# mlcolab/Pathfinder.jl

Hardware: AMD Instinct MI355X
Metric: ELBO draws/sec (multipathfinder hot path: fit + ELBO + pool + PSIS + resample) (higher is better)
Workload: dtype f64

## Files before the change

### pathfinder.jl_amd/csrc/api_ctx.hip

```cpp
#include "api_internal.h"

#include <map>
#include <mutex>
#include <string>
#include <stdarg.h>
#include <stdio.h>

static thread_local char g_err[1024] = "";

void pf_set_error(const char *fmt, ...) {
    va_list ap;
    va_start(ap, fmt);
    vsnprintf(g_err, sizeof(g_err), fmt, ap);
    va_end(ap);
}

static hipEvent_t pf_kev_get(pfmi_ctx *c) {
    if (!c->kev_pool.empty()) { hipEvent_t e = c->kev_pool.back(); c->kev_pool.pop_back(); return e; }
    hipEvent_t e = nullptr;
    (void)hipEventCreate(&e);
    return e;
}
static void pf_kernel_resolve(pfmi_ctx *c, bool keep) {
    for (auto &p : c->kpending) {
// ... 5 lines not shown
        }
        if (p.e0) c->kev_pool.push_back(p.e0);
        if (p.e1) c->kev_pool.push_back(p.e1);
    }
    c->kpending.clear();
}
void pf_kernel_begin(pfmi_ctx *c) {
    if (c->profile == 1) (void)hipEventRecord(c->kev0, c->stream);
    else if (c->profile == 2) {
        if (c->kpending.size() >= 4096) pf_kernel_resolve(c, true);
        if (c->kcur) c->kev_pool.push_back(c->kcur);
        c->kcur = pf_kev_get(c);
        if (c->kcur) (void)hipEventRecord(c->kcur, c->stream);
    }
}
void pf_kernel_end(pfmi_ctx *c, const char *name) {
    if (c->profile == 2) {
        hipEvent_t e1 = pf_kev_get(c);
        if (e1) (void)hipEventRecord(e1, c->stream);
        c->kpending.push_back({name, c->kcur, e1});
        c->kcur = nullptr;
        return;
    }
    if (c->profile != 1) return;
    (void)hipEventRecord(c->kev1, c->stream);
    (void)hipEventSynchronize(c->kev1);
    float ms = 0.f;
    (void)hipEventElapsedTime(&ms, c->kev0, c->kev1);
    KernelStat &s = c->kstats[name];
    s.ms += ms;
    s.launches += 1;
}

#define PF_ARENA_BYTES (16u << 20)
#define PF_ARENA_MAX (4u << 20)
void pf_arena_reset(pfmi_ctx *c) { c->arena.off = 0; }
int32_t pf_upload(pfmi_ctx *c, void *dst, const void *src, size_t bytes) {
    if (bytes == 0) return PFMI_OK;
    if (bytes > PF_ARENA_MAX) {
        PF_HIP(hipMemcpyAsync(dst, src, bytes, hipMemcpyHostToDevice, c->stream));
        PF_HIP(hipStreamSynchronize(c->stream));
        pf_arena_reset(c);
        return PFMI_OK;
    }
    PinArena &a = c->arena;
    if (!a.base) {
        void *pp = nullptr;
        PF_HIP(hipHostMalloc(&pp, PF_ARENA_BYTES, hipHostMallocDefault));
        a.base = reinterpret_cast<char *>(pp); a.cap = PF_ARENA_BYTES; a.off = 0;
    }
    if (a.off + bytes > a.cap) {
        PF_HIP(hipStreamSynchronize(c->stream));
        a.off = 0;
    }
    memcpy(a.base + a.off, src, bytes);
    PF_HIP(hipMemcpyAsync(dst, a.base + a.off, bytes, hipMemcpyHostToDevice, c->stream));
    a.off += (bytes + 255) & ~(size_t)255;
    return PFMI_OK;
}
#define PF_DL_BYTES (4u << 20)
#define PF_DL_MAX (1u << 20)
int32_t pf_download(pfmi_ctx *c, void *dst, const void *src, size_t bytes) {
    if (bytes == 0) return PFMI_OK;
    PinArena &a = c->dl;
    if (bytes <= PF_DL_MAX) {
        if (!a.base) {
            void *pp = nullptr;
            PF_HIP(hipHostMalloc(&pp, PF_DL_BYTES, hipHostMallocMapped));
            a.base = reinterpret_cast<char *>(pp); a.cap = PF_DL_BYTES; a.off = 0;
        }
        if (a.off + bytes <= a.cap) {
            static const bool immediate = [] { const char *e = getenv("PFMI_DL_IMMEDIATE"); return e && e[0] == '1'; }();
            if (immediate) PF_HIP(hipMemcpyAsync(a.base + a.off, src, bytes, hipMemcpyDeviceToHost, c->stream));
            c->dl_pending.push_back(DlPending{dst, a.base + a.off, bytes, c->defer, immediate ? nullptr : static_cast<const char *>(src), immediate});
            a.off += (bytes + 255) & ~(size_t)255;
            return PFMI_OK;
        }
    }
    PF_TRY(pf_dl_flush(c));
    PF_HIP(hipMemcpyAsync(dst, src, bytes, hipMemcpyDeviceToHost, c->stream));
    return PFMI_OK;
}
static void pf_deferred_drop(pfmi_ctx *c) { c->dl_pending.clear(); c->post_sync.clear(); c->dl.off = 0; }
#define PF_DL_NSEG 24
struct DlSegs { const char *src[PF_DL_NSEG]; char *dst[PF_DL_NSEG]; uint32_t bytes[PF_DL_NSEG]; };
__global__ __launch_bounds__(256) void pf_dl_gather_kernel(DlSegs S) {
    const int y = blockIdx.y;
    const char *src = S.src[y];
    char *dst = S.dst[y];
    const uint32_t n = S.bytes[y];
    if (((reinterpret_cast<uintptr_t>(src) | reinterpret_cast<uintptr_t>(dst) | n) & 7u) == 0) {
        const uint32_t n8 = n >> 3;
        for (uint32_t i = blockIdx.x * 256 + threadIdx.x; i < n8; i += gridDim.x * 256)
            reinterpret_cast<uint64_t *>(dst)[i] = reinterpret_cast<const uint64_t *>(src)[i];
    } else {
        for (uint32_t i = blockIdx.x * 256 + threadIdx.x; i < n; i += gridDim.x * 256) dst[i] = src[i];
    }
}
int32_t pf_dl_flush(pfmi_ctx *c) {
    DlSegs S;
    int n = 0;
    uint32_t big = 0;
    auto launch = [&]() -> int32_t {
        if (n == 0) return PFMI_OK;
        const unsigned gx = big > (64u << 10) ? 32 : big > (4u << 10) ? 4 : 1;
        hipLaunchKernelGGL(pf_dl_gather_kernel, dim3(gx, (unsigned)n), dim3(256), 0, c->stream, S);
        PF_HIP(hipGetLastError());
        n = 0; big = 0;
        return PFMI_OK;
    };
    for (DlPending &q : c->dl_pending) {
        if (q.issued || q.src == nullptr) continue;
        S.src[n] = q.src; S.dst[n] = const_cast<char *>(q.slot); S.bytes[n] = (uint32_t)q.bytes;
        if ((uint32_t)q.bytes > big) big = (uint32_t)q.bytes;
        q.issued = true;
        if (++n == PF_DL_NSEG) PF_TRY(launch());
    }
    return launch();
}
int32_t pf_stream_sync(pfmi_ctx *c) {
    {
        const int32_t rf = pf_dl_flush(c);
        if (rf != PFMI_OK) { pf_deferred_drop(c); return rf; }
    }
    const hipError_t e = hipStreamSynchronize(c->stream);
    if (e != hipSuccess) { pf_deferred_drop(c); PF_HIP(e); }
    for (const DlPending &q : c->dl_pending) memcpy(q.dst, q.slot, q.bytes);
    c->dl_pending.clear();
    c->dl.off = 0;
    pf_arena_reset(c);
    int32_t rc = PFMI_OK;
    std::vector<std::function<int32_t()>> hooks;
    hooks.swap(c->post_sync);
    for (auto &h : hooks) { const int32_t r = h(); if (rc == PFMI_OK) rc = r; }
    return rc;
}
void pf_download_forget(pfmi_ctx *c) {
    size_t w = 0;
    for (size_t i = 0; i < c->dl_pending.size(); ++i) if (c->dl_pending[i].keep) c->dl_pending[w++] = c->dl_pending[i];
    c->dl_pending.resize(w);
    if (w == 0) c->dl.off = 0;
}
int32_t ensure_pinned(pfmi_ctx *c, size_t x_bytes, size_t lp_bytes) {
    for (int b = 0; b < 2; ++b) {
        if (x_bytes > c->pin_x_cap) {
            if (c->pin_x[b]) (void)hipHostFree(c->pin_x[b]);
            c->pin_x[b] = nullptr;
            PF_HIP(hipHostMalloc(&c->pin_x[b], x_bytes, hipHostMallocDefault));
        }
        if (lp_bytes > c->pin_lp_cap) {
            if (c->pin_lp[b]) (void)hipHostFree(c->pin_lp[b]);
            c->pin_lp[b] = nullptr;
            PF_HIP(hipHostMalloc(&c->pin_lp[b], lp_bytes, hipHostMallocDefault));
        }
        if (!c->cb_ev[b]) PF_HIP(hipEventCreateWithFlags(&c->cb_ev[b], hipEventDisableTiming));
    }
    if (x_bytes > c->pin_x_cap) c->pin_x_cap = x_bytes;
    if (lp_bytes > c->pin_lp_cap) c->pin_lp_cap = lp_bytes;
    return PFMI_OK;
}

namespace {
std::mutex g_dbg_mu;
std::map<std::string, const char *> g_dbg;
}
const char *pf_debug_get(const char *name) {
    {
        std::lock_guard<std::mutex> lk(g_dbg_mu);
        auto it = g_dbg.find(name);
        if (it != g_dbg.end()) return it->second;
    }
    static const bool env_hooks = [] { const char *e = getenv("PFMI_DEBUG_HOOKS"); return e && e[0] == '1'; }();
    return env_hooks ? getenv(name) : nullptr;
}

void stream_abandon(pfmi_ctx *c) {
    for (hipStream_t s : {c->s_opt, c->s_fit, c->s_scan1}) if (s) (void)hipStreamSynchronize(s);
    for (hipStream_t s : c->s_cb) if (s) (void)hipStreamSynchronize(s);
    c->sr.active = false;
    c->stream_pending = false;
    c->stream_drain = false;
}

void lbc_abandon(pfmi_ctx *c) {
    if (!c->lbc.active) return;
    (void)hipStreamSynchronize(c->stream);
    c->lbc.active = false;
    c->opt_pending = false;
}

extern "C" {

const char *pfmi_last_error(void) { return g_err; }

int32_t pfmi_debug_set(const char *key, const char *value) {
    PF_CHECK(key != nullptr && strncmp(key, "PFMI_", 5) == 0, PFMI_ERR_ARG, "debug_set: keys are the PFMI_* hook names");
    const char *copy = (value && value[0]) ? strdup(value) : nullptr;
    PF_CHECK(copy != nullptr || !(value && value[0]), PFMI_ERR_ARG, "debug_set: out of memory");
    std::lock_guard<std::mutex> lk(g_dbg_mu);
    g_dbg[key] = copy;
    return PFMI_OK;
}
int32_t pfmi_version(void) { return 100; }

int32_t pfmi_device_count(int32_t *count) {
    PF_CHECK(count != nullptr, PFMI_ERR_ARG, "null count");
    int n = 0;
    hipError_t e = hipGetDeviceCount(&n);
    if (e != hipSuccess) { *count = 0; pf_set_error("hipGetDeviceCount: %s", hipGetErrorString(e)); return PFMI_ERR_HIP; }
    *count = n;
    return PFMI_OK;
}

int32_t pfmi_create(int32_t device, pfmi_ctx **out) {
    PF_CHECK(out != nullptr, PFMI_ERR_ARG, "null out");
    *out = nullptr;
    int n = 0;
    PF_HIP(hipGetDeviceCount(&n));
    PF_CHECK(n > 0, PFMI_ERR_HIP, "no HIP device visible: libpfmi has no CPU fallback");
    PF_CHECK(device >= 0 && device < n, PFMI_ERR_ARG, "device %d out of range (%d devices)", device, n);
    hipDeviceProp_t prop;
    PF_HIP(hipGetDeviceProperties(&prop, device));
    PF_CHECK(strncmp(prop.gcnArchName, "gfx950", 6) == 0, PFMI_ERR_UNSUPPORTED,
             "libpfmi is built for gfx950 (MI355X) only; device %d is %s", device, prop.gcnArchName);
    PF_HIP(hipSetDevice(device));
    pfmi_ctx *c = new pfmi_ctx();
    c->device = device;
    c->ncu = prop.multiProcessorCount;
    PF_HIP(hipStreamCreateWithFlags(&c->stream, hipStreamNonBlocking));
    PF_HIP(hipEventCreate(&c->ev0));
    PF_HIP(hipEventCreate(&c->ev1));
    PF_HIP(hipEventCreate(&c->kev0));
    PF_HIP(hipEventCreate(&c->kev1));
    *out = c;
    return PFMI_OK;
}

int32_t pfmi_destroy(pfmi_ctx *c) {
    if (!c) return PFMI_OK;
    pf_comm_ctx_dying(c);
    (void)hipSetDevice(c->device);
    stream_abandon(c);
    lbc_abandon(c);
    (void)hipStreamSynchronize(c->stream);
    for (int b = 0; b < 2; ++b) {
        if (c->pin_x[b]) (void)hipHostFree(c->pin_x[b]);
        if (c->pin_lp[b]) (void)hipHostFree(c->pin_lp[b]);
        if (c->cb_ev[b]) (void)hipEventDestroy(c->cb_ev[b]);
    }
    if (c->arena.base) (void)hipHostFree(c->arena.base);
    if (c->dl.base) (void)hipHostFree(c->dl.base);
    (void)hipEventDestroy(c->ev0); (void)hipEventDestroy(c->ev1);
    (void)hipEventDestroy(c->kev0); (void)hipEventDestroy(c->kev1);
    pf_kernel_resolve(c, false);
    for (hipEvent_t e : c->kev_pool) (void)hipEventDestroy(e);
    for (hipEvent_t e : {c->sg_fit, c->sg_opt, c->sg_scan[0], c->sg_scan[1], c->sg_start}) if (e) (void)hipEventDestroy(e);
    for (hipStream_t s : {c->s_opt, c->s_fit, c->s_scan1}) if (s) (void)hipStreamDestroy(s);
    for (hipStream_t s : c->s_cb) if (s) (void)hipStreamDestroy(s);
    for (hipEvent_t e : c->sg_cb) if (e) (void)hipEventDestroy(e);
    if (c->h_prog) (void)hipHostFree(c->h_prog);
    if (c->lc_status) (void)hipHostFree(c->lc_status);
    if (c->h_list) (void)hipHostFree(c->h_list);
    (void)hipStreamDestroy(c->stream);
    delete c;
    return PFMI_OK;
}

int32_t pfmi_sync(pfmi_ctx *c) {
    PF_CTX(c);
    return pf_stream_sync(c);
}

int32_t pfmi_timer_start(pfmi_ctx *c) {
    PF_CTX(c);
    PF_HIP(hipEventRecord(c->ev0, c->stream));
    return PFMI_OK;
}
int32_t pfmi_timer_stop(pfmi_ctx *c, double *ms) {
    PF_CTX(c);
    PF_HIP(hipEventRecord(c->ev1, c->stream));
    PF_HIP(hipEventSynchronize(c->ev1));
    float f = 0.f;
    PF_HIP(hipEventElapsedTime(&f, c->ev0, c->ev1));
    if (ms) *ms = f;
    return PFMI_OK;
}
int32_t pfmi_profile(pfmi_ctx *c, int32_t enable) {
    PF_CTX(c);
    PF_CHECK(enable >= 0 && enable <= 2, PFMI_ERR_ARG, "profile: mode %d outside 0..2", enable);
    pf_kernel_resolve(c, false);
    c->profile = enable;
    c->kstats.clear();
    return PFMI_OK;
}
int32_t pfmi_kernel_time(pfmi_ctx *c, const char *name, double *ms, int64_t *launches) {
    PF_CTX(c);
    PF_CHECK(name != nullptr, PFMI_ERR_ARG, "null name");
    pf_kernel_resolve(c, true);
    if (strcmp(name, "qf_handover_lost") == 0) {
        if (ms) *ms = 0.0;
        if (launches) *launches = c->qf_lost_total;
        return PFMI_OK;
    }
    if (strncmp(name, "qf:", 3) == 0) {
        auto pl = c->qf_plans.find(name);
        if (ms) *ms = 0.0;
        if (launches) *launches = (pl == c->qf_plans.end()) ? 0 : pl->second;
        return PFMI_OK;
    }
    auto it = c->kstats.find(name);
    if (ms) *ms = (it == c->kstats.end()) ? 0.0 : it->second.ms;
    if (launches) *launches = (it == c->kstats.end()) ? 0 : it->second.launches;
    return PFMI_OK;
}

int32_t pfmi_defer_downloads(pfmi_ctx *c, int32_t mode) {
    PF_CHECK(c != nullptr, PFMI_ERR_ARG, "null pfmi_ctx");
    if (mode < 0) { pf_deferred_drop(c); c->defer = false; return PFMI_OK; }
    c->defer = mode != 0;
    return PFMI_OK;
}

int32_t pfmi_host_rand_u64(uint64_t seed, uint64_t t0, int64_t n, uint32_t stream, uint64_t *out) {
    PF_CHECK(n >= 0 && (out != nullptr || n == 0), PFMI_ERR_ARG, "host_rand_u64: bad arguments");
    const uint32_t key0 = (uint32_t)seed, key1 = (uint32_t)(seed >> 32);
    for (int64_t i = 0; i < n; ++i) {
        const uint64_t t = t0 + (uint64_t)i;
        uint32_t c0 = (uint32_t)t, c1 = (uint32_t)(t >> 32), c2 = stream, c3 = 0u, k0 = key0, k1 = key1;
        for (int r = 0; r < 10; ++r) {
            const uint64_t p0 = (uint64_t)0xD2511F53u * c0, p1 = (uint64_t)0xCD9E8D57u * c2;
            const uint32_t n0 = (uint32_t)(p1 >> 32) ^ c1 ^ k0, n2 = (uint32_t)(p0 >> 32) ^ c3 ^ k1;
            c1 = (uint32_t)p1; c3 = (uint32_t)p0; c0 = n0; c2 = n2;
            k0 += 0x9E3779B9u; k1 += 0xBB67AE85u;
        }
        out[i] = (uint64_t)c0 | ((uint64_t)c1 << 32);
    }
    return PFMI_OK;
}
int32_t pfmi_host_rand_u64_multi(int32_t m, const uint64_t *seeds, const uint64_t *t0, int64_t n, uint32_t stream, uint64_t *out) {
    PF_CHECK(m >= 0 && n >= 0 && (m == 0 || (seeds && t0)) && (out != nullptr || (int64_t)m * n == 0), PFMI_ERR_ARG, "host_rand_u64_multi: bad arguments");
    for (int32_t j = 0; j < m; ++j) PF_TRY(pfmi_host_rand_u64(seeds[j], t0[j], n, stream, out + (size_t)j * (size_t)n));
    return PFMI_OK;
}

int32_t pfmi_malloc_dev(pfmi_ctx *c, int64_t bytes, void **dev_ptr) {
    PF_CTX(c);
    PF_CHECK(dev_ptr != nullptr && bytes > 0, PFMI_ERR_ARG, "malloc_dev: bad arguments");
    PF_HIP(hipMalloc(dev_ptr, (size_t)bytes));
    return PFMI_OK;
}
int32_t pfmi_free_dev(pfmi_ctx *c, void *dev_ptr) {
    PF_CTX(c);
    if (dev_ptr) PF_HIP(hipFree(dev_ptr));
    return PFMI_OK;
}
int32_t pfmi_host_alloc(int64_t bytes, void **host_ptr) {
    PF_CHECK(bytes > 0 && host_ptr, PFMI_ERR_ARG, "host_alloc: bad arguments");
    *host_ptr = nullptr;
    PF_HIP(hipHostMalloc(host_ptr, (size_t)bytes, hipHostMallocPortable | hipHostMallocMapped));
    return PFMI_OK;
}
int32_t pfmi_host_free(void *host_ptr) {
    if (host_ptr) PF_HIP(hipHostFree(host_ptr));
    return PFMI_OK;
}
int32_t pfmi_memcpy_h2d(pfmi_ctx *c, void *dst, const void *src, int64_t bytes) {
    PF_CTX(c);
    return pf_upload(c, dst, src, (size_t)bytes);
}
int32_t pfmi_memcpy_d2h(pfmi_ctx *c, void *dst, const void *src, int64_t bytes) {
    PF_CTX(c);
    return d2h(c, dst, src, (size_t)bytes);
}

}
```

### pathfinder.jl_amd/csrc/api_elbo.hip

```cpp
#include "api_internal.h"

#include <algorithm>
#include <array>
#include <chrono>
#include <memory>
#include <thread>
#include <vector>

static void host_callback_block(pfmi_ctx *c, const double *X, int d, int64_t n, double *out) {
    const TargetDev &T = c->target;
    int t = c->cb_threads;
    if (t > n) t = (int)n;
    if (t <= 1) { T.fn(X, d, n, out, T.user); return; }
    const int64_t per = (n + t - 1) / t;
    std::vector<std::thread> th;
    th.reserve((size_t)t - 1);
    for (int i = 1; i < t; ++i) {
        const int64_t j0 = (int64_t)i * per, j1 = std::min<int64_t>(n, j0 + per);
        if (j0 >= j1) break;
        try {
            th.emplace_back([=, &T] { T.fn(X + (size_t)j0 * (size_t)d, d, j1 - j0, out + j0, T.user); });
        } catch (...) {
            T.fn(X + (size_t)j0 * (size_t)d, d, j1 - j0, out + j0, T.user);
        }
    }
    T.fn(X, d, std::min<int64_t>(n, per), out, T.user);
    for (std::thread &x : th) x.join();
}

int32_t callback_logp(pfmi_ctx *c, const double *d_x, int64_t n, double *d_lp) {
    const int d = c->d;
    int64_t chunk = (int64_t)((64ll << 20) / (sizeof(double) * (size_t)d));
    if (chunk < 1) chunk = 1;
    if (chunk > n) chunk = n;
    PF_TRY(ensure_pinned(c, sizeof(double) * (size_t)chunk * d, sizeof(double) * (size_t)chunk));
    for (int64_t s0 = 0; s0 < n; s0 += chunk) {
        const int64_t ns = (n - s0 < chunk) ? n - s0 : chunk;
        PF_TRY(d2h(c, c->pin_x[0], d_x + (size_t)s0 * d, sizeof(double) * (size_t)ns * d));
        host_callback_block(c, reinterpret_cast<const double *>(c->pin_x[0]), d, ns, reinterpret_cast<double *>(c->pin_lp[0]));
        PF_TRY(pf_upload(c, d_lp + s0, c->pin_lp[0], sizeof(double) * (size_t)ns));
    }
    return PFMI_OK;
}

int64_t devcb_chunk_fits(const pfmi_ctx *c, int64_t per_fit_doubles, int64_t nf, int64_t N) {
    double mb = 2048.0;
    const char *e = pf_debug_get("PFMI_DEVCB_CHUNK_MB");
    if (e && atof(e) > 0) mb = atof(e);
    else {
        const int64_t ngroups = (N + 15) / 16, ncu = c->ncu > 0 ? c->ncu : 256;
        const int64_t split = ngroups / 16 > 0 ? ngroups / 16 : 1;
        const double want_mb = (double)((2 * ncu + split - 1) / split) * sizeof(double) * (double)per_fit_doubles / 1048576.0;
        size_t free_b = 0, total_b = 0;
        if (want_mb > mb && hipMemGetInfo(&free_b, &total_b) == hipSuccess) {
            const double cap_mb = (double)free_b / 4.0 / 1048576.0;
            mb = want_mb < cap_mb ? want_mb : (cap_mb > mb ? cap_mb : mb);
        }
    }
    int64_t chunk = (int64_t)(mb * 1048576.0 / (sizeof(double) * (double)per_fit_doubles));
    if (chunk < 1) chunk = 1;
    if (chunk > nf) chunk = nf > 0 ? nf : 1;
    return chunk;
}

int32_t devcb_logp(pfmi_ctx *c, const double *d_x, int64_t n, double *d_lp, const int32_t *d_points, int64_t npts, int64_t N) {
    pf_kernel_begin(c);
    c->target.dev_fn(d_x, c->d, n, d_lp, (void *)c->stream, c->target.user);
    pf_kernel_end(c, "device_callback");
    PF_HIP(hipGetLastError());
    return pf_launch_nan_failed(c, npts, N, d_points, d_lp);
}

int32_t elbo_reserve(pfmi_ctx *c, size_t P, int32_t K, int64_t N) {
    PF_TRY(c->logp.ensure(sizeof(double) * P * N));
    PF_TRY(c->logq.ensure(sizeof(double) * P * N));
    PF_TRY(c->elbo.ensure(sizeof(double) * P));
    PF_TRY(c->se.ensure(sizeof(double) * P));
    return c->best_iter.ensure(sizeof(int64_t) * K);
}

int32_t devcb_scan_block(pfmi_ctx *c, hipStream_t ss, const int32_t *list, const uint64_t *seeds, int64_t n, int64_t N, const double *d_u,
                         int64_t ustride, double *bx, double *blp) {
    PF_TRY(pf_launch_elbo_draws(c, list, seeds, n, 0, N, d_u, ustride, bx, (int64_t)c->d * N, c->logp.as<double>(), c->logq.as<double>(), N,
                                false, true));
    pf_kernel_begin(c);
    c->target.dev_fn(bx, c->d, n * N, blp, (void *)ss, c->target.user);
    pf_kernel_end(c, "device_callback");
    PF_HIP(hipGetLastError());
    return pf_launch_scatter_rows(c, n, N, list, blp, c->logp.as<double>());
}

extern "C" {

int32_t pfmi_set_callback_threads(pfmi_ctx *c, int32_t nthreads) {
    PF_CTX(c);
    PF_CHECK(nthreads >= 1 && nthreads <= 1024, PFMI_ERR_ARG, "set_callback_threads: 1 <= nthreads <= 1024");
    c->cb_threads = nthreads;
    return PFMI_OK;
}

int32_t pfmi_elbo_batch_enqueue(pfmi_ctx *c, int64_t N, const uint64_t *seeds, const double *u_host) {
    PF_CTX_MUT(c);
    PF_CHECK(c->fitted, PFMI_ERR_STATE, "elbo_batch: call pfmi_fit_batch first");
    PF_CHECK(c->target.kind >= 0, PFMI_ERR_STATE, "elbo_batch: call pfmi_set_target first");
    PF_CHECK(c->target.d == c->d, PFMI_ERR_ARG, "target dimension %d != trace dimension %d", c->target.d, c->d);
    PF_CHECK(N >= 1 && seeds, PFMI_ERR_ARG, "elbo_batch: bad arguments");
    const int64_t P = c->P;
    const int d = c->d;
    c->N_e = N;
    PF_TRY(elbo_reserve(c, (size_t)P, c->K, N));
    int64_t nf = 0;
    for (int k = 0; k < c->K; ++k) nf += c->path_npts(k) - 1;
    const size_t off_ls = sizeof(uint64_t) * (size_t)P, off_li = off_ls + sizeof(uint64_t) * (size_t)(nf > 0 ? nf : 1);
    const size_t up_bytes = off_li + sizeof(int32_t) * (size_t)(nf > 0 ? nf : 1);
    std::vector<char> stage(up_bytes);
    memcpy(stage.data(), seeds, sizeof(uint64_t) * (size_t)P);
    {
        uint64_t *ls = reinterpret_cast<uint64_t *>(stage.data() + off_ls);
        int32_t *li = reinterpret_cast<int32_t *>(stage.data() + off_li);
        int64_t t = 0;
        for (int k = 0; k < c->K; ++k)
            for (int64_t p = c->off[k] + 1; p < c->off[k] + c->path_npts(k); ++p, ++t) { li[t] = (int32_t)p; ls[t] = seeds[p]; }
    }
    PF_TRY(c->seeds.ensure(up_bytes + 16));
    c->d_stream_tab = nullptr;
    PF_TRY(pf_upload(c, c->seeds.p, stage.data(), up_bytes));
    uint64_t *d_lseeds = reinterpret_cast<uint64_t *>(c->seeds.as<char>() + off_ls);
    int32_t *d_list = reinterpret_cast<int32_t *>(c->seeds.as<char>() + off_li);
    const double *d_u = nullptr;
    if (u_host) {
        PF_TRY(c->ubuf.ensure(sizeof(double) * (size_t)P * d * N));
        PF_TRY(pf_upload(c, c->ubuf.p, u_host, sizeof(double) * (size_t)P * d * N));
        d_u = c->ubuf.as<double>();
    }
    const int64_t ustride = (int64_t)d * N;
    if (c->target.kind == PFMI_TARGET_DEVICE_CALLBACK) {
        const int64_t per = (int64_t)d * N;
        int64_t chunk = devcb_chunk_fits(c, per, nf, N);
        int nb = nf > 1 ? PF_DCB_NB : 1;
        if (const char *ov = pf_debug_get("PFMI_DEVCB_OVERLAP")) { const int v = atoi(ov); nb = (v <= 0 || nf <= 1) ? 1 : (v < PF_DCB_NB ? (v < 2 ? 2 : v) : PF_DCB_NB); }
        if (nb > 1) {
            size_t free_b = 0, total_b = 0;
            double have = 0.0;
            for (int b = 0; b < PF_DCB_NB; ++b) have += (double)c->dcb_x[b].cap;
            if (hipMemGetInfo(&free_b, &total_b) == hipSuccess) have += (double)free_b;
            if ((double)nb * (double)sizeof(double) * (double)chunk * (double)(per + N) > 0.5 * have || chunk * nb > nf) chunk = (chunk + nb - 1) / nb;
            if (chunk < 1) chunk = 1;
        }
        for (int b = 0; b < nb; ++b) {
            PF_TRY(c->dcb_x[b].ensure(sizeof(double) * (size_t)chunk * per));
            PF_TRY(c->dcb_lp[b].ensure(sizeof(double) * (size_t)chunk * N));
        }
        for (int b = 1; b < nb; ++b)
            if (!c->s_cb[b - 1]) PF_HIP(hipStreamCreateWithFlags(&c->s_cb[b - 1], hipStreamNonBlocking));
        for (int b = 0; b < nb; ++b)
            if (!c->sg_cb[b]) PF_HIP(hipEventCreateWithFlags(&c->sg_cb[b], hipEventDisableTiming));
        if (nb > 1) {
            PF_HIP(hipEventRecord(c->sg_cb[0], c->stream));
            for (int b = 1; b < nb; ++b) PF_HIP(hipStreamWaitEvent(c->s_cb[b - 1], c->sg_cb[0], 0));
        }
        c->cb_bytes_dev = 0.0;
        int64_t blk = 0;
        for (int64_t s0 = 0; s0 < nf; s0 += chunk, ++blk) {
            const int64_t ns = (nf - s0 < chunk) ? nf - s0 : chunk;
            const int b = (int)(blk % nb);
            hipStream_t ss = b ? c->s_cb[b - 1] : c->stream;
            StreamSwap sw(c, ss);
            PF_TRY(devcb_scan_block(c, ss, d_list + s0, d_lseeds + s0, ns, N, d_u, ustride, c->dcb_x[b].as<double>(), c->dcb_lp[b].as<double>()));
            c->cb_bytes_dev += (double)sizeof(double) * (double)ns * (double)per;
        }
        for (int b = 1; b < nb && b < blk; ++b) {
            PF_HIP(hipEventRecord(c->sg_cb[b], c->s_cb[b - 1]));
            PF_HIP(hipStreamWaitEvent(c->stream, c->sg_cb[b], 0));
        }
    } else if (c->target.kind != PFMI_TARGET_HOST_CALLBACK) {
        PF_TRY(pf_launch_elbo_draws(c, d_list, d_lseeds, nf, 0, N, d_u, ustride, nullptr, 0, c->logp.as<double>(),
                                    c->logq.as<double>(), N, true, true));
    } else {
        const int64_t per = (int64_t)d * N;
        int64_t chunk = (int64_t)((64ll << 20) / (sizeof(double) * (size_t)per));
        if (chunk < 1) chunk = 1;
        if (chunk > nf) chunk = nf > 0 ? nf : 1;
        const size_t xb = sizeof(double) * (size_t)chunk * per, lb = sizeof(double) * (size_t)chunk * N;
        PF_TRY(ensure_pinned(c, xb, lb));
        for (int b = 0; b < 2; ++b) { PF_TRY(c->cb_x[b].ensure(xb)); PF_TRY(c->cb_lp[b].ensure(lb)); }
        c->cb_seconds = 0.0; c->cb_bytes_d2h = 0.0;
        const int64_t nblocks = (nf + chunk - 1) / chunk;
        auto enqueue = [&](int64_t i) -> int32_t {
            const int b = (int)(i & 1);
            const int64_t s0 = i * chunk, ns = (nf - s0 < chunk) ? nf - s0 : chunk;
            PF_TRY(pf_launch_elbo_draws(c, d_list + s0, d_lseeds + s0, ns, 0, N, d_u, ustride, c->cb_x[b].as<double>(), per,
                                        c->logp.as<double>(), c->logq.as<double>(), N, false, true));
            PF_HIP(hipMemcpyAsync(c->pin_x[b], c->cb_x[b].p, sizeof(double) * (size_t)ns * per, hipMemcpyDeviceToHost, c->stream));
            PF_HIP(hipEventRecord(c->cb_ev[b], c->stream));
            return PFMI_OK;
        };
        if (nblocks > 0) PF_TRY(enqueue(0));
        for (int64_t i = 0; i < nblocks; ++i) {
            const int b = (int)(i & 1);
            const int64_t s0 = i * chunk, ns = (nf - s0 < chunk) ? nf - s0 : chunk;
            if (i + 1 < nblocks) PF_TRY(enqueue(i + 1));
            PF_HIP(hipEventSynchronize(c->cb_ev[b]));
            const auto t0 = std::chrono::steady_clock::now();
            host_callback_block(c, reinterpret_cast<const double *>(c->pin_x[b]), d, ns * N, reinterpret_cast<double *>(c->pin_lp[b]));
            c->cb_seconds += std::chrono::duration<double>(std::chrono::steady_clock::now() - t0).count();
            c->cb_bytes_d2h += (double)sizeof(double) * (double)ns * (double)per;
            PF_HIP(hipMemcpyAsync(c->cb_lp[b].p, c->pin_lp[b], sizeof(double) * (size_t)ns * N, hipMemcpyHostToDevice, c->stream));
            PF_TRY(pf_launch_scatter_rows(c, ns, N, d_list + s0, c->cb_lp[b].as<double>(), c->logp.as<double>()));
        }
    }
    PF_TRY(pf_launch_elbo_reduce(c));
    c->elbo_done = true;
    c->elbo_pending = true;
    return PFMI_OK;
}

int32_t pfmi_elbo_batch_wait(pfmi_ctx *c, double *elbo, double *se, int64_t *best_iter) {
    PF_CTX(c);
    PF_CHECK(c->elbo_done, PFMI_ERR_STATE, "elbo_batch_wait: call pfmi_elbo_batch_enqueue first");
    c->elbo_pending = false;
    if (elbo) PF_TRY(pf_download(c, elbo, c->elbo.p, sizeof(double) * c->P));
    if (se) PF_TRY(pf_download(c, se, c->se.p, sizeof(double) * c->P));
    if (best_iter) PF_TRY(pf_download(c, best_iter, c->best_iter.p, sizeof(int64_t) * c->K));
    auto lost2 = std::make_shared<std::array<uint32_t, 2>>();
    (*lost2)[0] = (*lost2)[1] = 0;
    for (int q = 0; q < 2; ++q)
        if (c->qf_share_s[q].cap >= sizeof(uint32_t))
            PF_TRY(pf_download(c, &(*lost2)[(size_t)q], c->qf_share_s[q].as<char>() + c->qf_share_s[q].cap - sizeof(uint32_t), sizeof(uint32_t)));
    auto after = [c, lost2]() -> int32_t {
        uint32_t lost = (*lost2)[0] + (*lost2)[1];
        for (int q = 0; q < 2; ++q)
            if ((*lost2)[(size_t)q] != 0) (void)hipMemsetAsync(c->qf_share_s[q].as<char>() + c->qf_share_s[q].cap - sizeof(uint32_t), 0, sizeof(uint32_t), c->stream);
        {
            const char *fake = pf_debug_get("PFMI_QF_FAKE_LOST");
            if (fake && fake[0] == '1' && !c->qf_no_share) lost = 1;
        }
        if (lost != 0) {
            c->qf_no_share = true;
            c->qf_lost_total += lost;
            c->elbo_done = false; c->pooled = false;
            pf_set_error("ELBO scan: %u workgroup(s) gave up waiting for their fit's constants (GPU shared or dispatch serialised?); results discarded, "
                         "later scans on this context use the two-launch cut: enqueue the step again", lost);
            return PFMI_ERR_RETRY;
        }
        return PFMI_OK;
    };
    if (c->defer) { c->post_sync.push_back(after); return PFMI_OK; }
    PF_TRY(pf_stream_sync(c));
    return after();
}

int32_t pfmi_elbo_batch(pfmi_ctx *c, int64_t N, const uint64_t *seeds, const double *u_host, double *elbo,
                        double *se, int64_t *best_iter) {
    PF_TRY(pfmi_elbo_batch_enqueue(c, N, seeds, u_host));
    return pfmi_elbo_batch_wait(c, elbo, se, best_iter);
}

int32_t pfmi_callback_stats(pfmi_ctx *c, double *callback_seconds, double *bytes_to_host) {
    PF_CTX(c);
    if (callback_seconds) *callback_seconds = c->cb_seconds;
    if (bytes_to_host) *bytes_to_host = c->cb_bytes_d2h;
    return PFMI_OK;
}

int32_t pfmi_callback_stats_dev(pfmi_ctx *c, double *bytes_in_hbm) {
    PF_CTX(c);
    if (bytes_in_hbm) *bytes_in_hbm = c->cb_bytes_dev;
    return PFMI_OK;
}

int32_t pfmi_get_elbo_logs(pfmi_ctx *c, int64_t p, double *logp, double *logq) {
    PF_CTX(c);
    PF_CHECK(c->elbo_done, PFMI_ERR_STATE, "get_elbo_logs: call pfmi_elbo_batch first");
    PF_CHECK(p >= 0 && p < c->P, PFMI_ERR_ARG, "point out of range");
    if (logp) PF_TRY(d2h(c, logp, c->logp.as<double>() + (size_t)p * c->N_e, sizeof(double) * c->N_e));
    if (logq) PF_TRY(d2h(c, logq, c->logq.as<double>() + (size_t)p * c->N_e, sizeof(double) * c->N_e));
    return PFMI_OK;
}

int32_t pfmi_draws(pfmi_ctx *c, int64_t p, uint64_t seed, int64_t n0, int64_t N, const double *u_host, double *X,
                   double *logp, double *logq) {
    PF_CTX_MUT(c);
    PF_CHECK(c->fitted, PFMI_ERR_STATE, "draws: call pfmi_fit_batch first");
    PF_CHECK(p >= 0 && p < c->P && N >= 1 && n0 >= 0, PFMI_ERR_ARG, "draws: bad arguments");
    const int d = c->d;
    const bool have_t = c->target.kind >= 0 && c->target.d == d;
    PF_TRY(c->xbuf.ensure(sizeof(double) * (size_t)d * N));
    PF_TRY(c->scratch.ensure(sizeof(double) * 2 * N + 64));
    double *d_lp = c->scratch.as<double>(), *d_lq = d_lp + N;
    int32_t *d_pt = reinterpret_cast<int32_t *>(d_lq + N);
    uint64_t *d_sd = reinterpret_cast<uint64_t *>(d_lq + N) + 1;
    const int32_t pt = (int32_t)p;
    PF_TRY(pf_upload(c, d_pt, &pt, sizeof(int32_t)));
    PF_TRY(pf_upload(c, d_sd, &seed, sizeof(uint64_t)));
    const double *d_u = nullptr;
    if (u_host) {
        PF_TRY(c->ubuf.ensure(sizeof(double) * (size_t)d * N));
        PF_TRY(pf_upload(c, c->ubuf.p, u_host, sizeof(double) * (size_t)d * N));
        d_u = c->ubuf.as<double>();
    }
    const bool cb = have_t && c->target.kind == PFMI_TARGET_HOST_CALLBACK;
    const bool dcb = have_t && c->target.kind == PFMI_TARGET_DEVICE_CALLBACK;
    PF_TRY(pf_launch_elbo_draws(c, d_pt, d_sd, 1, n0, N, d_u, 0, c->xbuf.as<double>(), 0, d_lp, d_lq, N,
                                have_t && !cb && !dcb, false));
    if (cb) PF_TRY(callback_logp(c, c->xbuf.as<double>(), N, d_lp));
    if (dcb) PF_TRY(devcb_logp(c, c->xbuf.as<double>(), N, d_lp, d_pt, 1, N));
    if (X) PF_TRY(d2h(c, X, c->xbuf.p, sizeof(double) * (size_t)d * N));
    if (logp) PF_TRY(d2h(c, logp, d_lp, sizeof(double) * N));
    if (logq) PF_TRY(d2h(c, logq, d_lq, sizeof(double) * N));
    return PFMI_OK;
}

int32_t pfmi_logpdf(pfmi_ctx *c, int64_t p, int64_t N, const double *X, double *out) {
    PF_CTX(c);
    PF_CHECK(c->fitted, PFMI_ERR_STATE, "logpdf: call pfmi_fit_batch first");
    PF_CHECK(p >= 0 && p < c->P && N >= 1 && X && out, PFMI_ERR_ARG, "logpdf: bad arguments");
    PF_TRY(c->xbuf.ensure(sizeof(double) * (size_t)c->d * N));
    PF_TRY(c->scratch.ensure(sizeof(double) * N));
    PF_TRY(pf_upload(c, c->xbuf.p, X, sizeof(double) * (size_t)c->d * N));
    PF_TRY(pf_launch_logpdf(c, p, N, c->xbuf.as<double>(), c->scratch.as<double>()));
    PF_TRY(d2h(c, out, c->scratch.p, sizeof(double) * N));
    return PFMI_OK;
}

static int32_t mixture_stage(pfmi_ctx *c, int32_t K, const int64_t *points, int64_t N, bool own_comp, bool own_lse,
                             int32_t **d_pts, double **d_comp, double **d_lse) {
    PF_CHECK(c->fitted, PFMI_ERR_STATE, "mixture_logpdf: call pfmi_fit_batch first");
    PF_CHECK(K >= 1 && N >= 1 && points, PFMI_ERR_ARG, "mixture_logpdf: bad arguments (K=%d, N=%lld)", (int)K, (long long)N);
    std::vector<int32_t> pts(K);
    for (int32_t k = 0; k < K; ++k) {
        PF_CHECK(points[k] >= 0 && points[k] < c->P, PFMI_ERR_ARG, "mixture_logpdf: point %lld out of range [0, %lld)",
                 (long long)points[k], (long long)c->P);
        pts[k] = (int32_t)points[k];
    }
    const size_t pbytes = ((sizeof(int32_t) * (size_t)K + 7) / 8) * 8;
    const size_t cbytes = own_comp ? sizeof(double) * (size_t)K * N : 0, lbytes = own_lse ? sizeof(double) * (size_t)N : 0;
    PF_TRY(c->mix.ensure(pbytes + cbytes + lbytes));
    char *base = c->mix.as<char>();
    PF_TRY(pf_upload(c, base, pts.data(), sizeof(int32_t) * (size_t)K));
    *d_pts = reinterpret_cast<int32_t *>(base);
    *d_comp = own_comp ? reinterpret_cast<double *>(base + pbytes) : nullptr;
    *d_lse = own_lse ? reinterpret_cast<double *>(base + pbytes + cbytes) : nullptr;
    return PFMI_OK;
}

int32_t pfmi_mixture_logpdf(pfmi_ctx *c, int32_t K, const int64_t *points, int64_t N, const double *X, double *lse, double *comp) {
    PF_CTX_MUT(c);
    PF_CHECK(c->fitted, PFMI_ERR_STATE, "mixture_logpdf: call pfmi_fit_batch first");
    PF_CHECK(X && lse, PFMI_ERR_ARG, "mixture_logpdf: null X or lse");
    int32_t *d_pts;
    double *d_comp, *d_lse;
    PF_TRY(mixture_stage(c, K, points, N, true, true, &d_pts, &d_comp, &d_lse));
    PF_TRY(c->xbuf.ensure(sizeof(double) * (size_t)c->d * N));
    PF_TRY(pf_upload(c, c->xbuf.p, X, sizeof(double) * (size_t)c->d * N));
    PF_TRY(pf_launch_mixture_logpdf(c, K, d_pts, N, c->xbuf.as<double>(), d_lse, d_comp));
    if (comp) PF_TRY(pf_download(c, comp, d_comp, sizeof(double) * (size_t)K * N));
    PF_TRY(d2h(c, lse, d_lse, sizeof(double) * N));
    return PFMI_OK;
}

int32_t pfmi_mixture_logpdf_dev(pfmi_ctx *c, int32_t K, const int64_t *points, int64_t N, const void *X_dev, void *lse_dev,
                                void *comp_dev) {
    PF_CTX_MUT(c);
    PF_CHECK(c->fitted, PFMI_ERR_STATE, "mixture_logpdf: call pfmi_fit_batch first");
    PF_CHECK(X_dev && lse_dev, PFMI_ERR_ARG, "mixture_logpdf: null X or lse");
    int32_t *d_pts;
    double *d_comp, *d_lse;
    PF_TRY(mixture_stage(c, K, points, N, comp_dev == nullptr, false, &d_pts, &d_comp, &d_lse));
    if (comp_dev) d_comp = reinterpret_cast<double *>(comp_dev);
    return pf_launch_mixture_logpdf(c, K, d_pts, N, reinterpret_cast<const double *>(X_dev), reinterpret_cast<double *>(lse_dev),
                                    d_comp);
}

int32_t pfmi_woodbury_apply(pfmi_ctx *c, int64_t p, int32_t op, int64_t N, const double *X, double *out) {
    PF_CTX(c);
    PF_CHECK(c->fitted, PFMI_ERR_STATE, "woodbury_apply: call pfmi_fit_batch first");
    PF_CHECK(p >= 0 && p < c->P && N >= 1 && X && out, PFMI_ERR_ARG, "woodbury_apply: bad arguments");
    PF_CHECK(op >= PFMI_OP_UNWHITEN && op <= PFMI_OP_INVQUAD, PFMI_ERR_ARG, "woodbury_apply: unknown op %d", op);
    const size_t bytes = sizeof(double) * (size_t)c->d * N;
    PF_TRY(c->xbuf.ensure(bytes));
    PF_TRY(c->gbuf.ensure(bytes));
    PF_TRY(c->scratch.ensure(bytes));
    PF_TRY(pf_upload(c, c->xbuf.p, X, bytes));
    double *in = c->xbuf.as<double>(), *o1 = c->gbuf.as<double>(), *o2 = c->scratch.as<double>();
    const double *res = o1;
    switch (op) {
        case PFMI_OP_UNWHITEN: PF_TRY(pf_launch_woodbury_prim(c, 0, p, N, in, o1)); break;
        case PFMI_OP_WHITEN: PF_TRY(pf_launch_woodbury_prim(c, 1, p, N, in, o1)); break;
        case PFMI_OP_RMUL: PF_TRY(pf_launch_woodbury_prim(c, 2, p, N, in, o1)); break;
        case PFMI_OP_INVUNWHITEN: PF_TRY(pf_launch_woodbury_prim(c, 3, p, N, in, o1)); break;
        case PFMI_OP_MUL:
            PF_TRY(pf_launch_woodbury_prim(c, 2, p, N, in, o1));
            PF_TRY(pf_launch_woodbury_prim(c, 0, p, N, o1, o2));
            res = o2; break;
        case PFMI_OP_SOLVE:
            PF_TRY(pf_launch_woodbury_prim(c, 1, p, N, in, o1));
            PF_TRY(pf_launch_woodbury_prim(c, 3, p, N, o1, o2));
            res = o2; break;
        case PFMI_OP_QUAD:
            PF_TRY(pf_launch_woodbury_prim(c, 2, p, N, in, o1));
            PF_TRY(pf_launch_colsumsq(c, N, o1, o2));
            return d2h(c, out, o2, sizeof(double) * N);
        case PFMI_OP_INVQUAD:
            PF_TRY(pf_launch_woodbury_prim(c, 1, p, N, in, o1));
            PF_TRY(pf_launch_colsumsq(c, N, o1, o2));
            return d2h(c, out, o2, sizeof(double) * N);
    }
    return d2h(c, out, res, bytes);
}

int32_t pfmi_woodbury_diag(pfmi_ctx *c, int64_t p, double *diag) {
    PF_CTX(c);
    PF_CHECK(c->fitted, PFMI_ERR_STATE, "woodbury_diag: call pfmi_fit_batch first");
    PF_CHECK(p >= 0 && p < c->P && diag, PFMI_ERR_ARG, "woodbury_diag: bad arguments");
    PF_TRY(c->gbuf.ensure(sizeof(double) * c->d));
    PF_TRY(pf_launch_woodbury_diag(c, p, c->gbuf.as<double>()));
    return d2h(c, diag, c->gbuf.p, sizeof(double) * c->d);
}

}
```

### pathfinder.jl_amd/csrc/api_fit.hip

```cpp
#include "api_internal.h"
#include "fit_args.h"
#include <limits.h>

#include <memory>
#include <vector>

int32_t fit_reserve(pfmi_ctx *c, size_t P, int32_t K, size_t d, int32_t J, int32_t kpad) {
    const size_t kk = (size_t)kpad * kpad;
    PF_TRY(c->alpha_all.ensure(sizeof(double) * P * d));
    PF_TRY(c->hist_len.ensure(sizeof(int32_t) * P));
    PF_TRY(c->hist_src.ensure(sizeof(int32_t) * P * J));
    PF_TRY(c->hist_acc.ensure(sizeof(int32_t) * P));
    PF_TRY(c->n_rej.ensure(sizeof(int32_t) * K));
    PF_TRY(c->vh.ensure(sizeof(double) * P * d * kpad));
    PF_TRY(c->tmat.ensure(sizeof(double) * P * kk));
    PF_TRY(c->vchol.ensure(sizeof(double) * P * kk));
    PF_TRY(c->rq.ensure(sizeof(double) * P * kk));
    PF_TRY(c->dmat.ensure(sizeof(double) * P * kk));
    PF_TRY(c->sqrt_alpha.ensure(sizeof(double) * P * d));
    PF_TRY(c->mu.ensure(sizeof(double) * P * d));
    PF_TRY(c->logdet.ensure(sizeof(double) * P));
    PF_TRY(c->status.ensure(sizeof(int32_t) * P));
    PF_HIP(hipMemsetAsync(c->hist_src.p, 0, sizeof(int32_t) * P * J, c->stream));
    return PFMI_OK;
}

static int32_t fit_batch_impl(pfmi_ctx *c, int32_t J, double eps) {
    PF_CHECK(c->P > 0, PFMI_ERR_STATE, "fit_batch: no traces set");
    PF_CHECK(J >= 1, PFMI_ERR_ARG, "history_length must be >= 1");
    const int kpad = pf_kpad_for(J);
    PF_CHECK(kpad != 0, PFMI_ERR_UNSUPPORTED, "history_length %d > 32 unsupported", J);
    c->J = J; c->kpad = kpad;
    PF_TRY(fit_reserve(c, (size_t)c->P, c->K, (size_t)c->d, J, kpad));
    if (c->virt) {
        const HistSeg sg{c->st_npts.as<int32_t>(), 0, INT_MAX, nullptr, nullptr, c->hinit};
        PF_TRY(pf_launch_history(c, eps, &sg));
        PF_TRY(pf_launch_fit(c, 0, (int)c->vcap));
    } else {
        PF_TRY(pf_launch_history(c, eps));
        PF_TRY(pf_launch_fit(c));
    }
    c->fitted = true; c->elbo_done = false; c->pooled = false;
    return PFMI_OK;
}

extern "C" {

int32_t pfmi_set_hinit(pfmi_ctx *c, int32_t hinit) {
    PF_CTX(c);
    PF_CHECK(hinit == PFMI_HINIT_GILBERT || hinit == PFMI_HINIT_SCALAR_YS_OVER_YY, PFMI_ERR_ARG, "set_hinit: unknown Hinit %d", hinit);
    c->hinit = hinit;
    return PFMI_OK;
}
int32_t pfmi_fit_batch(pfmi_ctx *c, int32_t J, double eps) {
    PF_CTX_MUT(c);
    return fit_batch_impl(c, J, eps);
}
int32_t pfmi_fit_batch_ex(pfmi_ctx *c, int32_t J, double eps, int32_t hinit) {
    PF_CTX_MUT(c);
    PF_CHECK(hinit == PFMI_HINIT_GILBERT || hinit == PFMI_HINIT_SCALAR_YS_OVER_YY, PFMI_ERR_ARG, "fit_batch_ex: unknown Hinit %d", hinit);
    const int keep = c->hinit;
    c->hinit = hinit;
    const int32_t rc = fit_batch_impl(c, J, eps);
    c->hinit = keep;
    return rc;
}

int32_t pfmi_get_fit_status(pfmi_ctx *c, int32_t *status, int32_t *j_eff, double *logdet, int64_t *n_rejected) {
    PF_CTX(c);
    PF_CHECK(c->fitted, PFMI_ERR_STATE, "get_fit_status: call pfmi_fit_batch first");
    auto r = std::make_shared<std::vector<int32_t>>((size_t)c->K);
    if (status) PF_TRY(pf_download(c, status, c->status.p, sizeof(int32_t) * c->P));
    if (j_eff) PF_TRY(pf_download(c, j_eff, c->hist_len.p, sizeof(int32_t) * c->P));
    if (logdet) PF_TRY(pf_download(c, logdet, c->logdet.p, sizeof(double) * c->P));
    if (n_rejected) PF_TRY(pf_download(c, r->data(), c->n_rej.p, sizeof(int32_t) * c->K));
    const int K = c->K;
    auto widen = [r, n_rejected, K]() -> int32_t {
        if (n_rejected)
            for (int k = 0; k < K; ++k) n_rejected[k] = (*r)[(size_t)k];
        return PFMI_OK;
    };
    if (c->defer) { c->post_sync.push_back(widen); return PFMI_OK; }
    PF_TRY(pf_stream_sync(c));
    return widen();
}

int32_t pfmi_get_fit(pfmi_ctx *c, int64_t p, double *alpha, double *B, double *D, double *qr_factors, double *T,
                     double *V, double *mu, double *logdet) {
    PF_CTX(c);
    PF_CHECK(c->fitted, PFMI_ERR_STATE, "get_fit: call pfmi_fit_batch first");
    PF_CHECK(p >= 0 && p < c->P, PFMI_ERR_ARG, "get_fit: point %lld out of range", (long long)p);
    const int d = c->d, J = c->J, kp = c->kpad;
    int32_t j = 0;
    PF_TRY(d2h(c, &j, c->hist_len.as<int32_t>() + p, sizeof(int32_t)));
    const int m = 2 * j, k = d < m ? d : m;
    std::vector<double> al((size_t)d);
    PF_TRY(d2h(c, al.data(), c->alpha_all.as<double>() + (size_t)p * d, sizeof(double) * d));
    if (alpha) memcpy(alpha, al.data(), sizeof(double) * d);
    if (mu) PF_TRY(d2h(c, mu, c->mu.as<double>() + (size_t)p * d, sizeof(double) * d));
    if (logdet) PF_TRY(d2h(c, logdet, c->logdet.as<double>() + p, sizeof(double)));
    const size_t kk = (size_t)kp * kp;
    std::vector<double> small(kk);
    if (B && j > 0) {
        std::vector<int32_t> src((size_t)J);
        PF_TRY(d2h(c, src.data(), c->hist_src.as<int32_t>() + (size_t)p * J, sizeof(int32_t) * J));
        const int64_t p0 = c->off[(size_t)c->path_of[(size_t)p]];
        std::vector<double> t0((size_t)d), t1((size_t)d), g0((size_t)d), g1((size_t)d);
        for (int cidx = 0; cidx < j; ++cidx) {
            const size_t q0 = (size_t)(p0 + src[(size_t)cidx]) * d, q1 = q0 + d;
            PF_TRY(d2h(c, t0.data(), c->th() + q0, sizeof(double) * d));
            PF_TRY(d2h(c, t1.data(), c->th() + q1, sizeof(double) * d));
            PF_TRY(d2h(c, g0.data(), c->gr() + q0, sizeof(double) * d));
            PF_TRY(d2h(c, g1.data(), c->gr() + q1, sizeof(double) * d));
            for (int i = 0; i < d; ++i) {
                B[i + (size_t)d * cidx] = al[(size_t)i] * (g0[(size_t)i] - g1[(size_t)i]);
                B[i + (size_t)d * (j + cidx)] = t1[(size_t)i] - t0[(size_t)i];
            }
        }
    }
    if (D && m > 0) {
        PF_TRY(d2h(c, small.data(), c->dmat.as<double>() + (size_t)p * kk, sizeof(double) * kk));
        for (int a = 0; a < m; ++a)
            for (int b = 0; b < m; ++b) D[a + (size_t)m * b] = small[(size_t)a * kp + b];
    }
    if (T && k > 0) {
        PF_TRY(d2h(c, small.data(), c->tmat.as<double>() + (size_t)p * kk, sizeof(double) * kk));
        for (int a = 0; a < k; ++a)
            for (int b = 0; b < k; ++b) T[a + (size_t)k * b] = small[(size_t)a * kp + b];
    }
    if (V && k > 0) {
        PF_TRY(d2h(c, small.data(), c->vchol.as<double>() + (size_t)p * kk, sizeof(double) * kk));
        for (int a = 0; a < k; ++a)
            for (int b = 0; b < k; ++b) V[a + (size_t)k * b] = small[(size_t)a * kp + b];
    }
    if (qr_factors && m > 0) {
        std::vector<double> vh((size_t)d * kp);
        PF_TRY(d2h(c, vh.data(), c->vh.as<double>() + (size_t)p * d * kp, sizeof(double) * d * kp));
        PF_TRY(d2h(c, small.data(), c->rq.as<double>() + (size_t)p * kk, sizeof(double) * kk));
        for (int b = 0; b < m; ++b)
            for (int i = 0; i < d; ++i) {
                double v;
                if (i <= b && i < k) v = small[(size_t)i * kp + b];
                else if (b < k) v = vh[(size_t)i * kp + b];
                else v = 0.0;
                qr_factors[i + (size_t)d * b] = v;
            }
    }
    return PFMI_OK;
}

}
```

### pathfinder.jl_amd/csrc/api_inputs.hip

```cpp
#include "api_internal.h"

int32_t set_packed_layout(pfmi_ctx *c, int32_t K, int32_t d, const int64_t *counts) {
    c->off.assign((size_t)K + 1, 0);
    for (int k = 0; k < K; ++k) c->off[k + 1] = c->off[k] + counts[k];
    const int64_t P = c->off[K];
    PF_CHECK(P < (1ll << 31), PFMI_ERR_UNSUPPORTED, "too many trace points");
    c->path_of.resize((size_t)P);
    for (int k = 0; k < K; ++k)
        for (int64_t p = c->off[k]; p < c->off[k + 1]; ++p) c->path_of[(size_t)p] = k;
    c->K = K; c->d = d; c->P = P; c->virt = false;
    PF_TRY(c->d_off.ensure(sizeof(int64_t) * (K + 1)));
    PF_TRY(c->d_path_of.ensure(sizeof(int32_t) * P));
    PF_TRY(pf_upload(c, c->d_off.p, c->off.data(), sizeof(int64_t) * (K + 1)));
    return pf_upload(c, c->d_path_of.p, c->path_of.data(), sizeof(int32_t) * P);
}

int32_t staging_reserve(pfmi_ctx *c, int32_t K, size_t cap, int32_t d) {
    PF_TRY(c->st_theta.ensure(sizeof(double) * K * cap * d));
    PF_TRY(c->st_grad.ensure(sizeof(double) * K * cap * d));
    PF_TRY(c->st_lp.ensure(sizeof(double) * K * cap));
    PF_TRY(c->st_npts.ensure(sizeof(int32_t) * K));
    return c->lb_x0.ensure(sizeof(double) * (size_t)K * d);
}

#define PF_LBC_WINDOW 4
void lbc_begin(pfmi_ctx *c, int32_t K, int32_t J, int32_t maxiters, double g_tol, int32_t *prog) {
    LbcState &O = c->lbc;
    O.K = K; O.J = J; O.maxiters = maxiters; O.g_tol = g_tol;
    { const char *rj = pf_debug_get("PFMI_LBFGS_REJECT_EVERY"); O.reject_every = rj ? atoi(rj) : 0; }
    O.issued = 0; O.seen = 0; O.max_rounds = (int64_t)maxiters * (25 + 30) + 1; O.finished = false;
    O.rounds = 0; O.columns = 0; O.h_prog = prog;
    __atomic_store_n(c->lc_status, (int64_t)K, __ATOMIC_RELEASE);
}

int32_t lbc_issue_rounds(pfmi_ctx *c, hipStream_t s) {
    LbcState &O = c->lbc;
    const int64_t w = __atomic_load_n(c->lc_status, __ATOMIC_ACQUIRE);
    const int64_t round = w >> 32, active = w & 0xffffffffll;
    if (round > O.seen) O.seen = round;
    if (round == O.seen && active == 0) O.finished = true;
    const TargetDev &T = c->target;
    const int d = T.d;
    while (!O.finished && O.issued < O.max_rounds && O.issued - O.seen < PF_LBC_WINDOW) {
        T.grad_fn(c->lc_X.as<double>(), d, O.K, c->lc_out.as<double>(), (void *)s, T.grad_user);
        O.columns += O.K;
        ++O.issued;
        PF_TRY(pf_launch_lbc_step(c, O.issued, s));
        O.rounds = O.issued;
    }
    if (!O.finished && O.issued >= O.max_rounds && O.seen >= O.issued) O.finished = true;
    return PFMI_OK;
}

static int32_t lbc_enqueue(pfmi_ctx *c, int32_t K, const double *x0, int32_t J, int32_t maxiters, double g_tol) {
    const TargetDev &T = c->target;
    PF_CHECK(K > 0 && x0 && maxiters >= 0, PFMI_ERR_ARG, "optimize_batch: bad arguments");
    PF_CHECK(J >= 1 && J <= 32, PFMI_ERR_UNSUPPORTED, "optimize_batch: history_length %d outside 1..32 (closure target)", J);
    const int d = T.d;
    const size_t cap = (size_t)maxiters + 1;
    {
        size_t fr = 0, tot = 0;
        PF_HIP(hipMemGetInfo(&fr, &tot));
        const double need = 8.0 * K * ((double)cap * (2.0 * d + 1.0) + (6.0 + 2.0 * J) * d + 1.0) + (double)K * pf_lbc_path_state_bytes(J);
        PF_CHECK(need < 0.8 * (double)fr, PFMI_ERR_UNSUPPORTED, "optimize_batch: %.3g GB needed for K = %d, d = %d, J = %d, maxiters = %d; %.3g GB free",
                 need / 1e9, K, d, J, maxiters, (double)fr / 1e9);
    }
    PF_TRY(staging_reserve(c, K, cap, d));
    PF_TRY(pf_lbc_alloc(c, K, J, d));
    PF_TRY(pf_upload(c, c->lb_x0.p, x0, sizeof(double) * (size_t)K * d));
    if (c->s_opt) PF_HIP(hipStreamSynchronize(c->s_opt));
    lbc_begin(c, K, J, maxiters, g_tol, nullptr);
    c->lbc.active = true;
    c->opt_pending = true; c->opt_K = K; c->opt_cap = (int32_t)cap;
    results_reset(c); c->P = 0;
    pf_kernel_begin(c);
    const int32_t rc = pf_launch_lbc_init(c, c->stream);
    pf_kernel_end(c, "optimize");
    if (rc != PFMI_OK) lbc_abandon(c);
    return rc;
}

extern "C" {

int32_t pfmi_set_target(pfmi_ctx *c, const pfmi_target *t) {
    PF_CTX_MUT(c);
    PF_CHECK(t != nullptr, PFMI_ERR_ARG, "null target");
    PF_CHECK(t->d > 0, PFMI_ERR_ARG, "target dimension must be positive");
    lbc_abandon(c);
    if (c->sr.active && c->sr.closure) stream_abandon(c);
    TargetDev &T = c->target;
    T.kind = t->kind; T.d = t->d; T.r = 0; T.rpad = 0; T.offset = 0.0; T.fn = nullptr; T.dev_fn = nullptr; T.user = nullptr;
    T.grad_fn = nullptr; T.grad_user = nullptr;
    if (t->kind == PFMI_TARGET_GAUSS) {
        PF_CHECK(t->mean && t->a, PFMI_ERR_ARG, "GAUSS target needs mean and a");
        PF_CHECK(t->r >= 0 && t->r <= 16, PFMI_ERR_UNSUPPORTED, "GAUSS target rank %d > 16 unsupported", t->r);
        PF_CHECK(t->r == 0 || (t->Wd && t->G), PFMI_ERR_ARG, "GAUSS target with r > 0 needs Wd and G");
        const int d = t->d, r = t->r, rpad = (r == 0) ? 0 : (r <= 8 ? 8 : 16);
        T.r = r; T.rpad = rpad; T.offset = t->offset;
        PF_TRY(T.mean.ensure(sizeof(double) * d));
        PF_TRY(T.a.ensure(sizeof(double) * d));
        PF_TRY(pf_upload(c, T.mean.p, t->mean, sizeof(double) * d));
        PF_TRY(pf_upload(c, T.a.p, t->a, sizeof(double) * d));
        if (r > 0) {
            std::vector<double> wd((size_t)d * rpad, 0.0), g((size_t)rpad * rpad, 0.0);
            for (int i = 0; i < d; ++i)
                for (int j = 0; j < r; ++j) wd[(size_t)i * rpad + j] = t->Wd[i + (size_t)d * j];
            for (int j = 0; j < r; ++j)
                for (int l = 0; l <= j; ++l) g[(size_t)j * rpad + l] = t->G[j + (size_t)r * l];
            PF_TRY(T.wd.ensure(sizeof(double) * wd.size()));
            PF_TRY(T.g.ensure(sizeof(double) * g.size()));
            PF_TRY(pf_upload(c, T.wd.p, wd.data(), sizeof(double) * wd.size()));
            PF_TRY(pf_upload(c, T.g.p, g.data(), sizeof(double) * g.size()));
            const size_t rows16 = ((size_t)d + 15) / 16 * 16;
            std::vector<double> w16(rows16 * 16, 0.0);
            for (int i = 0; i < d; ++i)
                for (int j = 0; j < r; ++j) w16[(size_t)i * 16 + j] = t->Wd[i + (size_t)d * j];
            PF_TRY(T.wd16.ensure(sizeof(double) * w16.size()));
            PF_TRY(pf_upload(c, T.wd16.p, w16.data(), sizeof(double) * w16.size()));
        }
    } else if (t->kind == PFMI_TARGET_FUNNEL) {
    } else if (t->kind == PFMI_TARGET_HOST_CALLBACK) {
        PF_CHECK(t->fn != nullptr, PFMI_ERR_ARG, "HOST_CALLBACK target needs fn");
        T.fn = t->fn; T.user = t->user;
    } else if (t->kind == PFMI_TARGET_DEVICE_CALLBACK) {
        PF_CHECK(t->dev_fn != nullptr, PFMI_ERR_ARG, "DEVICE_CALLBACK target needs dev_fn");
        T.dev_fn = t->dev_fn; T.user = t->user;
    } else {
        T.kind = -1;
        PF_CHECK(false, PFMI_ERR_ARG, "unknown target kind %d", t->kind);
    }
    return PFMI_OK;
}

int32_t pfmi_set_traces(pfmi_ctx *c, int32_t K, const int64_t *npoints, int32_t d, const double *theta,
                        const double *grad) {
    PF_CTX_MUT(c);
    if (c->sr.active || c->stream_drain) stream_abandon(c);
    lbc_abandon(c);
    PF_CHECK(K > 0 && d > 0 && npoints && theta && grad, PFMI_ERR_ARG, "set_traces: bad arguments");
    for (int k = 0; k < K; ++k) PF_CHECK(npoints[k] >= 1, PFMI_ERR_ARG, "path %d has no points", k);
    results_reset(c);
    PF_TRY(set_packed_layout(c, K, d, npoints));
    const size_t bytes = sizeof(double) * (size_t)c->P * d;
    PF_TRY(c->theta.ensure(bytes));
    PF_TRY(c->grad.ensure(bytes));
    PF_TRY(pf_upload(c, c->theta.p, theta, bytes));
    return pf_upload(c, c->grad.p, grad, bytes);
}

int32_t pfmi_optimize_batch_enqueue(pfmi_ctx *c, int32_t K, const double *x0, int32_t J, int32_t maxiters, double g_tol) {
    PF_CTX_MUT(c);
    if (c->sr.active || c->stream_drain) stream_abandon(c);
    lbc_abandon(c);
    const TargetDev &T = c->target;
    if (T.kind == PFMI_TARGET_DEVICE_CALLBACK && T.grad_fn) return lbc_enqueue(c, K, x0, J, maxiters, g_tol);
    c->lbc.rounds = 0; c->lbc.columns = 0;
    PF_CHECK(T.kind == PFMI_TARGET_GAUSS || T.kind == PFMI_TARGET_FUNNEL, PFMI_ERR_UNSUPPORTED,
             "optimize_batch: needs a built-in target or a DEVICE_CALLBACK target with a gradient closure (pfmi_set_target_gradient)");
    PF_CHECK(K > 0 && x0 && maxiters >= 0, PFMI_ERR_ARG, "optimize_batch: bad arguments");
    PF_CHECK(J >= 1 && J <= 16, PFMI_ERR_UNSUPPORTED, "optimize_batch: history_length %d outside 1..16", J);
    const int d = T.d;
    const size_t cap = (size_t)maxiters + 1;
    PF_TRY(staging_reserve(c, K, cap, d));
    PF_TRY(pf_upload(c, c->lb_x0.p, x0, sizeof(double) * (size_t)K * d));
    pf_kernel_begin(c);
    PF_TRY(pf_launch_lbfgs(c, K, J, maxiters, g_tol, c->lb_x0.as<double>()));
    pf_kernel_end(c, "optimize");
    c->opt_pending = true; c->opt_K = K; c->opt_cap = (int32_t)cap;
    results_reset(c); c->P = 0;
    return PFMI_OK;
}

int32_t pfmi_optimize_batch_wait(pfmi_ctx *c, int64_t *npoints) {
    PF_CTX_MUT(c);
    PF_CHECK(c->opt_pending, PFMI_ERR_STATE, "optimize_batch_wait: no pfmi_optimize_batch_enqueue outstanding");
    PF_CHECK(npoints != nullptr, PFMI_ERR_ARG, "optimize_batch_wait: null npoints");
    if (c->lbc.active) {
        int32_t fin = 0;
        while (true) {
            PF_TRY(pfmi_optimize_batch_pump(c, &fin));
            if (fin) break;
            for (int i = 0; i < 64; ++i) __builtin_ia32_pause();
        }
        c->lbc.active = false;
    }
    c->opt_pending = false;
    const int K = c->opt_K, d = c->target.d;
    const size_t cap = (size_t)c->opt_cap;
    std::vector<int32_t> np32((size_t)K);
    PF_TRY(d2h(c, np32.data(), c->st_npts.p, sizeof(int32_t) * K));
    for (int k = 0; k < K; ++k) {
        PF_CHECK(np32[(size_t)k] >= 1 && (size_t)np32[(size_t)k] <= cap, PFMI_ERR_NUMERIC, "optimize_batch: path %d produced %d points", k,
                 np32[(size_t)k]);
        npoints[k] = np32[(size_t)k];
    }
    PF_TRY(set_packed_layout(c, K, d, npoints));
    const size_t bytes = sizeof(double) * (size_t)c->P * d;
    PF_TRY(c->theta.ensure(bytes));
    PF_TRY(c->grad.ensure(bytes));
    PF_TRY(c->trace_lp.ensure(sizeof(double) * c->P));
    pf_kernel_begin(c);
    PF_TRY(pf_launch_trace_pack(c, (int64_t)cap));
    pf_kernel_end(c, "trace_pack");
    c->have_trace_lp = true;
    return PFMI_OK;
}

int32_t pfmi_optimize_batch(pfmi_ctx *c, int32_t K, const double *x0, int32_t J, int32_t maxiters, double g_tol,
                            int64_t *npoints) {
    PF_CHECK(npoints != nullptr, PFMI_ERR_ARG, "optimize_batch: bad arguments");
    PF_TRY(pfmi_optimize_batch_enqueue(c, K, x0, J, maxiters, g_tol));
    return pfmi_optimize_batch_wait(c, npoints);
}

int32_t pfmi_set_target_gradient(pfmi_ctx *c, pfmi_logp_dev_fn logp_grad_fn, void *user) {
    PF_CTX(c);
    PF_CHECK(c->target.kind == PFMI_TARGET_DEVICE_CALLBACK, PFMI_ERR_ARG, "set_target_gradient: the current target is not a DEVICE_CALLBACK target");
    PF_CHECK(logp_grad_fn != nullptr, PFMI_ERR_ARG, "set_target_gradient: null closure");
    lbc_abandon(c);
    if (c->sr.active && c->sr.closure) stream_abandon(c);
    c->target.grad_fn = logp_grad_fn; c->target.grad_user = user;
    return PFMI_OK;
}

static int32_t lbc_pump_pass(pfmi_ctx *c, int32_t *finished) {
    LbcState &O = c->lbc;
    PF_TRY(lbc_issue_rounds(c, c->stream));
    if (!O.finished) {
        const hipError_t e = hipStreamQuery(c->stream);
        PF_CHECK(e == hipSuccess || e == hipErrorNotReady, PFMI_ERR_HIP, "optimize_batch_pump: %s", hipGetErrorString(e));
    }
    *finished = O.finished ? 1 : 0;
    return PFMI_OK;
}

int32_t pfmi_optimize_batch_pump(pfmi_ctx *c, int32_t *finished) {
    PF_CHECK(c != nullptr && finished != nullptr, PFMI_ERR_ARG, "optimize_batch_pump: null argument");
    PF_CHECK(c->lbc.active, PFMI_ERR_STATE, "optimize_batch_pump: no closure optimisation outstanding");
    PF_HIP(hipSetDevice(c->device));
    const int32_t rc = lbc_pump_pass(c, finished);
    if (rc != PFMI_OK) lbc_abandon(c);
    return rc;
}

int32_t pfmi_optimize_batch_cancel(pfmi_ctx *c) {
    PF_CHECK(c != nullptr, PFMI_ERR_ARG, "null pfmi_ctx");
    PF_HIP(hipSetDevice(c->device));
    lbc_abandon(c);
    return PFMI_OK;
}

int32_t pfmi_optimize_stats(pfmi_ctx *c, int64_t *rounds, int64_t *closure_columns) {
    PF_CHECK(c != nullptr, PFMI_ERR_ARG, "null pfmi_ctx");
    if (rounds) *rounds = c->lbc.rounds;
    if (closure_columns) *closure_columns = c->lbc.columns;
    return PFMI_OK;
}

int32_t pfmi_get_trace(pfmi_ctx *c, int32_t k, double *theta, double *logp, double *grad) {
    PF_CTX(c);
    PF_CHECK(c->P > 0 && k >= 0 && k < c->K, PFMI_ERR_ARG, "get_trace: bad path index");
    const int64_t p0 = c->off[(size_t)k], n = c->path_npts(k);
    const size_t bytes = sizeof(double) * (size_t)n * c->d;
    if (theta) PF_TRY(d2h(c, theta, c->th() + (size_t)p0 * c->d, bytes));
    if (grad) PF_TRY(d2h(c, grad, c->gr() + (size_t)p0 * c->d, bytes));
    if (logp) {
        PF_CHECK(c->have_trace_lp, PFMI_ERR_STATE, "get_trace: log densities exist only for pfmi_optimize_batch traces");
        PF_TRY(d2h(c, logp, c->tlp() + p0, sizeof(double) * n));
    }
    return PFMI_OK;
}

}
```

### pathfinder.jl_amd/csrc/api_internal.h

```cpp
#pragma once
#include "pfmi_common.h"
#include <stdlib.h>
#include <string.h>

#define PF_CTX(c)                                                          \
    do {                                                                   \
        PF_CHECK((c) != nullptr, PFMI_ERR_ARG, "null pfmi_ctx");           \
        PF_HIP(hipSetDevice((c)->device));                                 \
        pf_download_forget(c);                                             \
    } while (0)
#define PF_CTX_MUT(c)                                                      \
    do {                                                                   \
        PF_CTX(c);                                                         \
        PF_TRY(pf_dl_flush(c));                                            \
    } while (0)

inline int32_t d2h(pfmi_ctx *c, void *dst, const void *src, size_t bytes) {
    if (bytes == 0) return PFMI_OK;
    PF_TRY(pf_download(c, dst, src, bytes));
    return pf_stream_sync(c);
}

struct StreamSwap {
    pfmi_ctx *c; hipStream_t keep; int slot; bool seg;
    StreamSwap(pfmi_ctx *c_, hipStream_t s, int qf_slot = 0, bool seg_mode = false) : c(c_), keep(c_->stream), slot(c_->qf_slot), seg(c_->qf_seg_mode) {
        c->stream = s; c->qf_slot = qf_slot; c->qf_seg_mode = seg_mode;
    }
    ~StreamSwap() { c->stream = keep; c->qf_slot = slot; c->qf_seg_mode = seg; }
};

inline void results_reset(pfmi_ctx *c) { c->fitted = false; c->elbo_done = false; c->pooled = false; c->have_trace_lp = false; }

void stream_abandon(pfmi_ctx *c);
void lbc_abandon(pfmi_ctx *c);
int32_t ensure_pinned(pfmi_ctx *c, size_t x_bytes, size_t lp_bytes);

int32_t set_packed_layout(pfmi_ctx *c, int32_t K, int32_t d, const int64_t *counts);
int32_t staging_reserve(pfmi_ctx *c, int32_t K, size_t cap, int32_t d);
void lbc_begin(pfmi_ctx *c, int32_t K, int32_t J, int32_t maxiters, double g_tol, int32_t *prog);
int32_t lbc_issue_rounds(pfmi_ctx *c, hipStream_t s);

int32_t fit_reserve(pfmi_ctx *c, size_t P, int32_t K, size_t d, int32_t J, int32_t kpad);

int32_t elbo_reserve(pfmi_ctx *c, size_t P, int32_t K, int64_t N);
int64_t devcb_chunk_fits(const pfmi_ctx *c, int64_t per_fit_doubles, int64_t nf, int64_t N);
int32_t devcb_scan_block(pfmi_ctx *c, hipStream_t ss, const int32_t *list, const uint64_t *seeds, int64_t n, int64_t N, const double *d_u,
                         int64_t ustride, double *bx, double *blp);
int32_t callback_logp(pfmi_ctx *c, const double *d_x, int64_t n, double *d_lp);
int32_t devcb_logp(pfmi_ctx *c, const double *d_x, int64_t n, double *d_lp, const int32_t *d_points, int64_t npts, int64_t N);
```

### pathfinder.jl_amd/csrc/fit_args.h

```cpp
#pragma once
#include <stdint.h>

struct FitArgs {
    int d, J;
    int seg_l0, seg_len;
    int64_t vcap;
    const int32_t *npts;
    const int64_t *off;
    const int32_t *path_of;
    const double *theta, *grad, *alpha_all;
    const int32_t *hist_len, *hist_src;
    double *vh, *tmat, *vchol, *rq, *dmat, *sqrt_alpha, *mu, *logdet;
    int32_t *status;
    int64_t P;
    double *big;
};
#ifdef __HIPCC__
__device__ __forceinline__ bool pf_fit_point(const FitArgs &A, int64_t idx, int64_t &p) {
    if (A.seg_len == 0) { p = idx; return true; }
    const int k = (int)(idx / A.seg_len), l = A.seg_l0 + (int)(idx - (int64_t)k * A.seg_len);
    p = (int64_t)k * A.vcap + l;
    return l < __hip_atomic_load(A.npts + k, __ATOMIC_RELAXED, __HIP_MEMORY_SCOPE_AGENT);
}
#endif

struct HistSeg { const int32_t *npts; int l_begin, l_end; double *ial_state; int *nacc_state; int hinit; };
```

### pathfinder.jl_amd/csrc/fit_kernels.hip

```cpp
#include "pfmi_common.h"
#include "fit_args.h"
#include <limits.h>
#include <stdlib.h>

#ifndef FITREG_ABLATE
#define FITREG_ABLATE 0
#endif
#ifndef FITREG_XCD
#define FITREG_XCD 1
#endif
#ifndef FITREG_PROF
#define FITREG_PROF 0
#endif
#if FITREG_PROF
#define FR_STAMP(k) do { if ((blockIdx.x & 511) == 7 && threadIdx.x == 0) { const long long t_ = wall_clock64(); prof[k] = t_ - tlast; tlast = t_; } } while (0)
#else
#define FR_STAMP(k) do { } while (0)
#endif
#ifndef HIST_PROF
#define HIST_PROF 0
#endif
#define HIST_THREADS 256
#define FIT_THREADS 256

template <int EPT, int HIST_NT>
__global__ __launch_bounds__(HIST_NT) void pf_history_kernel(
    int d, int J, double eps, const int64_t *__restrict__ off, const double *__restrict__ theta,
    const double *__restrict__ grad, double *__restrict__ alpha_all, int *__restrict__ hist_len,
    int *__restrict__ hist_src, int *__restrict__ n_rej, int *__restrict__ acc_list, HistSeg sg) {
    const int k = blockIdx.x, tid = threadIdx.x;
    const int64_t p0 = off[k];
    const int Ltot = sg.npts ? sg.npts[k] - 1 : (int)(off[k + 1] - p0 - 1);
    const int L = Ltot < sg.l_end - 1 ? Ltot : sg.l_end - 1;
    const int b = sg.l_begin > 0 ? sg.l_begin - 1 : 0;
    if (sg.l_begin > 0 && b >= L) return;
    __shared__ double red[2 * 4 * (HIST_NT / 64)];
    int flip = 0;
    int n_acc = 0;
    int *const acc = acc_list + p0;

    constexpr int NS = EPT <= 6 ? 4 : 3;
    double al[EPT], ial[EPT], tq[NS][EPT], gq[NS][EPT];
    auto load_point = [&](const int pt, double (&tt)[EPT], double (&gg)[EPT]) {
        const size_t row = (size_t)(p0 + (pt <= L ? pt : L)) * d;
#pragma unroll
        for (int e = 0; e < EPT; ++e) {
            const int i = tid + HIST_NT * e, ic = i < d ? i : d - 1;
            tt[e] = theta[row + ic]; gg[e] = grad[row + ic];
        }
    };
#pragma unroll
    for (int e = 0; e < EPT; ++e) {
        const int i = tid + HIST_NT * e, ic = i < d ? i : d - 1;
        if (sg.l_begin > 0) {
            al[e] = alpha_all[(size_t)(p0 + b) * d + ic]; ial[e] = sg.ial_state[(size_t)k * d + ic];
        } else {
            al[e] = 1.0; ial[e] = 1.0;
            if (i < d) alpha_all[(size_t)p0 * d + i] = 1.0;
        }
    }
#pragma unroll
    for (int q = 0; q < NS; ++q) load_point(b + q, tq[q], gq[q]);
    if (sg.l_begin > 0) n_acc = sg.nacc_state[k];
    else if (tid == 0) hist_len[p0] = 0;
#if HIST_PROF
    long long hp[5] = {0, 0, 0, 0, 0}, hp_last = clock64();
#define HP_STAMP(k) do { const long long t_ = clock64(); hp[k] += t_ - hp_last; hp_last = t_; } while (0)
#else
#define HP_STAMP(k) do { } while (0)
#endif
    auto step = [&](const int l, double (&t0)[EPT], double (&g0)[EPT], const double (&t1)[EPT], const double (&g1)[EPT]) {
        HP_STAMP(4);
        double v[4] = {0.0, 0.0, 0.0, 0.0};
        double sv[EPT], yv[EPT];
#pragma unroll
        for (int e = 0; e < EPT; ++e) {
            const bool in = tid + HIST_NT * e < d;
            const double s = in ? t1[e] - t0[e] : 0.0, y = in ? g0[e] - g1[e] : 0.0;
            sv[e] = s; yv[e] = y;
            v[0] += y * s;
            v[1] += y * y;
            v[2] += y * al[e] * y;
            v[3] += s * ial[e] * s;
        }
        load_point(l - 1 + NS, t0, g0);
        HP_STAMP(0);
        pf_block_sum_mv<4, 4, (HIST_NT <= 256 ? HIST_NT / 64 : 0)>(v, red, flip);
        HP_STAMP(1);
        const bool accept = v[0] > eps * v[1];
        if (accept && sg.hinit == 1) {
            const double an = v[0] / v[1], ian = 1.0 / an;
#pragma unroll
            for (int e = 0; e < EPT; ++e) { al[e] = an; ial[e] = ian; }
            n_acc += 1;
        } else if (accept) {
            const double a = v[2], b = v[0], c = v[3], aoc = a / c, rb = 1.0 / b;
#pragma unroll
            for (int e = 0; e < EPT; ++e) {
                const double sa = sv[e] * ial[e];
                const double x = a * ial[e] + yv[e] * yv[e] - aoc * sa * sa;
                al[e] = b / x;
                ial[e] = x * rb;
            }
            n_acc += 1;
        }
        HP_STAMP(2);
#pragma unroll
        for (int e = 0; e < EPT; ++e) {
            const int i = tid + HIST_NT * e;
            if (i < d) alpha_all[(size_t)(p0 + l) * d + i] = al[e];
        }
        if (tid == 0) {
            if (accept) acc[n_acc - 1] = l - 1;
            hist_len[p0 + l] = n_acc < J ? n_acc : J;
            hist_src[(size_t)(p0 + l) * J] = n_acc;
        }
        HP_STAMP(3);
    };
    int l = b + 1;
    for (; l + NS - 1 <= L; l += NS) {
#pragma unroll
        for (int q = 0; q < NS; ++q) step(l + q, tq[q], gq[q], tq[(q + 1) % NS], gq[(q + 1) % NS]);
    }
    const int rem = L - l + 1;
#pragma unroll
    for (int q = 0; q < NS - 1; ++q)
        if (q < rem) step(l + q, tq[q], gq[q], tq[(q + 1) % NS], gq[(q + 1) % NS]);
#if HIST_PROF
    if (k == 0 && (tid & 63) == 0)
        printf("HIST_PROF wave %d: %d steps, cycles per step: dots+loads %lld block sum %lld update %lld stores %lld loop %lld\n", tid >> 6, L,
               hp[0] / L, hp[1] / L, hp[2] / L, hp[3] / L, hp[4] / L);
#endif
    if (tid == 0) n_rej[k] = L > 0 ? L - n_acc : 0;
    if (sg.ial_state) {
#pragma unroll
        for (int e = 0; e < EPT; ++e) { const int i = tid + HIST_NT * e; if (i < d) sg.ial_state[(size_t)k * d + i] = ial[e]; }
        if (tid == 0) sg.nacc_state[k] = n_acc;
    }
    __threadfence_block();
    __syncthreads();
    for (int q = b + 1 + tid; q <= L; q += HIST_NT) {
        int *row = hist_src + (size_t)(p0 + q) * J;
        const int na = row[0], re = na < J ? na : J;
        int first = 0;
        for (int c = 0; c < re; ++c) {
            const int v = acc[na - re + c];
            if (c == 0) first = v; else row[c] = v;
        }
        row[0] = re > 0 ? first : 0;
    }
}

template <int EPT>
__global__ __launch_bounds__(1024) void pf_history_lean_kernel(
    int d, int J, double eps, const int64_t *__restrict__ off, const double *__restrict__ theta,
    const double *__restrict__ grad, double *__restrict__ alpha_all, int *__restrict__ hist_len,
    int *__restrict__ hist_src, int *__restrict__ n_rej, int *__restrict__ acc_list, HistSeg sg) {
    constexpr int HIST_NT = 1024;
    extern __shared__ double hl_ial[];
    const int k = blockIdx.x, tid = threadIdx.x;
    const int64_t p0 = off[k];
    const int Ltot = sg.npts ? sg.npts[k] - 1 : (int)(off[k + 1] - p0 - 1);
    const int L = Ltot < sg.l_end - 1 ? Ltot : sg.l_end - 1;
    const int b = sg.l_begin > 0 ? sg.l_begin - 1 : 0;
    if (sg.l_begin > 0 && b >= L) return;
    __shared__ double red[2 * 4 * (HIST_NT / 64)];
    int flip = 0;
    int n_acc = 0;
    int *const acc = acc_list + p0;
    constexpr bool REREAD = EPT >= 9;
    double al[EPT], tc[REREAD ? 1 : EPT], gc[REREAD ? 1 : EPT], sv[EPT], yv[EPT];
#pragma unroll
    for (int e = 0; e < EPT; ++e) {
        const int i = tid + HIST_NT * e, ic = i < d ? i : d - 1;
        if (sg.l_begin > 0) {
            al[e] = alpha_all[(size_t)(p0 + b) * d + ic]; hl_ial[e * HIST_NT + tid] = sg.ial_state[(size_t)k * d + ic];
        } else {
            al[e] = 1.0; hl_ial[e * HIST_NT + tid] = 1.0;
            if (i < d) alpha_all[(size_t)p0 * d + i] = 1.0;
        }
        if (!REREAD) { tc[REREAD ? 0 : e] = theta[(size_t)(p0 + b) * d + ic]; gc[REREAD ? 0 : e] = grad[(size_t)(p0 + b) * d + ic]; }
    }
    if (sg.l_begin > 0) n_acc = sg.nacc_state[k];
    else if (tid == 0) hist_len[p0] = 0;
    for (int l = b + 1; l <= L; ++l) {
        const size_t row = (size_t)(p0 + l) * d;
        double v[4] = {0.0, 0.0, 0.0, 0.0};
#pragma unroll
        for (int e = 0; e < EPT; ++e) {
            const int i = tid + HIST_NT * e, ic = i < d ? i : d - 1;
            sv[e] = theta[row + ic]; yv[e] = grad[row + ic];
        }
#pragma unroll
        for (int e = 0; e < EPT; ++e) {
            const bool in = tid + HIST_NT * e < d;
            const double t1 = sv[e], g1 = yv[e];
            double t0, g0;
            if (REREAD) {
                const int i = tid + HIST_NT * e, ic = i < d ? i : d - 1;
                t0 = theta[row - d + ic]; g0 = grad[row - d + ic];
            } else { t0 = tc[REREAD ? 0 : e]; g0 = gc[REREAD ? 0 : e]; }
            const double s = in ? t1 - t0 : 0.0, y = in ? g0 - g1 : 0.0;
            if (!REREAD) { tc[REREAD ? 0 : e] = t1; gc[REREAD ? 0 : e] = g1; }
            sv[e] = s; yv[e] = y;
            const double ia = hl_ial[e * HIST_NT + tid];
            v[0] += y * s;
            v[1] += y * y;
            v[2] += y * al[e] * y;
            v[3] += s * ia * s;
        }
        pf_block_sum_mv<4, 4, 0>(v, red, flip);
        const bool accept = v[0] > eps * v[1];
        if (accept && sg.hinit == 1) {
            const double an = v[0] / v[1], ian = 1.0 / an;
#pragma unroll
            for (int e = 0; e < EPT; ++e) { al[e] = an; hl_ial[e * HIST_NT + tid] = ian; }
            n_acc += 1;
        } else if (accept) {
            const double a = v[2], b = v[0], c = v[3], aoc = a / c, rb = 1.0 / b;
#pragma unroll
            for (int e = 0; e < EPT; ++e) {
                const double ia = hl_ial[e * HIST_NT + tid];
                const double sa = sv[e] * ia;
                const double x = a * ia + yv[e] * yv[e] - aoc * sa * sa;
                al[e] = b / x;
                hl_ial[e * HIST_NT + tid] = x * rb;
            }
            n_acc += 1;
        }
#pragma unroll
        for (int e = 0; e < EPT; ++e) {
            const int i = tid + HIST_NT * e;
            if (i < d) alpha_all[(size_t)(p0 + l) * d + i] = al[e];
        }
        if (tid == 0) {
            if (accept) acc[n_acc - 1] = l - 1;
            hist_len[p0 + l] = n_acc < J ? n_acc : J;
            hist_src[(size_t)(p0 + l) * J] = n_acc;
        }
    }
    if (tid == 0) n_rej[k] = L > 0 ? L - n_acc : 0;
    if (sg.ial_state) {
#pragma unroll
        for (int e = 0; e < EPT; ++e) { const int i = tid + HIST_NT * e; if (i < d) sg.ial_state[(size_t)k * d + i] = hl_ial[e * HIST_NT + tid]; }
        if (tid == 0) sg.nacc_state[k] = n_acc;
    }
    __threadfence_block();
    __syncthreads();
    for (int q = b + 1 + tid; q <= L; q += HIST_NT) {
        int *row = hist_src + (size_t)(p0 + q) * J;
        const int na = row[0], re = na < J ? na : J;
        int first = 0;
        for (int c = 0; c < re; ++c) {
            const int v = acc[na - re + c];
            if (c == 0) first = v; else row[c] = v;
        }
        row[0] = re > 0 ? first : 0;
    }
}

__global__ __launch_bounds__(1024) void pf_history_mem_kernel(
    int d, int J, double eps, const int64_t *__restrict__ off, const double *__restrict__ theta,
    const double *__restrict__ grad, double *__restrict__ alpha_all, int *__restrict__ hist_len,
    int *__restrict__ hist_src, int *__restrict__ n_rej, int *__restrict__ acc_list, HistSeg sg) {
    constexpr int HIST_NT = 1024;
    const int k = blockIdx.x, tid = threadIdx.x;
    const int64_t p0 = off[k];
    const int Ltot = sg.npts ? sg.npts[k] - 1 : (int)(off[k + 1] - p0 - 1);
    const int L = Ltot < sg.l_end - 1 ? Ltot : sg.l_end - 1;
    const int b = sg.l_begin > 0 ? sg.l_begin - 1 : 0;
    if (sg.l_begin > 0 && b >= L) return;
    __shared__ double red[2 * 4 * (HIST_NT / 64)];
    int flip = 0;
    int n_acc = 0;
    int *const acc = acc_list + p0;
    if (sg.l_begin > 0) n_acc = sg.nacc_state[k];
    else {
        for (int i = tid; i < d; i += HIST_NT) alpha_all[(size_t)p0 * d + i] = 1.0;
        if (tid == 0) hist_len[p0] = 0;
    }
    for (int l = b + 1; l <= L; ++l) {
        const size_t row = (size_t)(p0 + l) * d;
        double v[4] = {0.0, 0.0, 0.0, 0.0};
        for (int i = tid; i < d; i += HIST_NT) {
            const double s = theta[row + i] - theta[row - d + i], y = grad[row - d + i] - grad[row + i];
            const double al = alpha_all[row - d + i];
            v[0] += y * s;
            v[1] += y * y;
            v[2] += y * al * y;
            v[3] += s * s / al;
        }
        pf_block_sum_mv<4, 4, 0>(v, red, flip);
        const bool accept = v[0] > eps * v[1];
        const double a = v[2], b = v[0], c = v[3], aoc = a / c;
        for (int i = tid; i < d; i += HIST_NT) {
            const double al = alpha_all[row - d + i];
            double an = al;
            if (accept) {
                const double s = theta[row + i] - theta[row - d + i], y = grad[row - d + i] - grad[row + i];
                const double sa = s / al;
                an = sg.hinit == 1 ? v[0] / v[1] : b / (a / al + y * y - aoc * sa * sa);
            }
            alpha_all[row + i] = an;
        }
        if (accept) n_acc += 1;
        if (tid == 0) {
            if (accept) acc[n_acc - 1] = l - 1;
            hist_len[p0 + l] = n_acc < J ? n_acc : J;
            hist_src[(size_t)(p0 + l) * J] = n_acc;
        }
    }
    if (tid == 0) n_rej[k] = L > 0 ? L - n_acc : 0;
    if (sg.nacc_state && tid == 0) sg.nacc_state[k] = n_acc;
    __threadfence_block();
    __syncthreads();
    for (int q = b + 1 + tid; q <= L; q += HIST_NT) {
        int *rowp = hist_src + (size_t)(p0 + q) * J;
        const int na = rowp[0], re = na < J ? na : J;
        int first = 0;
        for (int cc = 0; cc < re; ++cc) {
            const int vv = acc[na - re + cc];
            if (cc == 0) first = vv; else rowp[cc] = vv;
        }
        rowp[0] = re > 0 ? first : 0;
    }
}

#include "fit_args.h"

template <int KPAD>
__device__ __forceinline__ void pf_multi_dot(const double *M, int d, int i0, int c, double (&acc)[KPAD],
                                             double *red) {
#pragma unroll
    for (int cc = 0; cc < KPAD; ++cc) acc[cc] = 0.0;
    for (int i = i0 + (int)threadIdx.x; i < d; i += (int)blockDim.x) {
        const double *row = M + (size_t)i * KPAD;
        const double xc = row[c];
#pragma unroll
        for (int cc = 0; cc < KPAD; ++cc) acc[cc] += xc * row[cc];
    }
    pf_block_sum<KPAD>(acc, red);
}
template <int KPAD, typename F>
__device__ __forceinline__ void pf_vec_dot(const double *M, int d, F f, double (&acc)[KPAD], double *red) {
#pragma unroll
    for (int cc = 0; cc < KPAD; ++cc) acc[cc] = 0.0;
    for (int i = (int)threadIdx.x; i < d; i += (int)blockDim.x) {
        const double *row = M + (size_t)i * KPAD;
        const double x = f(i, row);
#pragma unroll
        for (int cc = 0; cc < KPAD; ++cc) acc[cc] += x * row[cc];
    }
    pf_block_sum<KPAD>(acc, red);
}

template <int KPAD>
__global__ __launch_bounds__(FIT_THREADS) void pf_fit_kernel(FitArgs A) {
    const int tid = threadIdx.x, nt = blockDim.x;
    int64_t p;
    if (!pf_fit_point(A, blockIdx.x, p)) { if (tid == 0) A.status[p] = PFMI_FIT_ABSENT; return; }
    const int d = A.d, J = A.J;
    const int path = A.path_of[p];
    const int64_t p0 = A.off[path];
    const int j = A.hist_len[p], m = 2 * j, k = d < m ? d : m;
    const double *alpha = A.alpha_all + (size_t)p * d;
    double *Vh = A.vh + (size_t)p * d * KPAD;
    double *sqa = A.sqrt_alpha + (size_t)p * d;
    double *mu = A.mu + (size_t)p * d;
    const double *theta_p = A.theta + (size_t)p * d, *grad_p = A.grad + (size_t)p * d;

    __shared__ double red[(FIT_THREADS / 64) * KPAD];
    __shared__ double sP[KPAD], sW[KPAD], sHead[KPAD], sTau[KPAD];
    constexpr bool BIG = KPAD > 32;
    constexpr int MSZ = BIG ? 1 : KPAD * KPAD;
    __shared__ double sD_[MSZ], sR_[MSZ], sT_[MSZ], sV_[MSZ], sG_[MSZ];
    double *sD = sD_, *sR = sR_, *sT = sT_, *sV = sV_, *sG = sG_;
    if constexpr (BIG) {
        const size_t sm0 = (size_t)p * KPAD * KPAD;
        sD = A.dmat + sm0; sR = A.rq + sm0; sT = A.tmat + sm0; sV = A.vchol + sm0;
        sG = A.big + (size_t)blockIdx.x * KPAD * KPAD;
    }
    __shared__ double sScal, sBeta, sLogdetV;
    __shared__ int sStatus;

    double bad = 0.0, ldu = 0.0;
    for (int i = tid; i < d; i += nt) {
        const double al = alpha[i];
        if (!(al > 0.0) || !isfinite(al)) bad = 1.0;
        const double s = sqrt(al);
        sqa[i] = s;
        ldu += log(s);
    }
    {
        double v[2] = {bad, ldu};
        pf_block_sum<2>(v, red);
        bad = v[0]; ldu = v[1];
    }
    if (tid == 0) sStatus = (bad > 0.0) ? PFMI_FIT_A_NOT_PD : PFMI_FIT_OK;
    for (int t = tid; t < KPAD * KPAD; t += nt) { sD[t] = 0.0; sR[t] = 0.0; sT[t] = 0.0; sV[t] = 0.0; sG[t] = 0.0; }
    __syncthreads();
    if (sStatus != PFMI_FIT_OK) {
        for (int i = tid; i < d; i += nt) {
            mu[i] = NAN;
            for (int c = 0; c < KPAD; ++c) Vh[(size_t)i * KPAD + c] = 0.0;
        }
        for (int t = tid; t < KPAD * KPAD; t += nt) {
            A.tmat[(size_t)p * KPAD * KPAD + t] = 0.0; A.vchol[(size_t)p * KPAD * KPAD + t] = 0.0;
            A.rq[(size_t)p * KPAD * KPAD + t] = 0.0; A.dmat[(size_t)p * KPAD * KPAD + t] = 0.0;
        }
        if (tid == 0) { A.status[p] = sStatus; A.logdet[p] = NAN; }
        return;
    }

    for (int i = tid; i < d; i += nt) {
        double *row = Vh + (size_t)i * KPAD;
        const double al = alpha[i], sa = sqa[i];
        for (int c = 0; c < j; ++c) {
            const int src = A.hist_src[(size_t)p * J + c];
            const size_t q0 = (size_t)(p0 + src) * d + i, q1 = (size_t)(p0 + src + 1) * d + i;
            const double y = A.grad[q0] - A.grad[q1];
            const double s = A.theta[q1] - A.theta[q0];
            row[c] = (al * y) / sa;
            row[j + c] = s / sa;
        }
        for (int c = m; c < KPAD; ++c) row[c] = 0.0;
    }
    __threadfence_block();
    __syncthreads();

    double acc[KPAD];
    constexpr int GR = 4;
    for (int c = 0; c < m; c += GR) {
        double accg[GR][KPAD];
#pragma unroll
        for (int g = 0; g < GR; ++g)
#pragma unroll
            for (int cc = 0; cc < KPAD; ++cc) accg[g][cc] = 0.0;
        for (int i = tid; i < d; i += nt) {
            const double *row = Vh + (size_t)i * KPAD;
            double r[KPAD], x[GR];
#pragma unroll
            for (int g = 0; g < GR; ++g) x[g] = 0.0;
#pragma unroll
            for (int cc = 0; cc < KPAD; ++cc) {
                r[cc] = row[cc];
#pragma unroll
                for (int g = 0; g < GR; ++g) if (cc == c + g) x[g] = r[cc];
            }
#pragma unroll
            for (int g = 0; g < GR; ++g)
#pragma unroll
                for (int cc = 0; cc < KPAD; ++cc) accg[g][cc] += x[g] * r[cc];
        }
#pragma unroll
        for (int g = 0; g < GR; ++g) {
            pf_block_sum<KPAD>(accg[g], red);
            if (tid == 0 && c + g < m) {
#pragma unroll
                for (int cc = 0; cc < KPAD; ++cc) sG[(c + g) * KPAD + cc] = accg[g][cc];
            }
        }
    }
    __syncthreads();
    if (tid == 0 && j > 0) {
        double *R = sT, *nRinv = sV, *Mm = sR;
        for (int a = 0; a < j; ++a)
            for (int b = 0; b < j; ++b) {
                R[a * KPAD + b] = (b >= a) ? sG[(j + a) * KPAD + b] : 0.0;
                nRinv[a * KPAD + b] = 0.0;
            }
        for (int c = 0; c < j; ++c)
            for (int r = c; r >= 0; --r) {
                double rhs = (r == c) ? -1.0 : 0.0;
                for (int t = r + 1; t <= c; ++t) rhs -= R[r * KPAD + t] * nRinv[t * KPAD + c];
                nRinv[r * KPAD + c] = rhs / R[r * KPAD + r];
            }
        for (int a = 0; a < j; ++a)
            for (int b = 0; b < j; ++b) {
                sD[a * KPAD + (j + b)] = nRinv[a * KPAD + b];
                sD[(j + a) * KPAD + b] = nRinv[b * KPAD + a];
                double v = (a <= b) ? sG[a * KPAD + b] : sG[b * KPAD + a];
                if (a == b) v += R[a * KPAD + a];
                Mm[a * KPAD + b] = v;
            }
        for (int a = 0; a < j; ++a)
            for (int b = 0; b < j; ++b) {
                double v = 0.0;
                for (int t = 0; t <= b; ++t) v += Mm[a * KPAD + t] * nRinv[t * KPAD + b];
                sG[a * KPAD + b] = v;
            }
        for (int a = 0; a < j; ++a)
            for (int b = 0; b < j; ++b) {
                double v = 0.0;
                for (int t = 0; t <= a; ++t) v += nRinv[t * KPAD + a] * sG[t * KPAD + b];
                sD[(j + a) * KPAD + (j + b)] = v;
            }
        for (int t = 0; t < KPAD * KPAD; ++t) { sT[t] = 0.0; sV[t] = 0.0; sR[t] = 0.0; }
    }
    __syncthreads();

    for (int c = 0; c < k; ++c) {
        if (c == 0) pf_multi_dot<KPAD>(Vh, d, c + 1, c, acc, red);
        if (tid == 0) {
            const double *rowc = Vh + (size_t)c * KPAD;
            double xn2 = 0.0;
#pragma unroll
            for (int cc = 0; cc < KPAD; ++cc) if (cc == c) xn2 = acc[cc];
            const double alpha_c = rowc[c];
            const double xnorm = sqrt(xn2);
            double tau, scal, beta;
            if (xnorm == 0.0) { tau = 0.0; scal = 0.0; beta = alpha_c; }
            else {
                beta = -copysign(hypot(alpha_c, xnorm), alpha_c);
                tau = (beta - alpha_c) / beta;
                scal = 1.0 / (alpha_c - beta);
            }
            sTau[c] = tau; sScal = scal; sBeta = beta;
#pragma unroll
            for (int cc = 0; cc < KPAD; ++cc) {
                const double vdot = rowc[cc] + scal * acc[cc];
                sP[cc] = (cc > c) ? tau * vdot : vdot;
            }
            sT[c * KPAD + c] = tau;
            for (int a = 0; a < c; ++a) {
                double v = 0.0;
                for (int b = a; b < c; ++b) v += sT[a * KPAD + b] * sP[b];
                sT[a * KPAD + c] = -tau * v;
            }
        }
        __syncthreads();
        {
            const double scal = sScal;
            double acc2[KPAD];
#pragma unroll
            for (int cc = 0; cc < KPAD; ++cc) acc2[cc] = 0.0;
            for (int i = c + 1 + tid; i < d; i += nt) {
                double *row = Vh + (size_t)i * KPAD;
                double r[KPAD];
#pragma unroll
                for (int cc = 0; cc < KPAD; ++cc) r[cc] = row[cc];
                double v = 0.0;
#pragma unroll
                for (int cc = 0; cc < KPAD; ++cc) if (cc == c) v = r[cc] * scal;
                double xn = 0.0;
#pragma unroll
                for (int cc = 0; cc < KPAD; ++cc) {
                    if (cc == c) { r[cc] = v; row[cc] = v; }
                    else if (cc > c) { r[cc] -= sP[cc] * v; row[cc] = r[cc]; }
                    if (cc == c + 1) xn = r[cc];
                }
                if (i > c + 1) {
#pragma unroll
                    for (int cc = 0; cc < KPAD; ++cc) acc2[cc] += xn * r[cc];
                }
            }
            if (tid == 0) {
                double *rowc = Vh + (size_t)c * KPAD;
                rowc[c] = sBeta;
#pragma unroll
                for (int cc = 0; cc < KPAD; ++cc) if (cc > c) rowc[cc] -= sP[cc];
            }
            if (c + 1 < k) {
                pf_block_sum<KPAD>(acc2, red);
#pragma unroll
                for (int cc = 0; cc < KPAD; ++cc) acc[cc] = acc2[cc];
            }
        }
        __threadfence_block();
        __syncthreads();
    }
    for (int t = tid; t < k * KPAD; t += nt) {
        const int a = t / KPAD, b = t % KPAD;
        if (b >= a) {
            sR[a * KPAD + b] = (b < m) ? Vh[(size_t)a * KPAD + b] : 0.0;
            Vh[(size_t)a * KPAD + b] = (b == a) ? 1.0 : 0.0;
        }
    }
    __threadfence_block();
    __syncthreads();
    if (tid == 0) {
        int st = PFMI_FIT_OK;
        double ldv = 0.0;
        for (int a = 0; a < k; ++a)
            for (int b = 0; b < m; ++b) {
                double v = 0.0;
                for (int t = a; t < m; ++t) v += sR[a * KPAD + t] * sD[t * KPAD + b];
                sG[a * KPAD + b] = v;
            }
        for (int a = 0; a < k; ++a)
            for (int b = a; b < k; ++b) {
                double v = (a == b) ? 1.0 : 0.0;
                for (int t = b; t < m; ++t) v += sG[a * KPAD + t] * sR[b * KPAD + t];
                sV[a * KPAD + b] = v;
            }
        for (int c = 0; c < k && st == PFMI_FIT_OK; ++c) {
            double diag = sV[c * KPAD + c];
            for (int t = 0; t < c; ++t) diag -= sV[t * KPAD + c] * sV[t * KPAD + c];
            if (!(diag > 0.0) || !isfinite(diag)) { st = PFMI_FIT_C_NOT_PD; break; }
            diag = sqrt(diag);
            sV[c * KPAD + c] = diag;
            ldv += log(diag);
            for (int b = c + 1; b < k; ++b) {
                double v = sV[c * KPAD + b];
                for (int t = 0; t < c; ++t) v -= sV[t * KPAD + c] * sV[t * KPAD + b];
                sV[c * KPAD + b] = v / diag;
            }
        }
        for (int a = k; a < KPAD; ++a) sV[a * KPAD + a] = 1.0;
        sStatus = st;
        sLogdetV = ldv;
    }
    __syncthreads();
    const size_t sm = (size_t)p * KPAD * KPAD;
    if constexpr (!BIG) {
        for (int t = tid; t < KPAD * KPAD; t += nt) {
            A.tmat[sm + t] = sT[t]; A.vchol[sm + t] = sV[t]; A.rq[sm + t] = sR[t]; A.dmat[sm + t] = sD[t];
        }
    } else { (void)sm; __threadfence_block(); }
    if (sStatus != PFMI_FIT_OK) {
        for (int i = tid; i < d; i += nt) mu[i] = NAN;
        if (tid == 0) { A.status[p] = sStatus; A.logdet[p] = NAN; }
        return;
    }
    pf_vec_dot<KPAD>(Vh, d, [&](int i, const double *) { return sqa[i] * grad_p[i]; }, acc, red);
    if (tid == 0) {
#pragma unroll
        for (int cc = 0; cc < KPAD; ++cc) sP[cc] = acc[cc];
        for (int a = 0; a < KPAD; ++a) {
            double v = 0.0;
            for (int b = 0; b <= a; ++b) v += sT[b * KPAD + a] * sP[b];
            sW[a] = v;
        }
    }
    __syncthreads();
    for (int i = tid; i < k; i += nt) {
        const double *row = Vh + (size_t)i * KPAD;
        double v = sqa[i] * grad_p[i];
        for (int cc = 0; cc < KPAD; ++cc) v -= row[cc] * sW[cc];
        sHead[i] = v;
    }
    __syncthreads();
    if (tid == 0) {
        for (int a = 0; a < k; ++a) {
            double v = 0.0;
            for (int b = a; b < k; ++b) v += sV[a * KPAD + b] * sHead[b];
            sHead[a] = v;
        }
        for (int a = k - 1; a >= 0; --a) {
            double v = 0.0;
            for (int b = 0; b <= a; ++b) v += sV[b * KPAD + a] * sHead[b];
            sHead[a] = v;
        }
    }
    __syncthreads();
    auto bvec = [&](int i, const double *row) {
        if (i < k) return sHead[i];
        double v = sqa[i] * grad_p[i];
#pragma unroll
        for (int cc = 0; cc < KPAD; ++cc) v -= row[cc] * sW[cc];
        return v;
    };
    pf_vec_dot<KPAD>(Vh, d, bvec, acc, red);
    if (tid == 0) {
#pragma unroll
        for (int cc = 0; cc < KPAD; ++cc) sP[cc] = acc[cc];
        for (int a = 0; a < KPAD; ++a) {
            double v = 0.0;
            for (int b = a; b < KPAD; ++b) v += sT[a * KPAD + b] * sP[b];
            sTau[a] = v;
        }
    }
    __syncthreads();
    for (int i = tid; i < d; i += nt) {
        const double *row = Vh + (size_t)i * KPAD;
        double v = bvec(i, row);
#pragma unroll
        for (int cc = 0; cc < KPAD; ++cc) v -= row[cc] * sTau[cc];
        mu[i] = theta_p[i] + sqa[i] * v;
    }
    if (tid == 0) {
        A.status[p] = PFMI_FIT_OK;
        A.logdet[p] = 2.0 * (ldu + sLogdetV);
    }
}

template <int KPAD, int RPT, int NT>
__global__ __launch_bounds__(NT, (KPAD <= 8 ? 4 : KPAD <= 12 ? 3 : 2)) void pf_fit_reg_kernel(FitArgs A) {
    int64_t p;
    {
        const int P = (int)gridDim.x, x = blockIdx.x & 7, slot = blockIdx.x >> 3, q8 = P >> 3, r8 = P & 7;
        int idx = x * q8 + (x < r8 ? x : r8) + slot;
        if (FITREG_XCD == 0) idx = blockIdx.x;
        if (!pf_fit_point(A, idx, p)) { if (threadIdx.x == 0) A.status[p] = PFMI_FIT_ABSENT; return; }
    }
    const int tid = threadIdx.x;
    const int d = A.d, J = A.J;
    const int path = A.path_of[p];
    const int64_t p0 = A.off[path];
    const int j = A.hist_len[p], m = 2 * j, k = d < m ? d : m;
    const double *alpha = A.alpha_all + (size_t)p * d;
    double *Vh = A.vh + (size_t)p * d * KPAD;
    double *sqa = A.sqrt_alpha + (size_t)p * d;
    double *mu = A.mu + (size_t)p * d;
    const double *theta_p = A.theta + (size_t)p * d, *grad_p = A.grad + (size_t)p * d;

    constexpr int NVMAX = KPAD;
    __shared__ __attribute__((aligned(16))) double red[2 * (NT / 64) * NVMAX];
    int flip = 0;
    __shared__ double sRow[2][KPAD];
    __shared__ double sD[KPAD * KPAD], sR[KPAD * KPAD], sT[KPAD * KPAD], sV[KPAD * KPAD], sG[KPAD * KPAD];
    __shared__ double sX1[(KPAD / 2) * KPAD], sX2[(KPAD / 2) * KPAD], sX3[(KPAD / 2) * KPAD];
    __shared__ double sGv[KPAD * KPAD], sVt[KPAD * KPAD];
    __shared__ double sT12[KPAD], sDl[KPAD];
    __shared__ double sLogdetV;
    __shared__ int sStatus;

#if FITREG_PROF
    long long prof[10] = {0, 0, 0, 0, 0, 0, 0, 0, 0, 0}, tlast = wall_clock64();
#endif
    double a[RPT][KPAD];
    double bad = 0.0, ldu = 0.0;
    double isa_r[RPT], al_r[RPT];
    int rl_r[RPT];
#pragma unroll
    for (int i = 0; i < RPT; ++i) { const int row = tid + NT * i; rl_r[i] = row < d ? row : d - 1; }
#pragma unroll
    for (int i = 0; i < RPT; ++i) al_r[i] = alpha[rl_r[i]];
#pragma unroll
    for (int i = 0; i < RPT; ++i) {
        const int row = tid + NT * i;
        const double al = al_r[i];
        const double s = sqrt(al);
        isa_r[i] = 1.0 / s;
        if (row < d) {
            if (!(al > 0.0) || !isfinite(al)) bad = 1.0;
            sqa[row] = s;
            ldu += log(s);
        }
    }
    {
        double v[2] = {bad, ldu};
        pf_block_sum_pp<2, NVMAX>(v, red, flip);
        bad = v[0]; ldu = v[1];
    }
    for (int t = tid; t < KPAD * KPAD; t += NT) { sD[t] = 0.0; sR[t] = 0.0; sT[t] = 0.0; sV[t] = 0.0; sG[t] = 0.0; sGv[t] = 0.0; sVt[t] = 0.0; }
    const size_t sm = (size_t)p * KPAD * KPAD;
    if (bad > 0.0) {
#pragma unroll
        for (int i = 0; i < RPT; ++i) {
            const int row = tid + NT * i;
            if (row < d) {
                mu[row] = NAN;
                for (int c = 0; c < KPAD; ++c) Vh[(size_t)row * KPAD + c] = 0.0;
            }
        }
        for (int t = tid; t < KPAD * KPAD; t += NT) { A.tmat[sm + t] = 0.0; A.vchol[sm + t] = 0.0; A.rq[sm + t] = 0.0; A.dmat[sm + t] = 0.0; }
        if (tid == 0) { A.status[p] = PFMI_FIT_A_NOT_PD; A.logdet[p] = NAN; }
        return;
    }
    FR_STAMP(0);
#pragma unroll
    for (int i = 0; i < RPT; ++i)
#pragma unroll
        for (int c = 0; c < KPAD; ++c) a[i][c] = 0.0;
#pragma unroll
    for (int c = 0; c < KPAD / 2; ++c) {
        if (c >= j) continue;
        const int src = A.hist_src[(size_t)p * J + c];
        const double *g0 = A.grad + (size_t)(p0 + src) * d, *g1 = g0 + d, *t0 = A.theta + (size_t)(p0 + src) * d, *t1 = t0 + d;
        double vg0[RPT], vg1[RPT], vt0[RPT], vt1[RPT];
#pragma unroll
        for (int i = 0; i < RPT; ++i) { vg0[i] = g0[rl_r[i]]; vg1[i] = g1[rl_r[i]]; vt0[i] = t0[rl_r[i]]; vt1[i] = t1[rl_r[i]]; }
#pragma unroll
        for (int i = 0; i < RPT; ++i) {
            const bool in = tid + NT * i < d;
            const double y = vg0[i] - vg1[i];
            const double sx = vt1[i] - vt0[i];
            const double by = in ? (al_r[i] * y) * isa_r[i] : 0.0, bs = in ? sx * isa_r[i] : 0.0;
            a[i][c] = by;
            if (j == KPAD / 2) a[i][KPAD / 2 + c] = bs;
            else {
#pragma unroll
                for (int cc = 0; cc < KPAD; ++cc) if (cc == j + c) a[i][cc] = bs;
            }
        }
    }
    FR_STAMP(1);
    double acc[KPAD];
#pragma unroll
    for (int c = 0; c < KPAD; ++c) {
        if (c >= k) continue;
        double *srow = sRow[c & 1];
        if (tid == c) {
#pragma unroll
            for (int cc = 0; cc < KPAD; ++cc) srow[cc] = a[0][cc];
        }
#pragma unroll
        for (int cc = 0; cc < KPAD; ++cc) acc[cc] = 0.0;
#pragma unroll
        for (int i = 0; i < RPT; ++i) {
            const int row = tid + NT * i;
            if (row > c) {
                double xc = 0.0;
#pragma unroll
                for (int cc = 0; cc < KPAD; ++cc) if (cc == c) xc = a[i][cc];
#pragma unroll
                for (int cc = 0; cc < KPAD; ++cc) acc[cc] += xc * a[i][cc];
            }
        }
        pf_block_sum_mv<KPAD, NVMAX>(acc, red, flip);
        double xn2 = 0.0;
#pragma unroll
        for (int cc = 0; cc < KPAD; ++cc) if (cc == c) xn2 = acc[cc];
        const double alpha_c = srow[c];
        double tau, scal, beta;
        if (xn2 == 0.0) { tau = 0.0; scal = 0.0; beta = alpha_c; }
        else {
            beta = -copysign(sqrt(fma(alpha_c, alpha_c, xn2)), alpha_c);
            tau = (beta - alpha_c) / beta;
            scal = 1.0 / (alpha_c - beta);
        }
        double (&wv)[KPAD] = acc;
#pragma unroll
        for (int cc = 0; cc < KPAD; ++cc) {
            const double vdot = srow[cc] + scal * acc[cc];
            wv[cc] = (cc > c) ? tau * vdot : vdot;
        }
        if (tid <= c && tid < KPAD) {
            double v = 0.0;
#pragma unroll
            for (int b = 0; b < KPAD; ++b) if (b >= tid && b < c) v += sT[tid * KPAD + b] * wv[b];
            const double tnew = (tid == c) ? tau : -tau * v;
            sT[tid * KPAD + c] = tnew;
            if (tid == c) {
#pragma unroll
                for (int cc = 0; cc < KPAD; ++cc) if (cc < c) { sGv[c * KPAD + cc] = wv[cc]; sGv[cc * KPAD + c] = wv[cc]; }
                sGv[c * KPAD + c] = fma(scal * scal, xn2, 1.0);
            }
        }
#pragma unroll
        for (int i = 0; i < RPT; ++i) {
            const int row = tid + NT * i;
            if (row > c) {
                double v = 0.0;
#pragma unroll
                for (int cc = 0; cc < KPAD; ++cc) if (cc == c) v = a[i][cc] * scal;
#pragma unroll
                for (int cc = 0; cc < KPAD; ++cc) {
                    if (cc == c) a[i][cc] = v;
                    else if (cc > c) a[i][cc] -= wv[cc] * v;
                }
            } else if (row == c) {
#pragma unroll
                for (int cc = 0; cc < KPAD; ++cc) {
                    if (cc == c) a[i][cc] = beta;
                    else if (cc > c) a[i][cc] -= wv[cc];
                }
            }
        }
    }
    FR_STAMP(2);
    if (tid < k) {
#pragma unroll
        for (int cc = 0; cc < KPAD; ++cc) {
            if (cc >= tid) {
                sR[tid * KPAD + cc] = (cc < m) ? a[0][cc] : 0.0;
                a[0][cc] = (cc == tid) ? 1.0 : 0.0;
            }
            if (cc < k) sVt[tid * KPAD + cc] = a[0][cc];
        }
    }
    __syncthreads();
    for (int t = tid; t < m * m; t += NT) {
        const int aa = t / m, b = t % m, u1 = (aa < b ? aa : b) < k - 1 ? (aa < b ? aa : b) : k - 1;
        double v = 0.0;
        for (int u = 0; u <= u1; ++u) v += sR[u * KPAD + aa] * sR[u * KPAD + b];
        sG[aa * KPAD + b] = v;
    }
    __syncthreads();
    if (j > 0) {
        double *R = sX1, *nRinv = sX2;
        for (int t = tid; t < j * j; t += NT) {
            const int aa = t / j, b = t % j;
            R[aa * KPAD + b] = (b >= aa) ? sG[(j + aa) * KPAD + b] : 0.0;
            nRinv[aa * KPAD + b] = 0.0;
        }
    }
    __syncthreads();
    if (tid < j) {
        const double *R = sX1;
        double *nRinv = sX2;
        const int c = tid;
        for (int r = c; r >= 0; --r) {
            double rhs = (r == c) ? -1.0 : 0.0;
            for (int t = r + 1; t <= c; ++t) rhs -= R[r * KPAD + t] * nRinv[t * KPAD + c];
            nRinv[r * KPAD + c] = rhs / R[r * KPAD + r];
        }
    }
    __syncthreads();
    if (j > 0) {
        for (int t = tid; t < j * j; t += NT) {
            const int aa = t / j, b = t % j;
            sD[aa * KPAD + (j + b)] = sX2[aa * KPAD + b];
            sD[(j + aa) * KPAD + b] = sX2[b * KPAD + aa];
            double v = (aa <= b) ? sG[aa * KPAD + b] : sG[b * KPAD + aa];
            if (aa == b) v += sX1[aa * KPAD + aa];
            sX3[aa * KPAD + b] = v;
        }
    }
    __syncthreads();
    if (j > 0) {
        for (int t = tid; t < j * j; t += NT) {
            const int aa = t / j, b = t % j;
            double v = 0.0;
            for (int u = 0; u <= b; ++u) v += sX3[aa * KPAD + u] * sX2[u * KPAD + b];
            sG[aa * KPAD + b] = v;
        }
    }
    __syncthreads();
    if (j > 0) {
        for (int t = tid; t < j * j; t += NT) {
            const int aa = t / j, b = t % j;
            double v = 0.0;
            for (int u = 0; u <= aa; ++u) v += sX2[u * KPAD + aa] * sG[u * KPAD + b];
            sD[(j + aa) * KPAD + (j + b)] = v;
        }
    }
    __syncthreads();
    FR_STAMP(3);
    for (int t = tid; t < k * m; t += NT) {
        const int aa = t / m, b = t % m;
        double v = 0.0;
        for (int u = aa; u < m; ++u) v += sR[aa * KPAD + u] * sD[u * KPAD + b];
        sG[aa * KPAD + b] = v;
    }
    __syncthreads();
    for (int t = tid; t < k * k; t += NT) {
        const int aa = t / k, b = t % k;
        if (b >= aa) {
            double v = (aa == b) ? 1.0 : 0.0;
            for (int u = b; u < m; ++u) v += sG[aa * KPAD + u] * sR[b * KPAD + u];
            sV[aa * KPAD + b] = v;
        }
    }
    __syncthreads();
    FR_STAMP(4);
    if (tid < 64) {
        const int b = tid;
        double col[KPAD];
#pragma unroll
        for (int t = 0; t < KPAD; ++t) col[t] = (b < k && t <= b) ? sV[t * KPAD + b] : 0.0;
        int status = PFMI_FIT_OK;
        double ldv = 0.0;
#pragma unroll
        for (int c = 0; c < ((FITREG_ABLATE & 1) ? 0 : KPAD); ++c) {
            if (c >= k || status != PFMI_FIT_OK) continue;
            double v = col[c];
#pragma unroll
            for (int t = 0; t < c; ++t) {
                const double vtc = pf_readlane_f64(col[t], c);
                v -= vtc * col[t];
            }
            const double diag = pf_readlane_f64(v, c);
            if (!(diag > 0.0) || !isfinite(diag)) { status = PFMI_FIT_C_NOT_PD; continue; }
            const double dc = sqrt(diag);
            ldv = ldv + log(dc);
            col[c] = (b == c) ? dc : (b > c ? v / dc : col[c]);
        }
#pragma unroll
        for (int t = 0; t < KPAD; ++t) if (b < k && t <= b) sV[t * KPAD + b] = col[t];
        if (b >= k && b < KPAD) sV[b * KPAD + b] = 1.0;
        if (b == 0) { sStatus = status; sLogdetV = ldv; }
    }
    __syncthreads();
    FR_STAMP(5);
    for (int t = tid; t < KPAD * KPAD; t += NT) {
        A.tmat[sm + t] = sT[t]; A.vchol[sm + t] = sV[t]; A.rq[sm + t] = sR[t]; A.dmat[sm + t] = sD[t];
    }
#pragma unroll
    for (int i = 0; i < RPT; ++i) {
        const int row = tid + NT * i;
        if (row < d) {
            double2 *o = reinterpret_cast<double2 *>(Vh + (size_t)row * KPAD);
#pragma unroll
            for (int cc = 0; cc < KPAD; cc += 2) o[cc >> 1] = make_double2(a[i][cc], a[i][cc + 1]);
        }
    }
    if (sStatus != PFMI_FIT_OK) {
#pragma unroll
        for (int i = 0; i < RPT; ++i) { const int row = tid + NT * i; if (row < d) mu[row] = NAN; }
        if (tid == 0) { A.status[p] = sStatus; A.logdet[p] = NAN; }
        return;
    }
    FR_STAMP(6);
    if (FITREG_ABLATE & 2) return;
    double agv[RPT];
#pragma unroll
    for (int i = 0; i < RPT; ++i) {
        const int row = tid + NT * i;
        agv[i] = (row < d) ? sqa[row] * grad_p[row] : 0.0;
    }
#pragma unroll
    for (int cc = 0; cc < KPAD; ++cc) acc[cc] = 0.0;
#pragma unroll
    for (int i = 0; i < RPT; ++i)
#pragma unroll
        for (int cc = 0; cc < KPAD; ++cc) acc[cc] += agv[i] * a[i][cc];
    pf_block_sum_mv<KPAD, NVMAX>(acc, red, flip);
    if (tid < 64) {
        const int aa = tid < KPAD ? tid : KPAD - 1;
        const bool live = tid < k;
        double w1l = 0.0, t1l = 0.0;
#pragma unroll
        for (int b = 0; b < KPAD; ++b) {
            w1l = (b == aa) ? acc[b] : w1l;
            t1l += sT[b * KPAD + aa] * acc[b];
        }
        double hbl = live ? agv[0] : 0.0;
#pragma unroll
        for (int cc = 0; cc < KPAD; ++cc) hbl -= sVt[aa * KPAD + cc] * pf_readlane_f64(t1l, cc);
        hbl = live ? hbl : 0.0;
        double tmpl = 0.0;
#pragma unroll
        for (int b = 0; b < KPAD; ++b) tmpl += sV[aa * KPAD + b] * pf_readlane_f64(hbl, b);
        double hdl = 0.0;
#pragma unroll
        for (int b = 0; b < KPAD; ++b) hdl += sV[b * KPAD + aa] * pf_readlane_f64(tmpl, b);
        const double dll = live ? hdl - hbl : 0.0;
        double w2l = w1l;
#pragma unroll
        for (int b = 0; b < KPAD; ++b) w2l -= sGv[aa * KPAD + b] * pf_readlane_f64(t1l, b);
#pragma unroll
        for (int r = 0; r < KPAD; ++r) w2l += sVt[r * KPAD + aa] * pf_readlane_f64(dll, r);
        double t2l = 0.0;
#pragma unroll
        for (int b = 0; b < KPAD; ++b) t2l += sT[aa * KPAD + b] * pf_readlane_f64(w2l, b);
        if (tid < KPAD) { sT12[tid] = t1l + t2l; sDl[tid] = dll; }
    }
    __syncthreads();
    double t12[KPAD];
#pragma unroll
    for (int cc = 0; cc < KPAD; ++cc) t12[cc] = sT12[cc];
    const double dl0 = (tid < k) ? sDl[tid < KPAD ? tid : 0] : 0.0;
#pragma unroll
    for (int i = 0; i < RPT; ++i) {
        const int row = tid + NT * i;
        if (row < d) {
            double v = agv[i];
#pragma unroll
            for (int cc = 0; cc < KPAD; ++cc) v -= a[i][cc] * t12[cc];
            if (i == 0) v += dl0;
            mu[row] = theta_p[row] + sqa[row] * v;
        }
    }
    FR_STAMP(7);
#if FITREG_PROF
    if ((blockIdx.x & 511) == 7 && tid == 0)
        printf("FITREG_PROF wg %d (10 ns ticks): prologue %lld rows %lld QR %lld gram+D %lld C %lld chol %lld out %lld mean %lld\n", (int)blockIdx.x, prof[0],
               prof[1], prof[2], prof[3], prof[4], prof[5], prof[6], prof[7]);
#endif
    if (tid == 0) {
        A.status[p] = PFMI_FIT_OK;
        A.logdet[p] = 2.0 * (ldu + sLogdetV);
    }
}

int32_t pf_launch_history(pfmi_ctx *c, double eps, const HistSeg *seg) {
    PF_CHECK(c->J <= 64, PFMI_ERR_UNSUPPORTED, "history_length %d > 64 unsupported", c->J);
    HistSeg sg = seg ? *seg : HistSeg{nullptr, 0, INT_MAX, nullptr, nullptr, 0};
    sg.hinit = c->hinit;
    pf_kernel_begin(c);
    {
        const char *hk = pf_debug_get("PFMI_HISTORY_KERNEL");
        if (c->d > 16 * 1024 || (hk && hk[0] == 'm')) {
            hipLaunchKernelGGL(pf_history_mem_kernel, dim3(c->K), dim3(1024), 0, c->stream, c->d, c->J, eps, c->d_off.as<int64_t>(),
                               c->th(), c->gr(), c->alpha_all.as<double>(), c->hist_len.as<int>(),
                               c->hist_src.as<int>(), c->n_rej.as<int>(), c->hist_acc.as<int>(), sg);
            pf_kernel_end(c, "history");
            PF_HIP(hipGetLastError());
            return PFMI_OK;
        }
    }
#define PF_HIST(E, NT)                                                                                           \
    hipLaunchKernelGGL((pf_history_kernel<E, NT>), dim3(c->K), dim3(NT), 0, c->stream, c->d, c->J, eps,           \
                       c->d_off.as<int64_t>(), c->th(), c->gr(),                      \
                       c->alpha_all.as<double>(), c->hist_len.as<int>(), c->hist_src.as<int>(), c->n_rej.as<int>(),          \
                       c->hist_acc.as<int>(), sg)
    if (c->d <= 64) PF_HIST(1, 64); else if (c->d <= 128) PF_HIST(2, 64); else if (c->d <= 256) PF_HIST(4, 64);
    else if (c->d <= 512) PF_HIST(2, 256); else if (c->d <= 1024) PF_HIST(4, 256);
    else { const int ept = (c->d + 1023) / 1024;
           const char *hk = pf_debug_get("PFMI_HISTORY_KERNEL");
           const bool lean = !(hk && hk[0] == 'p');
#define PF_HIST_LEAN(E)                                                                                                  \
    do {                                                                                                                \
        auto kern = pf_history_lean_kernel<E>;                                                                          \
        PF_TRY(pf_raise_lds_limit(c, reinterpret_cast<const void *>(kern), (int)(sizeof(double) * E * 1024)));           \
        hipLaunchKernelGGL(kern, dim3(c->K), dim3(1024), sizeof(double) * E * 1024, c->stream, c->d, c->J, eps,         \
                           c->d_off.as<int64_t>(), c->th(), c->gr(), c->alpha_all.as<double>(), \
                           c->hist_len.as<int>(), c->hist_src.as<int>(), c->n_rej.as<int>(), c->hist_acc.as<int>(), sg);  \
    } while (0)
           if (ept <= 2) PF_HIST(2, 1024);
           else if (ept <= 4) { if (lean) PF_HIST_LEAN(4); else PF_HIST(4, 1024); }
           else if (ept <= 6) { if (lean) PF_HIST_LEAN(6); else PF_HIST(6, 1024); }
           else if (ept <= 8) { if (lean) PF_HIST_LEAN(8); else PF_HIST(8, 1024); }
           else if (ept <= 10) { if (lean) PF_HIST_LEAN(10); else PF_HIST(10, 1024); }
           else if (ept <= 12) PF_HIST(12, 1024); else PF_HIST(16, 1024); }
#undef PF_HIST_LEAN
#undef PF_HIST
    pf_kernel_end(c, "history");
    PF_HIP(hipGetLastError());
    return PFMI_OK;
}

template <int KPAD>
static void launch_fit_t(pfmi_ctx *c, const FitArgs &a) {
    const char *force = pf_debug_get("PFMI_FIT_KERNEL");
    const bool allow_reg = !(force && force[0] == 'm');
    dim3 grid((unsigned)a.P), block(FIT_THREADS);
    if constexpr (KPAD <= 16) {
        if (allow_reg && a.d <= 256) { hipLaunchKernelGGL((pf_fit_reg_kernel<KPAD, 1, 256>), grid, dim3(256), 0, c->stream, a); return; }
        if (allow_reg && a.d <= 512) { hipLaunchKernelGGL((pf_fit_reg_kernel<KPAD, 2, 256>), grid, dim3(256), 0, c->stream, a); return; }
        if (allow_reg && a.d <= 1024) { hipLaunchKernelGGL((pf_fit_reg_kernel<KPAD, 4, 256>), grid, dim3(256), 0, c->stream, a); return; }
    }
    hipLaunchKernelGGL(pf_fit_kernel<KPAD>, grid, block, 0, c->stream, a);
}

int32_t pf_launch_fit_panel(pfmi_ctx *c, const FitArgs &a, bool *handled);
int32_t pf_launch_fit_tsqr(pfmi_ctx *c, const FitArgs &a, bool *handled);

int32_t pf_launch_fit(pfmi_ctx *c, int seg_l0, int seg_len) {
    FitArgs a;
    a.d = c->d; a.J = c->J;
    a.seg_l0 = seg_l0; a.seg_len = seg_len; a.vcap = c->vcap; a.npts = c->st_npts.as<int32_t>();
    PF_CHECK(seg_len == 0 || c->virt, PFMI_ERR_STATE, "fit: segment launches need the streaming layout");
    a.off = c->d_off.as<int64_t>(); a.path_of = c->d_path_of.as<int32_t>();
    a.theta = c->th(); a.grad = c->gr(); a.alpha_all = c->alpha_all.as<double>();
    a.hist_len = c->hist_len.as<int32_t>(); a.hist_src = c->hist_src.as<int32_t>();
    a.vh = c->vh.as<double>(); a.tmat = c->tmat.as<double>(); a.vchol = c->vchol.as<double>();
    a.rq = c->rq.as<double>(); a.dmat = c->dmat.as<double>(); a.sqrt_alpha = c->sqrt_alpha.as<double>();
    a.mu = c->mu.as<double>(); a.logdet = c->logdet.as<double>(); a.status = c->status.as<int32_t>();
    a.P = seg_len > 0 ? (int64_t)c->K * seg_len : c->P;
    a.big = nullptr;
    pf_kernel_begin(c);
    {
        const char *force = pf_debug_get("PFMI_FIT_KERNEL");
        bool handled = false;
        if (!(force && (force[0] == 'm' || force[0] == 'p'))) PF_TRY(pf_launch_fit_tsqr(c, a, &handled));
        if (!handled && !(force && force[0] == 'm')) PF_TRY(pf_launch_fit_panel(c, a, &handled));
        if (handled) {
            pf_kernel_end(c, "fit");
            PF_HIP(hipGetLastError());
            return PFMI_OK;
        }
    }
    if (c->kpad == 64) {
        PF_TRY(c->fit_scratch.ensure(sizeof(double) * (size_t)a.P * 64 * 64));
        a.big = c->fit_scratch.as<double>();
    }
    PF_CHECK((pf_dispatch_kpad<4, 8, 12, 16, 20, 32, 64>(c->kpad, [&](auto KP) { launch_fit_t<KP()>(c, a); })), PFMI_ERR_UNSUPPORTED,
             "unsupported kpad %d", c->kpad);
    pf_kernel_end(c, "fit");
    PF_HIP(hipGetLastError());
    return PFMI_OK;
}
```

### pathfinder.jl_amd/csrc/pfmi_common.h

```cpp
#pragma once
#include <hip/hip_runtime.h>
#include <stdint.h>
#include <chrono>
#include <functional>
#include <memory>
#include <string>
#include <map>
#include <set>
#include <type_traits>
#include <vector>

#include "../../include/pfmi.h"
#include "pfmi_icdftab.h"

#define PF_LOG2PI 1.8378770664093454835606594728112352797227949472755668

void pf_set_error(const char *fmt, ...);
#define PF_HIP(call)                                                                              \
    do {                                                                                          \
        hipError_t e__ = (call);                                                                  \
        if (e__ != hipSuccess) {                                                                  \
            pf_set_error("%s failed: %s (%s:%d)", #call, hipGetErrorString(e__), __FILE__, __LINE__); \
            return PFMI_ERR_HIP;                                                                  \
        }                                                                                         \
    } while (0)
#define PF_CHECK(cond, code, ...)                                                                 \
    do {                                                                                          \
        if (!(cond)) {                                                                            \
            pf_set_error(__VA_ARGS__);                                                            \
            return (code);                                                                        \
        }                                                                                         \
    } while (0)
#define PF_TRY(expr)                                                                              \
    do {                                                                                          \
        int32_t rc__ = (expr);                                                                    \
        if (rc__ != PFMI_OK) return rc__;                                                         \
    } while (0)

struct DevBuf {
    void *p = nullptr;
    size_t cap = 0;
    DevBuf() = default;
    DevBuf(const DevBuf &) = delete;
    DevBuf &operator=(const DevBuf &) = delete;
    DevBuf(DevBuf &&o) noexcept : p(o.p), cap(o.cap) { o.p = nullptr; o.cap = 0; }
    ~DevBuf() { release(); }
    int32_t ensure(size_t bytes) {
        if (bytes <= cap) return PFMI_OK;
        if (p) { (void)hipFree(p); p = nullptr; cap = 0; }
        size_t want = bytes < 256 ? 256 : bytes;
        PF_HIP(hipMalloc(&p, want));
        cap = want;
        return PFMI_OK;
    }
    void release() { if (p) (void)hipFree(p); p = nullptr; cap = 0; }
    template <typename T> T *as() const { return reinterpret_cast<T *>(p); }
};

template <int... KS, typename F>
inline bool pf_dispatch_kpad(int kpad, F &&f) {
    return ((kpad == KS ? (f(std::integral_constant<int, KS>{}), true) : false) || ...);
}
inline int pf_kpad_for(int J) {
    for (int o : {4, 8, 12, 16, 20, 32, 64}) if (2 * J <= o) return o;
    return 0;
}

struct KernelStat { double ms = 0.0; int64_t launches = 0; };

struct PinArena { char *base = nullptr; size_t cap = 0, off = 0; };
struct DlPending { void *dst; const char *slot; size_t bytes; bool keep; const char *src; bool issued; };

struct TargetDev {
    int32_t kind = -1, d = 0, r = 0, rpad = 0;
    double offset = 0.0;
    DevBuf mean, a, wd , g ;
    DevBuf wd16;
    pfmi_logp_fn fn = nullptr;
    pfmi_logp_dev_fn dev_fn = nullptr;
    void *user = nullptr;
    pfmi_logp_dev_fn grad_fn = nullptr;
    void *grad_user = nullptr;
};

struct LbcState {
    bool active = false;
    int K = 0, J = 0, maxiters = 0, reject_every = 0;
    double g_tol = 0.0;
    int64_t issued = 0, seen = 0, max_rounds = 0;
    bool finished = false;
    int64_t rounds = 0, columns = 0;
    int32_t *h_prog = nullptr;
};

struct pfmi_ctx {
    int device = 0;
    hipStream_t stream = nullptr;
    hipEvent_t ev0 = nullptr, ev1 = nullptr, kev0 = nullptr, kev1 = nullptr;
    int profile = 0;
    std::map<std::string, KernelStat> kstats;
    struct PendingStat { const char *name; hipEvent_t e0, e1; };
    std::vector<PendingStat> kpending;
    std::vector<hipEvent_t> kev_pool;
    hipEvent_t kcur = nullptr;
    std::set<const void *> lds_attr_done;
    PinArena arena;
    int cb_threads = 1;
    int hinit = 0;
    PinArena dl;
    std::vector<DlPending> dl_pending;
    bool defer = false;
    std::vector<std::function<int32_t()>> post_sync;
    int ncu = 0;

    int32_t K = 0, d = 0;
    int64_t P = 0;
    std::vector<int64_t> off;
    std::vector<int32_t> path_of;
    DevBuf theta, grad, d_off , d_path_of ;
    TargetDev target;
    bool have_trace_lp = false;
    DevBuf trace_lp;
    DevBuf st_theta, st_grad, st_lp, st_npts;
    bool virt = false;
    int64_t vcap = 0;
    std::vector<int32_t> npts_h;
    const uint64_t *d_stream_tab = nullptr;
    DevBuf hs_ial, hs_nacc;
    int32_t *h_prog = nullptr;
    int h_prog_cap = 0;
    char *h_list = nullptr;
    size_t h_list_cap = 0;
    hipStream_t s_opt = nullptr, s_fit = nullptr, s_scan1 = nullptr;
    hipEvent_t sg_fit = nullptr, sg_opt = nullptr, sg_scan[2] = {nullptr, nullptr}, sg_start = nullptr;
    struct StreamRun {
        bool active = false;
        int K = 0, J = 0, cap = 0, l_next = 0, nseg = 0, minlen = 16, last_min = -1, pub = 16;
        int64_t N = 0, s0 = 0;
        double eps = 0.0;
        uint64_t *d_lseeds = nullptr; int32_t *d_list = nullptr;
        bool scan_used[2] = {false, false};
        int64_t scan_ns[2] = {0, 0};
        int policy = 0, fit_eager = 1;
        int l_fit = 0;
        bool have_seeds = false;
        std::vector<uint64_t> seeds_pt;
        std::chrono::steady_clock::time_point t_progress, t_start;
        std::vector<double> trace;
        double host_s = 0.0; int host_n = 0;
        bool closure = false;
        int64_t dcb_chunk = 1;
        int64_t last_round = -1;
    } sr;
    bool stream_pending = false;
    bool stream_drain = false;
    bool qf_seg_mode = false;
    double *th() const { return virt ? st_theta.as<double>() : theta.as<double>(); }
    double *gr() const { return virt ? st_grad.as<double>() : grad.as<double>(); }
    double *tlp() const { return virt ? st_lp.as<double>() : trace_lp.as<double>(); }
    int64_t path_npts(int k) const { return virt ? (int64_t)npts_h[(size_t)k] : off[(size_t)k + 1] - off[(size_t)k]; }
    int ncu_eff = 0;
    DevBuf lb_hs, lb_hy, lb_x0;

    bool fitted = false;
    int32_t J = 0, kpad = 0;
    DevBuf alpha_all;
    DevBuf hist_len;
    DevBuf hist_src;
    DevBuf hist_acc;
    DevBuf n_rej;
    DevBuf vh;
    DevBuf tmat;
    DevBuf vchol;
    DevBuf rq;
    DevBuf dmat;
    DevBuf sqrt_alpha;
    DevBuf mu;
    DevBuf logdet;
    DevBuf status;
    DevBuf fit_scratch;

    bool elbo_done = false;
    int64_t N_e = 0;
    DevBuf seeds;
    DevBuf logp, logq;
    DevBuf elbo, se;
    DevBuf best_iter;
    DevBuf fit_list;
    DevBuf ubuf;
    DevBuf xbuf;
    DevBuf scratch;
    DevBuf mix;
    DevBuf qf_share_s[2];
    uint32_t qf_epoch_s[2] = {0, 0};
    int qf_slot = 0;
    bool qf_no_share = false;
    int64_t qf_lost_total = 0;
    std::map<std::string, int64_t> qf_plans;

    bool pooled = false;
    int64_t N_r = 0;
    DevBuf pool;
    DevBuf pool_lr;
    DevBuf pool_lp, pool_lq;
    DevBuf pool_points;
    DevBuf pool_seeds;
    int64_t S_w = 0;
    DevBuf lw;
    DevBuf w;
    DevBuf psis_out;
    DevBuf psis_aux;
    DevBuf tailbuf;
    DevBuf cdf;
    DevBuf idx;
    DevBuf gbuf;
    DevBuf sortk, sorti;
    DevBuf cb_x[2], cb_lp[2];
    void *pin_x[2] = {nullptr, nullptr}, *pin_lp[2] = {nullptr, nullptr};
    size_t pin_x_cap = 0, pin_lp_cap = 0;
    hipEvent_t cb_ev[2] = {nullptr, nullptr};
#define PF_DCB_NB 2
    DevBuf dcb_x[PF_DCB_NB], dcb_lp[PF_DCB_NB];
    hipStream_t s_cb[PF_DCB_NB - 1] = {};
    hipEvent_t sg_cb[PF_DCB_NB] = {};
    double cb_seconds = 0.0;
    double cb_bytes_d2h = 0.0;
    double cb_bytes_dev = 0.0;
    bool opt_pending = false;
    LbcState lbc;
    DevBuf lc_X, lc_out, lc_x, lc_g, lc_p, lc_gram, lc_st, lc_ctr;
    int64_t *lc_status = nullptr;
    int32_t opt_K = 0, opt_cap = 0;
    bool elbo_pending = false;
    bool pool_from_best = false;
    DevBuf pool_ok;
    DevBuf fail_seeds;
    DevBuf rs_err;
    DevBuf mom;
    DevBuf mom_part;
    DevBuf pcdf;
    DevBuf pcdf_part;
    DevBuf pcdf_thr;
    DevBuf pcdf_carry;
    DevBuf cross;
    DevBuf pool_center;
    DevBuf apply_z;
    DevBuf apply_part;
    DevBuf apply_y;
    DevBuf apply_v;
};

int32_t pf_upload(pfmi_ctx *c, void *dst, const void *src, size_t bytes);
void pf_arena_reset(pfmi_ctx *c);
int32_t pf_download(pfmi_ctx *c, void *dst, const void *src, size_t bytes);
int32_t pf_stream_sync(pfmi_ctx *c);
int32_t pf_dl_flush(pfmi_ctx *c);
void pf_download_forget(pfmi_ctx *c);

struct HistSeg;
int32_t pf_launch_history(pfmi_ctx *c, double eps, const HistSeg *seg = nullptr);
int32_t pf_launch_fit(pfmi_ctx *c, int seg_l0 = 0, int seg_len = 0);
int32_t pf_launch_elbo_draws(pfmi_ctx *c, const int32_t *d_points, const uint64_t *d_seeds, int64_t nfits,
                             int64_t n0, int64_t N, const double *d_u, int64_t u_stride,
                             double *d_x, int64_t x_stride, double *d_logp, double *d_logq,
                             int64_t log_stride, bool with_target, bool by_point);
int32_t pf_launch_elbo_reduce(pfmi_ctx *c);
int32_t pf_launch_logpdf(pfmi_ctx *c, int64_t point, int64_t N, const double *d_x, double *d_out);
int32_t pf_launch_mixture_logpdf(pfmi_ctx *c, int K, const int32_t *d_points, int64_t N, const double *d_x, double *d_lse,
                                 double *d_comp);
int32_t pf_launch_psis(pfmi_ctx *c, const double *d_lr, int64_t S);
int32_t pf_launch_pool_moments(pfmi_ctx *c, int64_t col_offset, int importance, const double *d_center);
int32_t pf_launch_pool_cdf(pfmi_ctx *c, int64_t col_offset, int importance, int nthr, const double *d_thr, const double *d_carry);
int32_t pf_launch_pool_cross(pfmi_ctx *c, int64_t col_offset, int importance, const double *d_center, const double *d_carry);
int32_t pf_launch_pool_apply(pfmi_ctx *c, int64_t col_offset, int importance, const double *d_center, int r, const double *d_v,
                             const double *d_carry);
const char *pf_debug_get(const char *name);
void pf_comm_ctx_dying(pfmi_ctx *c);
int32_t pf_launch_resample(pfmi_ctx *c, int64_t S, int64_t ndraws, int importance, int replace,
                           uint64_t seed, const double *d_uniforms);
int32_t pf_enqueue_resample(pfmi_ctx *c, int64_t S, int64_t ndraws, int importance, int replace,
                            uint64_t seed, const double *d_uniforms);
int32_t pf_resample_check(pfmi_ctx *c);
int32_t pf_launch_pool_pick(pfmi_ctx *c, int have_fail_seeds);
int32_t pf_launch_nan_failed(pfmi_ctx *c, int64_t npts, int64_t N, const int32_t *d_points, double *d_lp);
int32_t pf_launch_resample_direct(pfmi_ctx *c, int64_t S, int64_t ndraws, const double *d_uniforms);
int32_t pf_launch_gather(pfmi_ctx *c, int64_t ndraws, const int64_t *d_idx, int64_t col_offset, double *d_out, bool skip_unowned = false);
int32_t pf_launch_gather_pos(pfmi_ctx *c, int64_t n, const int64_t *d_idx, const int64_t *d_pos, int64_t col_offset, double *d_out);
int32_t pf_launch_scatter_cols(pfmi_ctx *c, int64_t n, const int64_t *d_pos, const double *d_in, double *d_out);
int32_t pf_launch_idx_digest(pfmi_ctx *c, int64_t ndraws, const int64_t *d_idx, double *d_out4, double local_err);
int32_t pf_launch_logratio(pfmi_ctx *c, int64_t n);
int32_t pf_launch_scatter_rows(pfmi_ctx *c, int64_t ns, int64_t N, const int32_t *d_points, const double *d_src, double *d_dst);
int32_t pf_launch_lbfgs(pfmi_ctx *c, int K, int J, int maxiters, double g_tol, const double *d_x0, int pub_mask = -1, int32_t *h_prog = nullptr);
int32_t pf_launch_trace_pack(pfmi_ctx *c, int64_t cap);
size_t pf_lbc_path_state_bytes(int J);
int32_t pf_lbc_alloc(pfmi_ctx *c, int K, int J, int d);
int32_t pf_launch_lbc_init(pfmi_ctx *c, hipStream_t s);
int32_t pf_launch_lbc_step(pfmi_ctx *c, int64_t round, hipStream_t s);
int32_t pf_launch_woodbury_prim(pfmi_ctx *c, int mode, int64_t p, int64_t N, const double *d_in, double *d_out);
int32_t pf_launch_colsumsq(pfmi_ctx *c, int64_t N, const double *d_x, double *d_out);
int32_t pf_launch_woodbury_diag(pfmi_ctx *c, int64_t p, double *d_out);

inline int32_t pf_raise_lds_limit(pfmi_ctx *c, const void *kern, int bytes) {
    if (c->lds_attr_done.count(kern)) return PFMI_OK;
    PF_HIP(hipFuncSetAttribute(kern, hipFuncAttributeMaxDynamicSharedMemorySize, bytes));
    c->lds_attr_done.insert(kern);
    return PFMI_OK;
}

void pf_kernel_begin(pfmi_ctx *c);
void pf_kernel_end(pfmi_ctx *c, const char *name);

#ifdef __HIPCC__

__device__ __forceinline__ uint32_t pf_xor3_key(uint32_t a, uint32_t b, uint32_t k) {
    if (__builtin_constant_p(k)) return a ^ b ^ k;
    uint32_t r;
    asm("v_bitop3_b32 %0, %1, %2, %3 bitop3:0x96" : "=v"(r) : "v"(a), "v"(b), "s"(k));
    return r;
}
#define PF_NORMAL_ROUNDS 7
template <int ROUNDS>
__device__ __forceinline__ void pf_philox4x32(uint32_t c0, uint32_t c1, uint32_t c2, uint32_t c3,
                                              uint32_t k0, uint32_t k1, uint32_t (&out)[4]) {
#pragma unroll
    for (int r = 0; r < ROUNDS; ++r) {
        uint64_t p0 = (uint64_t)0xD2511F53u * c0;
        uint64_t p1 = (uint64_t)0xCD9E8D57u * c2;
        uint32_t n0 = pf_xor3_key((uint32_t)(p1 >> 32), c1, k0);
        uint32_t n1 = (uint32_t)p1;
        uint32_t n2 = pf_xor3_key((uint32_t)(p0 >> 32), c3, k1);
        uint32_t n3 = (uint32_t)p0;
        c0 = n0; c1 = n1; c2 = n2; c3 = n3;
        k0 += 0x9E3779B9u; k1 += 0xBB67AE85u;
    }
    out[0] = c0; out[1] = c1; out[2] = c2; out[3] = c3;
}
__device__ __forceinline__ void pf_philox_round(uint32_t &c0, uint32_t &c1, uint32_t &c2, uint32_t &c3,
                                                uint32_t &k0, uint32_t &k1) {
    const uint64_t p0 = (uint64_t)0xD2511F53u * c0;
    const uint64_t p1 = (uint64_t)0xCD9E8D57u * c2;
    const uint32_t n0 = (uint32_t)(p1 >> 32) ^ c1 ^ k0;
    const uint32_t n1 = (uint32_t)p1;
    const uint32_t n2 = (uint32_t)(p0 >> 32) ^ c3 ^ k1;
    const uint32_t n3 = (uint32_t)p0;
    c0 = n0; c1 = n1; c2 = n2; c3 = n3;
    k0 += 0x9E3779B9u; k1 += 0xBB67AE85u;
}
__device__ __forceinline__ void pf_philox4x32_10(uint32_t c0, uint32_t c1, uint32_t c2, uint32_t c3, uint32_t k0, uint32_t k1,
                                                 uint32_t (&out)[4]) {
    pf_philox4x32<10>(c0, c1, c2, c3, k0, k1, out);
}
__device__ __forceinline__ void pf_philox_normals(uint32_t c0, uint32_t c1, uint32_t c2, uint32_t c3, uint32_t k0, uint32_t k1,
                                                  uint32_t (&out)[4]) {
    pf_philox4x32<PF_NORMAL_ROUNDS>(c0, c1, c2, c3, k0, k1, out);
}

static __device__ const double PF_ICDF_TAB_DEV[PF_ICDF_ENTRIES][4] = { PF_ICDF_TABLE_ROWS };

template <int NB = PF_ICDF_NB_LDS>
__device__ __forceinline__ void pf_icdf_load(double2 *tab) {
    constexpr int NENT = NB << PF_ICDF_B;
    const double2 *src = reinterpret_cast<const double2 *>(&PF_ICDF_TAB_DEV[0][0]);
    for (int i0 = threadIdx.x; i0 < 2 * NENT; i0 += 4 * blockDim.x) {
        double2 v[4];
#pragma unroll
        for (int u = 0; u < 4; ++u) { const int i = i0 + u * (int)blockDim.x; v[u] = src[i < 2 * NENT ? i : 2 * NENT - 1]; }
#pragma unroll
        for (int u = 0; u < 4; ++u) { const int i = i0 + u * (int)blockDim.x; if (i < 2 * NENT) tab[(i & 1) * NENT + (NENT - 1 - (i >> 1))] = v[u]; }
    }
}
__device__ __forceinline__ double pf_icdf_any(uint32_t x, uint32_t x2) {
    const uint32_t mag = x & 0x7FFFFFFFu;
    double v;
    if (mag >= (1u << PF_ICDF_TAILBITS)) v = (double)mag;
    else v = ((double)(((uint64_t)mag << 32) | x2) + 0.5) * 0x1p-32;
    const unsigned hi = (unsigned)__double2hiint(v);
    const int idx = PF_ICDF_IDX0 - (int)(hi >> (20 - PF_ICDF_B));
    const double *c = PF_ICDF_TAB_DEV[idx];
    const double q = fma(fma(fma(c[3], v, c[2]), v, c[1]), v, c[0]);
    return (x >> 31) ? -q : q;
}
template <int NB = PF_ICDF_NB_LDS, bool CLAMP = true>
__device__ __forceinline__ void pf_icdf_issue(uint32_t x, const double2 *lds_tab, double &v, double2 &c01, double2 &c23) {
    constexpr int NENT = NB << PF_ICDF_B;
    constexpr int SLOT0 = PF_ICDF_IDX0 - (NENT - 1);
    v = (double)(x & 0x7FFFFFFFu);
    const unsigned hi = (unsigned)__double2hiint(v);
    int slot = (int)(hi >> (20 - PF_ICDF_B)) - SLOT0;
    if (CLAMP) slot = slot > 0 ? slot : 0;
    c01 = lds_tab[slot]; c23 = lds_tab[NENT + slot];
}
#ifndef PF_ICDF_CLAMP_ADJ
#define PF_ICDF_CLAMP_ADJ 1
#endif
typedef double pf_v2d __attribute__((ext_vector_type(2)));
typedef const __attribute__((address_space(3))) pf_v2d *pf_lds_d2;
template <int NB = PF_ICDF_NB_LDS>
__device__ __forceinline__ uint32_t pf_icdf_adj(const double2 *lds_tab) {
    constexpr int NENT = NB << PF_ICDF_B;
    constexpr int SLOT0 = PF_ICDF_IDX0 - (NENT - 1);
    uint32_t off = (uint32_t)__builtin_amdgcn_readfirstlane((int)((uint32_t)(uintptr_t)(pf_lds_d2)lds_tab - (uint32_t)SLOT0 * 16u));
    asm volatile("" : "+s"(off));
    return off;
}
template <int NB = PF_ICDF_NB_LDS>
__device__ __forceinline__ void pf_icdf_issue_adj(uint32_t x, uint32_t adj, double &v, double2 &c01, double2 &c23) {
    constexpr int NENT = NB << PF_ICDF_B;
    v = (double)(x & 0x7FFFFFFFu);
    const unsigned hi = (unsigned)__double2hiint(v);
    unsigned idx = hi >> (20 - PF_ICDF_B);
#if PF_ICDF_CLAMP_ADJ
    idx = max(idx, (unsigned)(PF_ICDF_IDX0 - ((32 << PF_ICDF_B) - 1)));
#endif
    asm("" : "+v"(idx));
    const pf_lds_d2 e = (pf_lds_d2)(uintptr_t)(adj + (idx << 4));
    const pf_v2d a = e[0], b = e[NENT];
    c01 = make_double2(a.x, a.y); c23 = make_double2(b.x, b.y);
}
#define PF_ICDF_BFE_BITS 10
template <int NB = PF_ICDF_NB_LDS>
struct pf_icdf_bfe {
    static constexpr int NENT = NB << PF_ICDF_B;
    static constexpr int SLOT0 = PF_ICDF_IDX0 - (NENT - 1);
    static constexpr int BASE = SLOT0 & ((1 << PF_ICDF_BFE_BITS) - 1);
    static_assert((PF_ICDF_IDX0 >> PF_ICDF_BFE_BITS) == (SLOT0 >> PF_ICDF_BFE_BITS), "the LDS binades wrap in the bfe index");
    static constexpr int FRONT = BASE;
    static constexpr int BEHIND = (1 << PF_ICDF_BFE_BITS) - BASE - NENT;
};
#define PF_ICDF_BFE_FRONT (pf_icdf_bfe<>::FRONT)
#define PF_ICDF_BFE_BEHIND (pf_icdf_bfe<>::BEHIND)
template <int NB = PF_ICDF_NB_LDS>
__device__ __forceinline__ uint32_t pf_icdf_adj_bfe(const double2 *lds_tab) {
    uint32_t off = (uint32_t)__builtin_amdgcn_readfirstlane(
        (int)((uint32_t)(uintptr_t)(pf_lds_d2)lds_tab - (uint32_t)pf_icdf_bfe<NB>::BASE * 16u));
    asm volatile("" : "+s"(off));
    return off;
}
template <int NB = PF_ICDF_NB_LDS>
__device__ __forceinline__ void pf_icdf_issue_bfe(uint32_t x, uint32_t adj, double &v, double2 &c01, double2 &c23) {
    constexpr int NENT = NB << PF_ICDF_B;
    v = (double)(x & 0x7FFFFFFFu);
    const unsigned hi = (unsigned)__double2hiint(v);
    unsigned idx = (hi >> (20 - PF_ICDF_B)) & ((1u << PF_ICDF_BFE_BITS) - 1);
    asm("" : "+v"(idx));
    const pf_lds_d2 e = (pf_lds_d2)(uintptr_t)(adj + (idx << 4));
    const pf_v2d a = e[0], b = e[NENT];
    c01 = make_double2(a.x, a.y); c23 = make_double2(b.x, b.y);
}
__device__ __forceinline__ double pf_icdf_finish(uint32_t x, double v, const double2 &c01, const double2 &c23) {
    const double q = fma(fma(fma(c23.y, v, c23.x), v, c01.y), v, c01.x);
    unsigned hq;
    asm("v_bfi_b32 %0, %1, %2, %3" : "=v"(hq) : "s"(0x7FFFFFFFu), "v"((unsigned)__double2hiint(q)), "v"(x));
    return __hiloint2double((int)hq, __double2loint(q));
}
template <int NB = PF_ICDF_NB_LDS>
__device__ __forceinline__ bool pf_icdf_miss4(const uint32_t (&x)[4]) {
    const uint32_t m01 = min(x[0] & 0x7FFFFFFFu, x[1] & 0x7FFFFFFFu), m23 = min(x[2] & 0x7FFFFFFFu, x[3] & 0x7FFFFFFFu);
    return min(m01, m23) < (1u << (31 - NB));
}
template <int NB = PF_ICDF_NB_LDS>
__device__ __forceinline__ void pf_icdf4_fix(const uint32_t (&x)[4], uint32_t n, uint32_t g, uint32_t stream, uint32_t k0, uint32_t k1,
                                             double (&z)[4]) {
    uint32_t x2[4] = {0u, 0u, 0u, 0u};
    if (__any(pf_icdf_miss4<PF_ICDF_NB_LDS>(x))) pf_philox_normals(n, g, stream, 1u, k0, k1, x2);
#pragma unroll
    for (int t = 0; t < 4; ++t) if ((x[t] & 0x7FFFFFFFu) < (1u << (31 - NB))) z[t] = pf_icdf_any(x[t], x2[t]);
}
template <int NB = PF_ICDF_NB_LDS>
__device__ __forceinline__ void pf_icdf4(const uint32_t (&x)[4], uint32_t n, uint32_t g, uint32_t stream, uint32_t k0, uint32_t k1,
                                         const double2 *lds_tab, double (&z)[4]) {
#pragma unroll
    for (int t = 0; t < 4; ++t) {
        double dp;
        double2 c01, c23;
        pf_icdf_issue<NB>(x[t], lds_tab, dp, c01, c23);
        z[t] = pf_icdf_finish(x[t], dp, c01, c23);
    }
    if (__builtin_expect(__any(pf_icdf_miss4<NB>(x)), 0)) pf_icdf4_fix<NB>(x, n, g, stream, k0, k1, z);
}
template <int NB = PF_ICDF_NB_LDS>
__device__ __forceinline__ void pf_randn4(uint64_t seed, uint32_t g, uint32_t n, uint32_t stream, const double2 *lds_tab,
                                          double (&z)[4]) {
    uint32_t x[4];
    const uint32_t k0 = (uint32_t)seed, k1 = (uint32_t)(seed >> 32);
    pf_philox_normals(n, g, stream, 0u, k0, k1, x);
    pf_icdf4<NB>(x, n, g, stream, k0, k1, lds_tab, z);
}

__device__ __forceinline__ uint64_t pf_rand_u64(uint64_t seed, uint64_t t, uint32_t stream) {
    uint32_t x[4];
    pf_philox4x32_10((uint32_t)t, (uint32_t)(t >> 32), stream, 0u, (uint32_t)seed, (uint32_t)(seed >> 32), x);
    return (uint64_t)x[0] | ((uint64_t)x[1] << 32);
}

template <int CTRL, int ROW_MASK>
__device__ __forceinline__ double pf_dpp_add(double v) {
    const int lo = __double2loint(v), hi = __double2hiint(v);
    const int lo2 = __builtin_amdgcn_update_dpp(0, lo, CTRL, ROW_MASK, 0xf, true);
    const int hi2 = __builtin_amdgcn_update_dpp(0, hi, CTRL, ROW_MASK, 0xf, true);
    return v + __hiloint2double(hi2, lo2);
}
__device__ __forceinline__ double pf_readlane_f64(double x, int lane) {
    const int lo = __builtin_amdgcn_readlane(__double2loint(x), lane), hi = __builtin_amdgcn_readlane(__double2hiint(x), lane);
    return __hiloint2double(hi, lo);
}
__device__ __forceinline__ double pf_wave_sum(double v) {
    v = pf_dpp_add<0x111, 0xf>(v);
    v = pf_dpp_add<0x112, 0xf>(v);
    v = pf_dpp_add<0x114, 0xf>(v);
    v = pf_dpp_add<0x118, 0xf>(v);
    v = pf_dpp_add<0x142, 0xa>(v);
    v = pf_dpp_add<0x143, 0xc>(v);
    const int lo = __builtin_amdgcn_readlane(__double2loint(v), 63);
    const int hi = __builtin_amdgcn_readlane(__double2hiint(v), 63);
    return __hiloint2double(hi, lo);
}
__device__ __forceinline__ double pf_add_xor16(double s) {
    const unsigned lo = (unsigned)__double2loint(s), hi = (unsigned)__double2hiint(s);
    const auto a = __builtin_amdgcn_permlane16_swap(lo, lo, false, false);
    const auto b = __builtin_amdgcn_permlane16_swap(hi, hi, false, false);
    return __hiloint2double((int)b[0], (int)a[0]) + __hiloint2double((int)b[1], (int)a[1]);
}
__device__ __forceinline__ double pf_add_xor32(double s) {
    const unsigned lo = (unsigned)__double2loint(s), hi = (unsigned)__double2hiint(s);
    const auto a = __builtin_amdgcn_permlane32_swap(lo, lo, false, false);
    const auto b = __builtin_amdgcn_permlane32_swap(hi, hi, false, false);
    return __hiloint2double((int)b[0], (int)a[0]) + __hiloint2double((int)b[1], (int)a[1]);
}
__device__ __forceinline__ double pf_sum_q(double s) { return pf_add_xor32(pf_add_xor16(s)); }
__device__ __forceinline__ double pf_wave_max(double v) {
#pragma unroll
    for (int off = 32; off >= 1; off >>= 1) v = fmax(v, __shfl_xor(v, off, 64));
    return v;
}

template <int NV>
__device__ __forceinline__ void pf_block_sum(double (&v)[NV], double *red) {
    const int lane = threadIdx.x & 63, wave = threadIdx.x >> 6, nw = blockDim.x >> 6;
#pragma unroll
    for (int i = 0; i < NV; ++i) v[i] = pf_wave_sum(v[i]);
    __syncthreads();
    if (lane == 0) {
#pragma unroll
        for (int i = 0; i < NV; ++i) red[wave * NV + i] = v[i];
    }
    __syncthreads();
#pragma unroll
    for (int i = 0; i < NV; ++i) v[i] = red[i];
#pragma unroll 1
    for (int w = 1; w < nw; ++w) {
        const double *bw = red + w * NV;
#pragma unroll
        for (int i = 0; i < NV; ++i) v[i] += bw[i];
    }
}
template <int NV, int NVMAX, int NW = 0>
__device__ __forceinline__ void pf_block_sum_pp(double (&v)[NV], double *red, int &flip) {
    const int lane = threadIdx.x & 63, wave = threadIdx.x >> 6, nw = NW ? NW : (int)(blockDim.x >> 6);
    double *buf = red + flip * (nw * NVMAX);
    flip ^= 1;
#pragma unroll
    for (int i = 0; i < NV; ++i) v[i] = pf_wave_sum(v[i]);
    if (lane == 0) {
#pragma unroll
// ... 118 lines not shown
```

Before: 508.3 million.

## Fuse history walk and fit into one gated kernel with progress flags

Adds a single launch in which the first K workgroups run each path's history walk and publish progress through per-path atomic words every FIT_GATE_Q steps. The remaining workgroups, ordered by a host-computed fit order, spin until their point's history is published and then run the fit body. This is meant to overlap the serial history walk with fit work and remove a launch boundary. It risks deadlock-like stalls if the producer workgroups are not resident, so a spin limit with a lost counter falls back to the two-launch path and asks for a retry.

```diff
diff --git a/pathfinder.jl_amd/csrc/api_ctx.hip b/pathfinder.jl_amd/csrc/api_ctx.hip
--- a/pathfinder.jl_amd/csrc/api_ctx.hip
+++ b/pathfinder.jl_amd/csrc/api_ctx.hip
@@ -331,6 +331,11 @@
         if (launches) *launches = c->qf_lost_total;
         return PFMI_OK;
     }
+    if (strcmp(name, "fit_gate_lost") == 0) {
+        if (ms) *ms = 0.0;
+        if (launches) *launches = c->fit_lost_total;
+        return PFMI_OK;
+    }
     if (strncmp(name, "qf:", 3) == 0) {
         auto pl = c->qf_plans.find(name);
         if (ms) *ms = 0.0;
diff --git a/pathfinder.jl_amd/csrc/api_elbo.hip b/pathfinder.jl_amd/csrc/api_elbo.hip
--- a/pathfinder.jl_amd/csrc/api_elbo.hip
+++ b/pathfinder.jl_amd/csrc/api_elbo.hip
@@ -227,7 +227,10 @@
     for (int q = 0; q < 2; ++q)
         if (c->qf_share_s[q].cap >= sizeof(uint32_t))
             PF_TRY(pf_download(c, &(*lost2)[(size_t)q], c->qf_share_s[q].as<char>() + c->qf_share_s[q].cap - sizeof(uint32_t), sizeof(uint32_t)));
-    auto after = [c, lost2]() -> int32_t {
+    auto fit_lost = std::make_shared<uint32_t>(0u);
+    PF_TRY(fit_gate_queue(c, fit_lost));
+    auto after = [c, lost2, fit_lost]() -> int32_t {
+        PF_TRY(fit_gate_after(c, *fit_lost));
         uint32_t lost = (*lost2)[0] + (*lost2)[1];
         for (int q = 0; q < 2; ++q)
             if ((*lost2)[(size_t)q] != 0) (void)hipMemsetAsync(c->qf_share_s[q].as<char>() + c->qf_share_s[q].cap - sizeof(uint32_t), 0, sizeof(uint32_t), c->stream);
diff --git a/pathfinder.jl_amd/csrc/api_fit.hip b/pathfinder.jl_amd/csrc/api_fit.hip
--- a/pathfinder.jl_amd/csrc/api_fit.hip
+++ b/pathfinder.jl_amd/csrc/api_fit.hip
@@ -36,12 +36,31 @@
         const HistSeg sg{c->st_npts.as<int32_t>(), 0, INT_MAX, nullptr, nullptr, c->hinit};
         PF_TRY(pf_launch_history(c, eps, &sg));
         PF_TRY(pf_launch_fit(c, 0, (int)c->vcap));
+    } else if (pf_fit_gated_route(c)) {
+        PF_TRY(pf_launch_fit_gated(c, eps));
     } else {
         PF_TRY(pf_launch_history(c, eps));
         PF_TRY(pf_launch_fit(c));
     }
     c->fitted = true; c->elbo_done = false; c->pooled = false;
     return PFMI_OK;
+}
+
+int32_t fit_gate_queue(pfmi_ctx *c, const std::shared_ptr<uint32_t> &lost) {
+    *lost = 0;
+    if (!c->fit_gate_used) return PFMI_OK;
+    c->fit_gate_used = false;
+    return pf_download(c, lost.get(), c->fit_gate.as<unsigned long long>() + c->fit_gate_K, sizeof(uint32_t));
+}
+int32_t fit_gate_after(pfmi_ctx *c, uint32_t lost) {
+    if (lost == 0) return PFMI_OK;
+    (void)hipMemsetAsync(c->fit_gate.as<unsigned long long>() + c->fit_gate_K, 0, sizeof(unsigned long long), c->stream);
+    c->fit_no_gate = true;
+    c->fit_lost_total += lost;
+    c->fitted = false; c->elbo_done = false; c->pooled = false;
+    pf_set_error("fit: %u fit(s) gave up waiting for their path's history walk (GPU shared or dispatch serialised?); results discarded, later "
+                 "fits on this context run behind the walk as a launch of their own: enqueue the step again", lost);
+    return PFMI_ERR_RETRY;
 }
 
 extern "C" {
@@ -75,10 +94,12 @@
     if (logdet) PF_TRY(pf_download(c, logdet, c->logdet.p, sizeof(double) * c->P));
     if (n_rejected) PF_TRY(pf_download(c, r->data(), c->n_rej.p, sizeof(int32_t) * c->K));
     const int K = c->K;
-    auto widen = [r, n_rejected, K]() -> int32_t {
+    auto lost = std::make_shared<uint32_t>(0u);
+    PF_TRY(fit_gate_queue(c, lost));
+    auto widen = [c, lost, r, n_rejected, K]() -> int32_t {
         if (n_rejected)
             for (int k = 0; k < K; ++k) n_rejected[k] = (*r)[(size_t)k];
-        return PFMI_OK;
+        return fit_gate_after(c, *lost);
     };
     if (c->defer) { c->post_sync.push_back(widen); return PFMI_OK; }
     PF_TRY(pf_stream_sync(c));
diff --git a/pathfinder.jl_amd/csrc/api_inputs.hip b/pathfinder.jl_amd/csrc/api_inputs.hip
--- a/pathfinder.jl_amd/csrc/api_inputs.hip
+++ b/pathfinder.jl_amd/csrc/api_inputs.hip
@@ -1,4 +1,5 @@
 #include "api_internal.h"
+#include "fit_order.h"
 
 int32_t set_packed_layout(pfmi_ctx *c, int32_t K, int32_t d, const int64_t *counts) {
     c->off.assign((size_t)K + 1, 0);
@@ -12,6 +13,12 @@
     PF_TRY(c->d_off.ensure(sizeof(int64_t) * (K + 1)));
     PF_TRY(c->d_path_of.ensure(sizeof(int32_t) * P));
     PF_TRY(pf_upload(c, c->d_off.p, c->off.data(), sizeof(int64_t) * (K + 1)));
+    {
+        std::vector<int32_t> order;
+        pf_fit_gated_order(K, c->off.data(), order);
+        PF_TRY(c->fit_order.ensure(sizeof(int32_t) * P));
+        PF_TRY(pf_upload(c, c->fit_order.p, order.data(), sizeof(int32_t) * P));
+    }
     return pf_upload(c, c->d_path_of.p, c->path_of.data(), sizeof(int32_t) * P);
 }
 
diff --git a/pathfinder.jl_amd/csrc/api_internal.h b/pathfinder.jl_amd/csrc/api_internal.h
--- a/pathfinder.jl_amd/csrc/api_internal.h
+++ b/pathfinder.jl_amd/csrc/api_internal.h
@@ -42,6 +42,9 @@
 
 int32_t fit_reserve(pfmi_ctx *c, size_t P, int32_t K, size_t d, int32_t J, int32_t kpad);
 
+int32_t fit_gate_queue(pfmi_ctx *c, const std::shared_ptr<uint32_t> &lost);
+int32_t fit_gate_after(pfmi_ctx *c, uint32_t lost);
+
 int32_t elbo_reserve(pfmi_ctx *c, size_t P, int32_t K, int64_t N);
 int64_t devcb_chunk_fits(const pfmi_ctx *c, int64_t per_fit_doubles, int64_t nf, int64_t N);
 int32_t devcb_scan_block(pfmi_ctx *c, hipStream_t ss, const int32_t *list, const uint64_t *seeds, int64_t n, int64_t N, const double *d_u,
diff --git a/pathfinder.jl_amd/csrc/fit_args.h b/pathfinder.jl_amd/csrc/fit_args.h
--- a/pathfinder.jl_amd/csrc/fit_args.h
+++ b/pathfinder.jl_amd/csrc/fit_args.h
@@ -15,6 +15,16 @@
     int64_t P;
     double *big;
 };
+struct FitGate {
+    double eps;
+    int hinit, K;
+    double *alpha_all;
+    int32_t *hist_len, *hist_src, *n_rej, *acc_list;
+    unsigned long long *prog;
+    unsigned *lost;
+    unsigned epoch;
+    const int32_t *order;
+};
 #ifdef __HIPCC__
 __device__ __forceinline__ bool pf_fit_point(const FitArgs &A, int64_t idx, int64_t &p) {
     if (A.seg_len == 0) { p = idx; return true; }
diff --git a/pathfinder.jl_amd/csrc/fit_kernels.hip b/pathfinder.jl_amd/csrc/fit_kernels.hip
--- a/pathfinder.jl_amd/csrc/fit_kernels.hip
+++ b/pathfinder.jl_amd/csrc/fit_kernels.hip
@@ -1,5 +1,6 @@
 #include "pfmi_common.h"
 #include "fit_args.h"
+#include "fit_order.h"
 #include <limits.h>
 #include <stdlib.h>
 
@@ -20,15 +21,55 @@
 #ifndef HIST_PROF
 #define HIST_PROF 0
 #endif
+#ifndef PF_FIT_GATED_DEFAULT
+#define PF_FIT_GATED_DEFAULT 1
+#endif
 #define HIST_THREADS 256
 #define FIT_THREADS 256
 
-template <int EPT, int HIST_NT>
-__global__ __launch_bounds__(HIST_NT) void pf_history_kernel(
-    int d, int J, double eps, const int64_t *__restrict__ off, const double *__restrict__ theta,
+#ifndef FIT_GATE_Q
+#define FIT_GATE_Q 16
+#endif
+#ifndef FIT_GATE_SPINS
+#define FIT_GATE_SPINS 2000000
+#endif
+template <bool GATED, typename T>
+__device__ __forceinline__ void pf_gate_st(T *p, T v) {
+    if (GATED) __hip_atomic_store(p, v, __ATOMIC_RELAXED, __HIP_MEMORY_SCOPE_AGENT); else *p = v;
+}
+template <bool GATED>
+__device__ __forceinline__ int pf_gate_ld(const int32_t *p) {
+    return GATED ? __hip_atomic_load(p, __ATOMIC_RELAXED, __HIP_MEMORY_SCOPE_AGENT) : *p;
+}
+__device__ __forceinline__ void pf_walk_publish(unsigned long long *word, unsigned epoch, int l) {
+    asm volatile("s_waitcnt vmcnt(0)" ::: "memory");
+    __syncthreads();
+    if (threadIdx.x == 0)
+        __hip_atomic_store(word, ((unsigned long long)epoch << 32) | (unsigned)l, __ATOMIC_RELAXED, __HIP_MEMORY_SCOPE_AGENT);
+}
+__device__ __forceinline__ bool pf_fit_wait(const unsigned long long *word, unsigned epoch, int l, int *s_ok) {
+    if (threadIdx.x == 0) {
+        int spins = 0, ok = 0;
+        for (;;) {
+            const unsigned long long v = __hip_atomic_load(word, __ATOMIC_RELAXED, __HIP_MEMORY_SCOPE_AGENT);
+            if ((unsigned)(v >> 32) == epoch && (int)(unsigned)v >= l) { ok = 1; break; }
+            if (++spins >= FIT_GATE_SPINS) break;
+            __builtin_amdgcn_s_sleep(32);
+        }
+        __builtin_amdgcn_fence(__ATOMIC_ACQUIRE, "agent");
+        asm volatile("s_waitcnt vmcnt(0)" ::: "memory");
+        *s_ok = ok;
+    }
+    __syncthreads();
+    return *s_ok != 0;
+}
+
+template <int EPT, int HIST_NT, bool GATED>
+__device__ __forceinline__ void pf_history_role(
+    const int k, int d, int J, double eps, const int64_t *__restrict__ off, const double *__restrict__ theta,
     const double *__restrict__ grad, double *__restrict__ alpha_all, int *__restrict__ hist_len,
-    int *__restrict__ hist_src, int *__restrict__ n_rej, int *__restrict__ acc_list, HistSeg sg) {
-    const int k = blockIdx.x, tid = threadIdx.x;
+    int *__restrict__ hist_src, int *__restrict__ n_rej, int *__restrict__ acc_list, HistSeg sg, unsigned long long *prog, unsigned epoch) {
+    const int tid = threadIdx.x;
     const int64_t p0 = off[k];
     const int Ltot = sg.npts ? sg.npts[k] - 1 : (int)(off[k + 1] - p0 - 1);
     const int L = Ltot < sg.l_end - 1 ? Ltot : sg.l_end - 1;
@@ -56,13 +97,13 @@
             al[e] = alpha_all[(size_t)(p0 + b) * d + ic]; ial[e] = sg.ial_state[(size_t)k * d + ic];
         } else {
             al[e] = 1.0; ial[e] = 1.0;
-            if (i < d) alpha_all[(size_t)p0 * d + i] = 1.0;
+            if (i < d) pf_gate_st<GATED>(alpha_all + (size_t)p0 * d + i, 1.0);
         }
     }
 #pragma unroll
     for (int q = 0; q < NS; ++q) load_point(b + q, tq[q], gq[q]);
     if (sg.l_begin > 0) n_acc = sg.nacc_state[k];
-    else if (tid == 0) hist_len[p0] = 0;
+    else if (tid == 0) pf_gate_st<GATED>(hist_len + p0, 0);
 #if HIST_PROF
     long long hp[5] = {0, 0, 0, 0, 0}, hp_last = clock64();
 #define HP_STAMP(k) do { const long long t_ = clock64(); hp[k] += t_ - hp_last; hp_last = t_; } while (0)
@@ -108,19 +149,41 @@
 #pragma unroll
         for (int e = 0; e < EPT; ++e) {
             const int i = tid + HIST_NT * e;
-            if (i < d) alpha_all[(size_t)(p0 + l) * d + i] = al[e];
+            if (i < d) pf_gate_st<GATED>(alpha_all + (size_t)(p0 + l) * d + i, al[e]);
         }
         if (tid == 0) {
             if (accept) acc[n_acc - 1] = l - 1;
-            hist_len[p0 + l] = n_acc < J ? n_acc : J;
-            hist_src[(size_t)(p0 + l) * J] = n_acc;
+            pf_gate_st<GATED>(hist_len + p0 + l, n_acc < J ? n_acc : J);
+            pf_gate_st<GATED>(hist_src + (size_t)(p0 + l) * J, n_acc);
         }
         HP_STAMP(3);
     };
+    auto expand = [&](const int lo, const int hi) {
+        for (int q = lo + 1 + tid; q <= hi; q += HIST_NT) {
+            int *row = hist_src + (size_t)(p0 + q) * J;
+            const int na = pf_gate_ld<GATED>(row), re = na < J ? na : J;
+            int first = 0;
+            for (int c = 0; c < re; ++c) {
+                const int v = acc[na - re + c];
+                if (c == 0) first = v; else pf_gate_st<GATED>(row + c, v);
+            }
+            pf_gate_st<GATED>(row, re > 0 ? first : 0);
+        }
+    };
+    int lo_pub = b;
+    auto publish = [&](const int hi) {
+        __threadfence_block();
+        __syncthreads();
+        expand(lo_pub, hi);
+        pf_walk_publish(prog + k, epoch, hi);
+        lo_pub = hi;
+    };
+    if (GATED) publish(b);
     int l = b + 1;
     for (; l + NS - 1 <= L; l += NS) {
 #pragma unroll
         for (int q = 0; q < NS; ++q) step(l + q, tq[q], gq[q], tq[(q + 1) % NS], gq[(q + 1) % NS]);
+        if (GATED && (l + NS - 1 - b) % FIT_GATE_Q == 0) publish(l + NS - 1);
     }
     const int rem = L - l + 1;
 #pragma unroll
@@ -137,18 +200,17 @@
         for (int e = 0; e < EPT; ++e) { const int i = tid + HIST_NT * e; if (i < d) sg.ial_state[(size_t)k * d + i] = ial[e]; }
         if (tid == 0) sg.nacc_state[k] = n_acc;
     }
+    if (GATED) { publish(L); return; }
     __threadfence_block();
     __syncthreads();
-    for (int q = b + 1 + tid; q <= L; q += HIST_NT) {
-        int *row = hist_src + (size_t)(p0 + q) * J;
-        const int na = row[0], re = na < J ? na : J;
-        int first = 0;
-        for (int c = 0; c < re; ++c) {
-            const int v = acc[na - re + c];
-            if (c == 0) first = v; else row[c] = v;
-        }
-        row[0] = re > 0 ? first : 0;
-    }
+    expand(b, L);
+}
+template <int EPT, int HIST_NT>
+__global__ __launch_bounds__(HIST_NT) void pf_history_kernel(
+    int d, int J, double eps, const int64_t *__restrict__ off, const double *__restrict__ theta,
+    const double *__restrict__ grad, double *__restrict__ alpha_all, int *__restrict__ hist_len,
+    int *__restrict__ hist_src, int *__restrict__ n_rej, int *__restrict__ acc_list, HistSeg sg) {
+    pf_history_role<EPT, HIST_NT, false>(blockIdx.x, d, J, eps, off, theta, grad, alpha_all, hist_len, hist_src, n_rej, acc_list, sg, nullptr, 0u);
 }
 
 template <int EPT>
@@ -686,6 +748,7 @@
 
 template <int KPAD, int RPT, int NT>
 __global__ __launch_bounds__(NT, (KPAD <= 8 ? 4 : KPAD <= 12 ? 3 : 2)) void pf_fit_reg_kernel(FitArgs A) {
+    constexpr bool GATED = false;
     int64_t p;
     {
         const int P = (int)gridDim.x, x = blockIdx.x & 7, slot = blockIdx.x >> 3, q8 = P >> 3, r8 = P & 7;
@@ -693,376 +756,85 @@
         if (FITREG_XCD == 0) idx = blockIdx.x;
         if (!pf_fit_point(A, idx, p)) { if (threadIdx.x == 0) A.status[p] = PFMI_FIT_ABSENT; return; }
     }
-    const int tid = threadIdx.x;
-    const int d = A.d, J = A.J;
-    const int path = A.path_of[p];
-    const int64_t p0 = A.off[path];
-    const int j = A.hist_len[p], m = 2 * j, k = d < m ? d : m;
-    const double *alpha = A.alpha_all + (size_t)p * d;
-    double *Vh = A.vh + (size_t)p * d * KPAD;
-    double *sqa = A.sqrt_alpha + (size_t)p * d;
-    double *mu = A.mu + (size_t)p * d;
-    const double *theta_p = A.theta + (size_t)p * d, *grad_p = A.grad + (size_t)p * d;
-
-    constexpr int NVMAX = KPAD;
-    __shared__ __attribute__((aligned(16))) double red[2 * (NT / 64) * NVMAX];
-    int flip = 0;
-    __shared__ double sRow[2][KPAD];
-    __shared__ double sD[KPAD * KPAD], sR[KPAD * KPAD], sT[KPAD * KPAD], sV[KPAD * KPAD], sG[KPAD * KPAD];
-    __shared__ double sX1[(KPAD / 2) * KPAD], sX2[(KPAD / 2) * KPAD], sX3[(KPAD / 2) * KPAD];
-    __shared__ double sGv[KPAD * KPAD], sVt[KPAD * KPAD];
-    __shared__ double sT12[KPAD], sDl[KPAD];
-    __shared__ double sLogdetV;
-    __shared__ int sStatus;
-
-#if FITREG_PROF
-    long long prof[10] = {0, 0, 0, 0, 0, 0, 0, 0, 0, 0}, tlast = wall_clock64();
-#endif
-    double a[RPT][KPAD];
-    double bad = 0.0, ldu = 0.0;
-    double isa_r[RPT], al_r[RPT];
-    int rl_r[RPT];
-#pragma unroll
-    for (int i = 0; i < RPT; ++i) { const int row = tid + NT * i; rl_r[i] = row < d ? row : d - 1; }
-#pragma unroll
-    for (int i = 0; i < RPT; ++i) al_r[i] = alpha[rl_r[i]];
-#pragma unroll
-    for (int i = 0; i < RPT; ++i) {
-        const int row = tid + NT * i;
-        const double al = al_r[i];
-        const double s = sqrt(al);
-        isa_r[i] = 1.0 / s;
-        if (row < d) {
-            if (!(al > 0.0) || !isfinite(al)) bad = 1.0;
-            sqa[row] = s;
-            ldu += log(s);
-        }
-    }
+#include "fit_reg_body.h"
+}
+
+template <int KPAD, int RPT, int EPT>
+__global__ __launch_bounds__(256, (KPAD <= 8 ? 4 : KPAD <= 12 ? 3 : 2)) void pf_fit_gated_kernel(FitArgs A, FitGate G) {
+    constexpr int NT = 256;
+    constexpr bool GATED = true;
+    if ((int)blockIdx.x < G.K) {
+        const HistSeg sg{nullptr, 0, INT_MAX, nullptr, nullptr, G.hinit};
+        pf_history_role<EPT, 256, true>((int)blockIdx.x, A.d, A.J, G.eps, A.off, A.theta, A.grad, G.alpha_all, G.hist_len, G.hist_src, G.n_rej,
+                                        G.acc_list, sg, G.prog, G.epoch);
+        return;
+    }
+    __shared__ int sGateOk;
+    const int64_t p = G.order[pf_fit_gated_pos(G.K, A.P, blockIdx.x)];
     {
-        double v[2] = {bad, ldu};
-        pf_block_sum_pp<2, NVMAX>(v, red, flip);
-        bad = v[0]; ldu = v[1];
-    }
-    for (int t = tid; t < KPAD * KPAD; t += NT) { sD[t] = 0.0; sR[t] = 0.0; sT[t] = 0.0; sV[t] = 0.0; sG[t] = 0.0; sGv[t] = 0.0; sVt[t] = 0.0; }
-    const size_t sm = (size_t)p * KPAD * KPAD;
-    if (bad > 0.0) {
-#pragma unroll
-        for (int i = 0; i < RPT; ++i) {
-            const int row = tid + NT * i;
-            if (row < d) {
-                mu[row] = NAN;
-                for (int c = 0; c < KPAD; ++c) Vh[(size_t)row * KPAD + c] = 0.0;
-            }
-        }
-        for (int t = tid; t < KPAD * KPAD; t += NT) { A.tmat[sm + t] = 0.0; A.vchol[sm + t] = 0.0; A.rq[sm + t] = 0.0; A.dmat[sm + t] = 0.0; }
-        if (tid == 0) { A.status[p] = PFMI_FIT_A_NOT_PD; A.logdet[p] = NAN; }
-        return;
-    }
-    FR_STAMP(0);
-#pragma unroll
-    for (int i = 0; i < RPT; ++i)
-#pragma unroll
-        for (int c = 0; c < KPAD; ++c) a[i][c] = 0.0;
-#pragma unroll
-    for (int c = 0; c < KPAD / 2; ++c) {
-        if (c >= j) continue;
-        const int src = A.hist_src[(size_t)p * J + c];
-        const double *g0 = A.grad + (size_t)(p0 + src) * d, *g1 = g0 + d, *t0 = A.theta + (size_t)(p0 + src) * d, *t1 = t0 + d;
-        double vg0[RPT], vg1[RPT], vt0[RPT], vt1[RPT];
-#pragma unroll
-        for (int i = 0; i < RPT; ++i) { vg0[i] = g0[rl_r[i]]; vg1[i] = g1[rl_r[i]]; vt0[i] = t0[rl_r[i]]; vt1[i] = t1[rl_r[i]]; }
-#pragma unroll
-        for (int i = 0; i < RPT; ++i) {
-            const bool in = tid + NT * i < d;
-            const double y = vg0[i] - vg1[i];
-            const double sx = vt1[i] - vt0[i];
-            const double by = in ? (al_r[i] * y) * isa_r[i] : 0.0, bs = in ? sx * isa_r[i] : 0.0;
-            a[i][c] = by;
-            if (j == KPAD / 2) a[i][KPAD / 2 + c] = bs;
-            else {
-#pragma unroll
-                for (int cc = 0; cc < KPAD; ++cc) if (cc == j + c) a[i][cc] = bs;
-            }
-        }
-    }
-    FR_STAMP(1);
-    double acc[KPAD];
-#pragma unroll
-    for (int c = 0; c < KPAD; ++c) {
-        if (c >= k) continue;
-        double *srow = sRow[c & 1];
-        if (tid == c) {
-#pragma unroll
-            for (int cc = 0; cc < KPAD; ++cc) srow[cc] = a[0][cc];
-        }
-#pragma unroll
-        for (int cc = 0; cc < KPAD; ++cc) acc[cc] = 0.0;
-#pragma unroll
-        for (int i = 0; i < RPT; ++i) {
-            const int row = tid + NT * i;
-            if (row > c) {
-                double xc = 0.0;
-#pragma unroll
-                for (int cc = 0; cc < KPAD; ++cc) if (cc == c) xc = a[i][cc];
-#pragma unroll
-                for (int cc = 0; cc < KPAD; ++cc) acc[cc] += xc * a[i][cc];
-            }
-        }
-        pf_block_sum_mv<KPAD, NVMAX>(acc, red, flip);
-        double xn2 = 0.0;
-#pragma unroll
-        for (int cc = 0; cc < KPAD; ++cc) if (cc == c) xn2 = acc[cc];
-        const double alpha_c = srow[c];
-        double tau, scal, beta;
-        if (xn2 == 0.0) { tau = 0.0; scal = 0.0; beta = alpha_c; }
-        else {
-            beta = -copysign(sqrt(fma(alpha_c, alpha_c, xn2)), alpha_c);
-            tau = (beta - alpha_c) / beta;
-            scal = 1.0 / (alpha_c - beta);
-        }
-        double (&wv)[KPAD] = acc;
-#pragma unroll
-        for (int cc = 0; cc < KPAD; ++cc) {
-            const double vdot = srow[cc] + scal * acc[cc];
-            wv[cc] = (cc > c) ? tau * vdot : vdot;
-        }
-        if (tid <= c && tid < KPAD) {
-            double v = 0.0;
-#pragma unroll
-            for (int b = 0; b < KPAD; ++b) if (b >= tid && b < c) v += sT[tid * KPAD + b] * wv[b];
-            const double tnew = (tid == c) ? tau : -tau * v;
-            sT[tid * KPAD + c] = tnew;
-            if (tid == c) {
-#pragma unroll
-                for (int cc = 0; cc < KPAD; ++cc) if (cc < c) { sGv[c * KPAD + cc] = wv[cc]; sGv[cc * KPAD + c] = wv[cc]; }
-                sGv[c * KPAD + c] = fma(scal * scal, xn2, 1.0);
-            }
-        }
-#pragma unroll
-        for (int i = 0; i < RPT; ++i) {
-            const int row = tid + NT * i;
-            if (row > c) {
-                double v = 0.0;
-#pragma unroll
-                for (int cc = 0; cc < KPAD; ++cc) if (cc == c) v = a[i][cc] * scal;
-#pragma unroll
-                for (int cc = 0; cc < KPAD; ++cc) {
-                    if (cc == c) a[i][cc] = v;
-                    else if (cc > c) a[i][cc] -= wv[cc] * v;
-                }
-            } else if (row == c) {
-#pragma unroll
-                for (int cc = 0; cc < KPAD; ++cc) {
-                    if (cc == c) a[i][cc] = beta;
-                    else if (cc > c) a[i][cc] -= wv[cc];
-                }
-            }
-        }
-    }
-    FR_STAMP(2);
-    if (tid < k) {
-#pragma unroll
-        for (int cc = 0; cc < KPAD; ++cc) {
-            if (cc >= tid) {
-                sR[tid * KPAD + cc] = (cc < m) ? a[0][cc] : 0.0;
-                a[0][cc] = (cc == tid) ? 1.0 : 0.0;
-            }
-            if (cc < k) sVt[tid * KPAD + cc] = a[0][cc];
-        }
-    }
-    __syncthreads();
-    for (int t = tid; t < m * m; t += NT) {
-        const int aa = t / m, b = t % m, u1 = (aa < b ? aa : b) < k - 1 ? (aa < b ? aa : b) : k - 1;
-        double v = 0.0;
-        for (int u = 0; u <= u1; ++u) v += sR[u * KPAD + aa] * sR[u * KPAD + b];
-        sG[aa * KPAD + b] = v;
-    }
-    __syncthreads();
-    if (j > 0) {
-        double *R = sX1, *nRinv = sX2;
-        for (int t = tid; t < j * j; t += NT) {
-            const int aa = t / j, b = t % j;
-            R[aa * KPAD + b] = (b >= aa) ? sG[(j + aa) * KPAD + b] : 0.0;
-            nRinv[aa * KPAD + b] = 0.0;
-        }
-    }
-    __syncthreads();
-    if (tid < j) {
-        const double *R = sX1;
-        double *nRinv = sX2;
-        const int c = tid;
-        for (int r = c; r >= 0; --r) {
-            double rhs = (r == c) ? -1.0 : 0.0;
-            for (int t = r + 1; t <= c; ++t) rhs -= R[r * KPAD + t] * nRinv[t * KPAD + c];
-            nRinv[r * KPAD + c] = rhs / R[r * KPAD + r];
-        }
-    }
-    __syncthreads();
-    if (j > 0) {
-        for (int t = tid; t < j * j; t += NT) {
-            const int aa = t / j, b = t % j;
-            sD[aa * KPAD + (j + b)] = sX2[aa * KPAD + b];
-            sD[(j + aa) * KPAD + b] = sX2[b * KPAD + aa];
-            double v = (aa <= b) ? sG[aa * KPAD + b] : sG[b * KPAD + aa];
-            if (aa == b) v += sX1[aa * KPAD + aa];
-            sX3[aa * KPAD + b] = v;
-        }
-    }
-    __syncthreads();
-    if (j > 0) {
-        for (int t = tid; t < j * j; t += NT) {
-            const int aa = t / j, b = t % j;
-            double v = 0.0;
-            for (int u = 0; u <= b; ++u) v += sX3[aa * KPAD + u] * sX2[u * KPAD + b];
-            sG[aa * KPAD + b] = v;
-        }
-    }
-    __syncthreads();
-    if (j > 0) {
-        for (int t = tid; t < j * j; t += NT) {
-            const int aa = t / j, b = t % j;
-            double v = 0.0;
-            for (int u = 0; u <= aa; ++u) v += sX2[u * KPAD + aa] * sG[u * KPAD + b];
-            sD[(j + aa) * KPAD + (j + b)] = v;
-        }
-    }
-    __syncthreads();
-    FR_STAMP(3);
-    for (int t = tid; t < k * m; t += NT) {
-        const int aa = t / m, b = t % m;
-        double v = 0.0;
-        for (int u = aa; u < m; ++u) v += sR[aa * KPAD + u] * sD[u * KPAD + b];
-        sG[aa * KPAD + b] = v;
-    }
-    __syncthreads();
-    for (int t = tid; t < k * k; t += NT) {
-        const int aa = t / k, b = t % k;
-        if (b >= aa) {
-            double v = (aa == b) ? 1.0 : 0.0;
-            for (int u = b; u < m; ++u) v += sG[aa * KPAD + u] * sR[b * KPAD + u];
-            sV[aa * KPAD + b] = v;
-        }
-    }
-    __syncthreads();
-    FR_STAMP(4);
-    if (tid < 64) {
-        const int b = tid;
-        double col[KPAD];
-#pragma unroll
-        for (int t = 0; t < KPAD; ++t) col[t] = (b < k && t <= b) ? sV[t * KPAD + b] : 0.0;
-        int status = PFMI_FIT_OK;
-        double ldv = 0.0;
-#pragma unroll
-        for (int c = 0; c < ((FITREG_ABLATE & 1) ? 0 : KPAD); ++c) {
-            if (c >= k || status != PFMI_FIT_OK) continue;
-            double v = col[c];
-#pragma unroll
-            for (int t = 0; t < c; ++t) {
-                const double vtc = pf_readlane_f64(col[t], c);
-                v -= vtc * col[t];
-            }
-            const double diag = pf_readlane_f64(v, c);
-            if (!(diag > 0.0) || !isfinite(diag)) { status = PFMI_FIT_C_NOT_PD; continue; }
-            const double dc = sqrt(diag);
-            ldv = ldv + log(dc);
-            col[c] = (b == c) ? dc : (b > c ? v / dc : col[c]);
-        }
-#pragma unroll
-        for (int t = 0; t < KPAD; ++t) if (b < k && t <= b) sV[t * KPAD + b] = col[t];
-        if (b >= k && b < KPAD) sV[b * KPAD + b] = 1.0;
-        if (b == 0) { sStatus = status; sLogdetV = ldv; }
-    }
-    __syncthreads();
-    FR_STAMP(5);
-    for (int t = tid; t < KPAD * KPAD; t += NT) {
-        A.tmat[sm + t] = sT[t]; A.vchol[sm + t] = sV[t]; A.rq[sm + t] = sR[t]; A.dmat[sm + t] = sD[t];
-    }
-#pragma unroll
-    for (int i = 0; i < RPT; ++i) {
-        const int row = tid + NT * i;
-        if (row < d) {
-            double2 *o = reinterpret_cast<double2 *>(Vh + (size_t)row * KPAD);
-#pragma unroll
-            for (int cc = 0; cc < KPAD; cc += 2) o[cc >> 1] = make_double2(a[i][cc], a[i][cc + 1]);
-        }
-    }
-    if (sStatus != PFMI_FIT_OK) {
-#pragma unroll
-        for (int i = 0; i < RPT; ++i) { const int row = tid + NT * i; if (row < d) mu[row] = NAN; }
-        if (tid == 0) { A.status[p] = sStatus; A.logdet[p] = NAN; }
-        return;
-    }
-    FR_STAMP(6);
-    if (FITREG_ABLATE & 2) return;
-    double agv[RPT];
-#pragma unroll
-    for (int i = 0; i < RPT; ++i) {
-        const int row = tid + NT * i;
-        agv[i] = (row < d) ? sqa[row] * grad_p[row] : 0.0;
-    }
-#pragma unroll
-    for (int cc = 0; cc < KPAD; ++cc) acc[cc] = 0.0;
-#pragma unroll
-    for (int i = 0; i < RPT; ++i)
-#pragma unroll
-        for (int cc = 0; cc < KPAD; ++cc) acc[cc] += agv[i] * a[i][cc];
-    pf_block_sum_mv<KPAD, NVMAX>(acc, red, flip);
-    if (tid < 64) {
-        const int aa = tid < KPAD ? tid : KPAD - 1;
-        const bool live = tid < k;
-        double w1l = 0.0, t1l = 0.0;
-#pragma unroll
-        for (int b = 0; b < KPAD; ++b) {
-            w1l = (b == aa) ? acc[b] : w1l;
-            t1l += sT[b * KPAD + aa] * acc[b];
-        }
-        double hbl = live ? agv[0] : 0.0;
-#pragma unroll
-        for (int cc = 0; cc < KPAD; ++cc) hbl -= sVt[aa * KPAD + cc] * pf_readlane_f64(t1l, cc);
-        hbl = live ? hbl : 0.0;
-        double tmpl = 0.0;
-#pragma unroll
-        for (int b = 0; b < KPAD; ++b) tmpl += sV[aa * KPAD + b] * pf_readlane_f64(hbl, b);
-        double hdl = 0.0;
-#pragma unroll
-        for (int b = 0; b < KPAD; ++b) hdl += sV[b * KPAD + aa] * pf_readlane_f64(tmpl, b);
-        const double dll = live ? hdl - hbl : 0.0;
-        double w2l = w1l;
-#pragma unroll
-        for (int b = 0; b < KPAD; ++b) w2l -= sGv[aa * KPAD + b] * pf_readlane_f64(t1l, b);
-#pragma unroll
-        for (int r = 0; r < KPAD; ++r) w2l += sVt[r * KPAD + aa] * pf_readlane_f64(dll, r);
-        double t2l = 0.0;
-#pragma unroll
-        for (int b = 0; b < KPAD; ++b) t2l += sT[aa * KPAD + b] * pf_readlane_f64(w2l, b);
-        if (tid < KPAD) { sT12[tid] = t1l + t2l; sDl[tid] = dll; }
-    }
-    __syncthreads();
-    double t12[KPAD];
-#pragma unroll
-    for (int cc = 0; cc < KPAD; ++cc) t12[cc] = sT12[cc];
-    const double dl0 = (tid < k) ? sDl[tid < KPAD ? tid : 0] : 0.0;
-#pragma unroll
-    for (int i = 0; i < RPT; ++i) {
-        const int row = tid + NT * i;
-        if (row < d) {
-            double v = agv[i];
-#pragma unroll
-            for (int cc = 0; cc < KPAD; ++cc) v -= a[i][cc] * t12[cc];
-            if (i == 0) v += dl0;
-            mu[row] = theta_p[row] + sqa[row] * v;
-        }
-    }
-    FR_STAMP(7);
-#if FITREG_PROF
-    if ((blockIdx.x & 511) == 7 && tid == 0)
-        printf("FITREG_PROF wg %d (10 ns ticks): prologue %lld rows %lld QR %lld gram+D %lld C %lld chol %lld out %lld mean %lld\n", (int)blockIdx.x, prof[0],
-               prof[1], prof[2], prof[3], prof[4], prof[5], prof[6], prof[7]);
-#endif
-    if (tid == 0) {
-        A.status[p] = PFMI_FIT_OK;
-        A.logdet[p] = 2.0 * (ldu + sLogdetV);
-    }
+        const int wpath = A.path_of[p];
+        if (!pf_fit_wait(G.prog + wpath, G.epoch, (int)(p - A.off[wpath]), &sGateOk)) {
+            for (int i = threadIdx.x; i < A.d; i += NT) A.mu[(size_t)p * A.d + i] = NAN;
+            if (threadIdx.x == 0) { A.status[p] = PFMI_FIT_NONFINITE; A.logdet[p] = NAN; atomicAdd(G.lost, 1u); }
+            return;
+        }
+    }
+#include "fit_reg_body.h"
+}
+
+template <int KPAD>
+static bool launch_fit_gated_t(pfmi_ctx *c, const FitArgs &a, const FitGate &g) {
+    if constexpr (KPAD <= 16) {
+        const dim3 grid((unsigned)(g.K + a.P)), block(256);
+        if (a.d <= 512) hipLaunchKernelGGL((pf_fit_gated_kernel<KPAD, 2, 2>), grid, block, 0, c->stream, a, g);
+        else hipLaunchKernelGGL((pf_fit_gated_kernel<KPAD, 4, 4>), grid, block, 0, c->stream, a, g);
+        return true;
+    }
+    return false;
+}
+
+static void fit_args_fill(pfmi_ctx *c, FitArgs &a, int seg_l0, int seg_len) {
+    a.d = c->d; a.J = c->J;
+    a.seg_l0 = seg_l0; a.seg_len = seg_len; a.vcap = c->vcap; a.npts = c->st_npts.as<int32_t>();
+    a.off = c->d_off.as<int64_t>(); a.path_of = c->d_path_of.as<int32_t>();
+    a.theta = c->th(); a.grad = c->gr(); a.alpha_all = c->alpha_all.as<double>();
+    a.hist_len = c->hist_len.as<int32_t>(); a.hist_src = c->hist_src.as<int32_t>();
+    a.vh = c->vh.as<double>(); a.tmat = c->tmat.as<double>(); a.vchol = c->vchol.as<double>();
+    a.rq = c->rq.as<double>(); a.dmat = c->dmat.as<double>(); a.sqrt_alpha = c->sqrt_alpha.as<double>();
+    a.mu = c->mu.as<double>(); a.logdet = c->logdet.as<double>(); a.status = c->status.as<int32_t>();
+    a.P = seg_len > 0 ? (int64_t)c->K * seg_len : c->P;
+    a.big = nullptr;
+}
+
+bool pf_fit_gated_route(const pfmi_ctx *c) {
+    if (c->virt || c->d <= 256 || c->d > 1024 || c->kpad > 16 || c->fit_no_gate || c->fit_order.p == nullptr) return false;
+    if (pf_debug_get("PFMI_FIT_KERNEL") || pf_debug_get("PFMI_HISTORY_KERNEL")) return false;
+    const char *g = pf_debug_get("PFMI_FIT_GATED");
+    return g ? g[0] != '0' : PF_FIT_GATED_DEFAULT != 0;
+}
+int32_t pf_launch_fit_gated(pfmi_ctx *c, double eps) {
+    PF_TRY(c->fit_gate.ensure(sizeof(unsigned long long) * ((size_t)c->K + 1)));
+    if (c->fit_gate_K != c->K || c->fit_epoch == 0xffffffffu) {
+        PF_HIP(hipMemsetAsync(c->fit_gate.p, 0, c->fit_gate.cap, c->stream));
+        c->fit_gate_K = c->K; c->fit_epoch = 0;
+    }
+    FitArgs a;
+    fit_args_fill(c, a, 0, 0);
+    FitGate g;
+    g.eps = eps; g.hinit = c->hinit; g.K = c->K;
+    g.alpha_all = c->alpha_all.as<double>(); g.hist_len = c->hist_len.as<int32_t>(); g.hist_src = c->hist_src.as<int32_t>();
+    g.n_rej = c->n_rej.as<int32_t>(); g.acc_list = c->hist_acc.as<int32_t>();
+    g.prog = c->fit_gate.as<unsigned long long>();
+    g.lost = reinterpret_cast<unsigned *>(g.prog + c->K);
+    g.epoch = ++c->fit_epoch;
+    g.order = c->fit_order.as<int32_t>();
+    pf_kernel_begin(c);
+    PF_CHECK((pf_dispatch_kpad<4, 8, 12, 16>(c->kpad, [&](auto KP) { launch_fit_gated_t<KP()>(c, a, g); })), PFMI_ERR_UNSUPPORTED,
+             "unsupported kpad %d", c->kpad);
+    pf_kernel_end(c, "fit");
+    PF_HIP(hipGetLastError());
+    c->fit_gate_used = true;
+    return PFMI_OK;
 }
 
 int32_t pf_launch_history(pfmi_ctx *c, double eps, const HistSeg *seg) {
@@ -1130,17 +902,8 @@
 
 int32_t pf_launch_fit(pfmi_ctx *c, int seg_l0, int seg_len) {
     FitArgs a;
-    a.d = c->d; a.J = c->J;
-    a.seg_l0 = seg_l0; a.seg_len = seg_len; a.vcap = c->vcap; a.npts = c->st_npts.as<int32_t>();
     PF_CHECK(seg_len == 0 || c->virt, PFMI_ERR_STATE, "fit: segment launches need the streaming layout");
-    a.off = c->d_off.as<int64_t>(); a.path_of = c->d_path_of.as<int32_t>();
-    a.theta = c->th(); a.grad = c->gr(); a.alpha_all = c->alpha_all.as<double>();
-    a.hist_len = c->hist_len.as<int32_t>(); a.hist_src = c->hist_src.as<int32_t>();
-    a.vh = c->vh.as<double>(); a.tmat = c->tmat.as<double>(); a.vchol = c->vchol.as<double>();
-    a.rq = c->rq.as<double>(); a.dmat = c->dmat.as<double>(); a.sqrt_alpha = c->sqrt_alpha.as<double>();
-    a.mu = c->mu.as<double>(); a.logdet = c->logdet.as<double>(); a.status = c->status.as<int32_t>();
-    a.P = seg_len > 0 ? (int64_t)c->K * seg_len : c->P;
-    a.big = nullptr;
+    fit_args_fill(c, a, seg_l0, seg_len);
     pf_kernel_begin(c);
     {
         const char *force = pf_debug_get("PFMI_FIT_KERNEL");
diff --git a/pathfinder.jl_amd/csrc/fit_order.h b/pathfinder.jl_amd/csrc/fit_order.h
--- /dev/null
+++ b/pathfinder.jl_amd/csrc/fit_order.h
@@ -0,0 +1,38 @@
+#pragma once
+#include <stdint.h>
+#include <algorithm>
+#include <vector>
+
+#if defined(__HIPCC__)
+#define PF_ORDER_HD __host__ __device__
+#else
+#define PF_ORDER_HD
+#endif
+
+PF_ORDER_HD inline int64_t pf_fit_gated_pos(int64_t K, int64_t P, int64_t b) {
+    const int x = (int)(b & 7);
+    int64_t start = 0, first_x = 0;
+    for (int xx = 0; xx <= x; ++xx) {
+        const int64_t first = K + ((xx - K) & 7);
+        if (xx == x) { first_x = first; break; }
+        if (first < K + P) start += (K + P - 1 - first) / 8 + 1;
+    }
+    return start + ((b - first_x) >> 3);
+}
+
+inline void pf_fit_gated_order(int64_t K, const int64_t *off, std::vector<int32_t> &order) {
+    const int64_t P = off[K];
+    order.resize((size_t)P);
+    std::vector<int32_t> l_of((size_t)P);
+    for (int64_t k = 0; k < K; ++k)
+        for (int64_t p = off[k]; p < off[k + 1]; ++p) l_of[(size_t)p] = (int32_t)(p - off[k]);
+    for (int64_t p = 0; p < P; ++p) order[(size_t)p] = (int32_t)p;
+    int64_t start = 0;
+    for (int x = 0; x < 8; ++x) {
+        const int64_t first = K + ((x - K) & 7);
+        const int64_t n = first < K + P ? (K + P - 1 - first) / 8 + 1 : 0;
+        std::stable_sort(order.begin() + start, order.begin() + start + n,
+                         [&](int32_t a, int32_t b) { return l_of[(size_t)a] < l_of[(size_t)b]; });
+        start += n;
+    }
+}
diff --git a/pathfinder.jl_amd/csrc/fit_reg_body.h b/pathfinder.jl_amd/csrc/fit_reg_body.h
--- /dev/null
+++ b/pathfinder.jl_amd/csrc/fit_reg_body.h
@@ -0,0 +1,370 @@
+    const int tid = threadIdx.x;
+    const int d = A.d, J = A.J;
+    const int path = A.path_of[p];
+    const int64_t p0 = A.off[path];
+    const int j = pf_gate_ld<GATED>(A.hist_len + p), m = 2 * j, k = d < m ? d : m;
+    const double *alpha = A.alpha_all + (size_t)p * d;
+    double *Vh = A.vh + (size_t)p * d * KPAD;
+    double *sqa = A.sqrt_alpha + (size_t)p * d;
+    double *mu = A.mu + (size_t)p * d;
+    const double *theta_p = A.theta + (size_t)p * d, *grad_p = A.grad + (size_t)p * d;
+
+    constexpr int NVMAX = KPAD;
+    __shared__ __attribute__((aligned(16))) double red[2 * (NT / 64) * NVMAX];
+    int flip = 0;
+    __shared__ double sRow[2][KPAD];
+    __shared__ double sD[KPAD * KPAD], sR[KPAD * KPAD], sT[KPAD * KPAD], sV[KPAD * KPAD], sG[KPAD * KPAD];
+    __shared__ double sX1[(KPAD / 2) * KPAD], sX2[(KPAD / 2) * KPAD], sX3[(KPAD / 2) * KPAD];
+    __shared__ double sGv[KPAD * KPAD], sVt[KPAD * KPAD];
+    __shared__ double sT12[KPAD], sDl[KPAD];
+    __shared__ double sLogdetV;
+    __shared__ int sStatus;
+
+#if FITREG_PROF
+    long long prof[10] = {0, 0, 0, 0, 0, 0, 0, 0, 0, 0}, tlast = wall_clock64();
+#endif
+    double a[RPT][KPAD];
+    double bad = 0.0, ldu = 0.0;
+    double isa_r[RPT], al_r[RPT];
+    int rl_r[RPT];
+#pragma unroll
+    for (int i = 0; i < RPT; ++i) { const int row = tid + NT * i; rl_r[i] = row < d ? row : d - 1; }
+#pragma unroll
+    for (int i = 0; i < RPT; ++i) al_r[i] = alpha[rl_r[i]];
+#pragma unroll
+    for (int i = 0; i < RPT; ++i) {
+        const int row = tid + NT * i;
+        const double al = al_r[i];
+        const double s = sqrt(al);
+        isa_r[i] = 1.0 / s;
+        if (row < d) {
+            if (!(al > 0.0) || !isfinite(al)) bad = 1.0;
+            sqa[row] = s;
+            ldu += log(s);
+        }
+    }
+    {
+        double v[2] = {bad, ldu};
+        pf_block_sum_pp<2, NVMAX>(v, red, flip);
+        bad = v[0]; ldu = v[1];
+    }
+    for (int t = tid; t < KPAD * KPAD; t += NT) { sD[t] = 0.0; sR[t] = 0.0; sT[t] = 0.0; sV[t] = 0.0; sG[t] = 0.0; sGv[t] = 0.0; sVt[t] = 0.0; }
+    const size_t sm = (size_t)p * KPAD * KPAD;
+    if (bad > 0.0) {
+#pragma unroll
+        for (int i = 0; i < RPT; ++i) {
+            const int row = tid + NT * i;
+            if (row < d) {
+                mu[row] = NAN;
+                for (int c = 0; c < KPAD; ++c) Vh[(size_t)row * KPAD + c] = 0.0;
+            }
+        }
+        for (int t = tid; t < KPAD * KPAD; t += NT) { A.tmat[sm + t] = 0.0; A.vchol[sm + t] = 0.0; A.rq[sm + t] = 0.0; A.dmat[sm + t] = 0.0; }
+        if (tid == 0) { A.status[p] = PFMI_FIT_A_NOT_PD; A.logdet[p] = NAN; }
+        return;
+    }
+    FR_STAMP(0);
+#pragma unroll
+    for (int i = 0; i < RPT; ++i)
+#pragma unroll
+        for (int c = 0; c < KPAD; ++c) a[i][c] = 0.0;
+#pragma unroll
+    for (int c = 0; c < KPAD / 2; ++c) {
+        if (c >= j) continue;
+        const int src = pf_gate_ld<GATED>(A.hist_src + (size_t)p * J + c);
+        const double *g0 = A.grad + (size_t)(p0 + src) * d, *g1 = g0 + d, *t0 = A.theta + (size_t)(p0 + src) * d, *t1 = t0 + d;
+        double vg0[RPT], vg1[RPT], vt0[RPT], vt1[RPT];
+#pragma unroll
+        for (int i = 0; i < RPT; ++i) { vg0[i] = g0[rl_r[i]]; vg1[i] = g1[rl_r[i]]; vt0[i] = t0[rl_r[i]]; vt1[i] = t1[rl_r[i]]; }
+#pragma unroll
+        for (int i = 0; i < RPT; ++i) {
+            const bool in = tid + NT * i < d;
+            const double y = vg0[i] - vg1[i];
+            const double sx = vt1[i] - vt0[i];
+            const double by = in ? (al_r[i] * y) * isa_r[i] : 0.0, bs = in ? sx * isa_r[i] : 0.0;
+            a[i][c] = by;
+            if (j == KPAD / 2) a[i][KPAD / 2 + c] = bs;
+            else {
+#pragma unroll
+                for (int cc = 0; cc < KPAD; ++cc) if (cc == j + c) a[i][cc] = bs;
+            }
+        }
+    }
+    FR_STAMP(1);
+    double acc[KPAD];
+#pragma unroll
+    for (int c = 0; c < KPAD; ++c) {
+        if (c >= k) continue;
+        double *srow = sRow[c & 1];
+        if (tid == c) {
+#pragma unroll
+            for (int cc = 0; cc < KPAD; ++cc) srow[cc] = a[0][cc];
+        }
+#pragma unroll
+        for (int cc = 0; cc < KPAD; ++cc) acc[cc] = 0.0;
+#pragma unroll
+        for (int i = 0; i < RPT; ++i) {
+            const int row = tid + NT * i;
+            if (row > c) {
+                double xc = 0.0;
+#pragma unroll
+                for (int cc = 0; cc < KPAD; ++cc) if (cc == c) xc = a[i][cc];
+#pragma unroll
+                for (int cc = 0; cc < KPAD; ++cc) acc[cc] += xc * a[i][cc];
+            }
+        }
+        pf_block_sum_mv<KPAD, NVMAX>(acc, red, flip);
+        double xn2 = 0.0;
+#pragma unroll
+        for (int cc = 0; cc < KPAD; ++cc) if (cc == c) xn2 = acc[cc];
+        const double alpha_c = srow[c];
+        double tau, scal, beta;
+        if (xn2 == 0.0) { tau = 0.0; scal = 0.0; beta = alpha_c; }
+        else {
+            beta = -copysign(sqrt(fma(alpha_c, alpha_c, xn2)), alpha_c);
+            tau = (beta - alpha_c) / beta;
+            scal = 1.0 / (alpha_c - beta);
+        }
+        double (&wv)[KPAD] = acc;
+#pragma unroll
+        for (int cc = 0; cc < KPAD; ++cc) {
+            const double vdot = srow[cc] + scal * acc[cc];
+            wv[cc] = (cc > c) ? tau * vdot : vdot;
+        }
+        if (tid <= c && tid < KPAD) {
+            double v = 0.0;
+#pragma unroll
+            for (int b = 0; b < KPAD; ++b) if (b >= tid && b < c) v += sT[tid * KPAD + b] * wv[b];
+            const double tnew = (tid == c) ? tau : -tau * v;
+            sT[tid * KPAD + c] = tnew;
+            if (tid == c) {
+#pragma unroll
+                for (int cc = 0; cc < KPAD; ++cc) if (cc < c) { sGv[c * KPAD + cc] = wv[cc]; sGv[cc * KPAD + c] = wv[cc]; }
+                sGv[c * KPAD + c] = fma(scal * scal, xn2, 1.0);
+            }
+        }
+#pragma unroll
+        for (int i = 0; i < RPT; ++i) {
+            const int row = tid + NT * i;
+            if (row > c) {
+                double v = 0.0;
+#pragma unroll
+                for (int cc = 0; cc < KPAD; ++cc) if (cc == c) v = a[i][cc] * scal;
+#pragma unroll
+                for (int cc = 0; cc < KPAD; ++cc) {
+                    if (cc == c) a[i][cc] = v;
+                    else if (cc > c) a[i][cc] -= wv[cc] * v;
+                }
+            } else if (row == c) {
+#pragma unroll
+                for (int cc = 0; cc < KPAD; ++cc) {
+                    if (cc == c) a[i][cc] = beta;
+                    else if (cc > c) a[i][cc] -= wv[cc];
+                }
+            }
+        }
+    }
+    FR_STAMP(2);
+    if (tid < k) {
+#pragma unroll
+        for (int cc = 0; cc < KPAD; ++cc) {
+            if (cc >= tid) {
+                sR[tid * KPAD + cc] = (cc < m) ? a[0][cc] : 0.0;
+                a[0][cc] = (cc == tid) ? 1.0 : 0.0;
+            }
+            if (cc < k) sVt[tid * KPAD + cc] = a[0][cc];
+        }
+    }
+    __syncthreads();
+    for (int t = tid; t < m * m; t += NT) {
+        const int aa = t / m, b = t % m, u1 = (aa < b ? aa : b) < k - 1 ? (aa < b ? aa : b) : k - 1;
+        double v = 0.0;
+        for (int u = 0; u <= u1; ++u) v += sR[u * KPAD + aa] * sR[u * KPAD + b];
+        sG[aa * KPAD + b] = v;
+    }
+    __syncthreads();
+    if (j > 0) {
+        double *R = sX1, *nRinv = sX2;
+        for (int t = tid; t < j * j; t += NT) {
+            const int aa = t / j, b = t % j;
+            R[aa * KPAD + b] = (b >= aa) ? sG[(j + aa) * KPAD + b] : 0.0;
+            nRinv[aa * KPAD + b] = 0.0;
+        }
+    }
+    __syncthreads();
+    if (tid < j) {
+        const double *R = sX1;
+        double *nRinv = sX2;
+        const int c = tid;
+        for (int r = c; r >= 0; --r) {
+            double rhs = (r == c) ? -1.0 : 0.0;
+            for (int t = r + 1; t <= c; ++t) rhs -= R[r * KPAD + t] * nRinv[t * KPAD + c];
+            nRinv[r * KPAD + c] = rhs / R[r * KPAD + r];
+        }
+    }
+    __syncthreads();
+    if (j > 0) {
+        for (int t = tid; t < j * j; t += NT) {
+            const int aa = t / j, b = t % j;
+            sD[aa * KPAD + (j + b)] = sX2[aa * KPAD + b];
+            sD[(j + aa) * KPAD + b] = sX2[b * KPAD + aa];
+            double v = (aa <= b) ? sG[aa * KPAD + b] : sG[b * KPAD + aa];
+            if (aa == b) v += sX1[aa * KPAD + aa];
+            sX3[aa * KPAD + b] = v;
+        }
+    }
+    __syncthreads();
+    if (j > 0) {
+        for (int t = tid; t < j * j; t += NT) {
+            const int aa = t / j, b = t % j;
+            double v = 0.0;
+            for (int u = 0; u <= b; ++u) v += sX3[aa * KPAD + u] * sX2[u * KPAD + b];
+            sG[aa * KPAD + b] = v;
+        }
+    }
+    __syncthreads();
+    if (j > 0) {
+        for (int t = tid; t < j * j; t += NT) {
+            const int aa = t / j, b = t % j;
+            double v = 0.0;
+            for (int u = 0; u <= aa; ++u) v += sX2[u * KPAD + aa] * sG[u * KPAD + b];
+            sD[(j + aa) * KPAD + (j + b)] = v;
+        }
+    }
+    __syncthreads();
+    FR_STAMP(3);
+    for (int t = tid; t < k * m; t += NT) {
+        const int aa = t / m, b = t % m;
+        double v = 0.0;
+        for (int u = aa; u < m; ++u) v += sR[aa * KPAD + u] * sD[u * KPAD + b];
+        sG[aa * KPAD + b] = v;
+    }
+    __syncthreads();
+    for (int t = tid; t < k * k; t += NT) {
+        const int aa = t / k, b = t % k;
+        if (b >= aa) {
+            double v = (aa == b) ? 1.0 : 0.0;
+            for (int u = b; u < m; ++u) v += sG[aa * KPAD + u] * sR[b * KPAD + u];
+            sV[aa * KPAD + b] = v;
+        }
+    }
+    __syncthreads();
+    FR_STAMP(4);
+    if (tid < 64) {
+        const int b = tid;
+        double col[KPAD];
+#pragma unroll
+        for (int t = 0; t < KPAD; ++t) col[t] = (b < k && t <= b) ? sV[t * KPAD + b] : 0.0;
+        int status = PFMI_FIT_OK;
+        double ldv = 0.0;
+#pragma unroll
+        for (int c = 0; c < ((FITREG_ABLATE & 1) ? 0 : KPAD); ++c) {
+            if (c >= k || status != PFMI_FIT_OK) continue;
+            double v = col[c];
+#pragma unroll
+            for (int t = 0; t < c; ++t) {
+                const double vtc = pf_readlane_f64(col[t], c);
+                v -= vtc * col[t];
+            }
+            const double diag = pf_readlane_f64(v, c);
+            if (!(diag > 0.0) || !isfinite(diag)) { status = PFMI_FIT_C_NOT_PD; continue; }
+            const double dc = sqrt(diag);
+            ldv = ldv + log(dc);
+            col[c] = (b == c) ? dc : (b > c ? v / dc : col[c]);
+        }
+#pragma unroll
+        for (int t = 0; t < KPAD; ++t) if (b < k && t <= b) sV[t * KPAD + b] = col[t];
+        if (b >= k && b < KPAD) sV[b * KPAD + b] = 1.0;
+        if (b == 0) { sStatus = status; sLogdetV = ldv; }
+    }
+    __syncthreads();
+    FR_STAMP(5);
+    for (int t = tid; t < KPAD * KPAD; t += NT) {
+        A.tmat[sm + t] = sT[t]; A.vchol[sm + t] = sV[t]; A.rq[sm + t] = sR[t]; A.dmat[sm + t] = sD[t];
+    }
+#pragma unroll
+    for (int i = 0; i < RPT; ++i) {
+        const int row = tid + NT * i;
+        if (row < d) {
+            double2 *o = reinterpret_cast<double2 *>(Vh + (size_t)row * KPAD);
+#pragma unroll
+            for (int cc = 0; cc < KPAD; cc += 2) o[cc >> 1] = make_double2(a[i][cc], a[i][cc + 1]);
+        }
+    }
+    if (sStatus != PFMI_FIT_OK) {
+#pragma unroll
+        for (int i = 0; i < RPT; ++i) { const int row = tid + NT * i; if (row < d) mu[row] = NAN; }
+        if (tid == 0) { A.status[p] = sStatus; A.logdet[p] = NAN; }
+        return;
+    }
+    FR_STAMP(6);
+    if (FITREG_ABLATE & 2) return;
+    double agv[RPT];
+#pragma unroll
+    for (int i = 0; i < RPT; ++i) {
+        const int row = tid + NT * i;
+        agv[i] = (row < d) ? sqa[row] * grad_p[row] : 0.0;
+    }
+#pragma unroll
+    for (int cc = 0; cc < KPAD; ++cc) acc[cc] = 0.0;
+#pragma unroll
+    for (int i = 0; i < RPT; ++i)
+#pragma unroll
+        for (int cc = 0; cc < KPAD; ++cc) acc[cc] += agv[i] * a[i][cc];
+    pf_block_sum_mv<KPAD, NVMAX>(acc, red, flip);
+    if (tid < 64) {
+        const int aa = tid < KPAD ? tid : KPAD - 1;
+        const bool live = tid < k;
+        double w1l = 0.0, t1l = 0.0;
+#pragma unroll
+        for (int b = 0; b < KPAD; ++b) {
+            w1l = (b == aa) ? acc[b] : w1l;
+            t1l += sT[b * KPAD + aa] * acc[b];
+        }
+        double hbl = live ? agv[0] : 0.0;
+#pragma unroll
+        for (int cc = 0; cc < KPAD; ++cc) hbl -= sVt[aa * KPAD + cc] * pf_readlane_f64(t1l, cc);
+        hbl = live ? hbl : 0.0;
+        double tmpl = 0.0;
+#pragma unroll
+        for (int b = 0; b < KPAD; ++b) tmpl += sV[aa * KPAD + b] * pf_readlane_f64(hbl, b);
+        double hdl = 0.0;
+#pragma unroll
+        for (int b = 0; b < KPAD; ++b) hdl += sV[b * KPAD + aa] * pf_readlane_f64(tmpl, b);
+        const double dll = live ? hdl - hbl : 0.0;
+        double w2l = w1l;
+#pragma unroll
+        for (int b = 0; b < KPAD; ++b) w2l -= sGv[aa * KPAD + b] * pf_readlane_f64(t1l, b);
+#pragma unroll
+        for (int r = 0; r < KPAD; ++r) w2l += sVt[r * KPAD + aa] * pf_readlane_f64(dll, r);
+        double t2l = 0.0;
+#pragma unroll
+        for (int b = 0; b < KPAD; ++b) t2l += sT[aa * KPAD + b] * pf_readlane_f64(w2l, b);
+        if (tid < KPAD) { sT12[tid] = t1l + t2l; sDl[tid] = dll; }
+    }
+    __syncthreads();
+    double t12[KPAD];
+#pragma unroll
+    for (int cc = 0; cc < KPAD; ++cc) t12[cc] = sT12[cc];
+    const double dl0 = (tid < k) ? sDl[tid < KPAD ? tid : 0] : 0.0;
+#pragma unroll
+    for (int i = 0; i < RPT; ++i) {
+        const int row = tid + NT * i;
+        if (row < d) {
+            double v = agv[i];
+#pragma unroll
+            for (int cc = 0; cc < KPAD; ++cc) v -= a[i][cc] * t12[cc];
+            if (i == 0) v += dl0;
+            mu[row] = theta_p[row] + sqa[row] * v;
+        }
+    }
+    FR_STAMP(7);
+#if FITREG_PROF
+    if ((blockIdx.x & 511) == 7 && tid == 0)
+        printf("FITREG_PROF wg %d (10 ns ticks): prologue %lld rows %lld QR %lld gram+D %lld C %lld chol %lld out %lld mean %lld\n", (int)blockIdx.x, prof[0],
+               prof[1], prof[2], prof[3], prof[4], prof[5], prof[6], prof[7]);
+#endif
+    if (tid == 0) {
+        A.status[p] = PFMI_FIT_OK;
+        A.logdet[p] = 2.0 * (ldu + sLogdetV);
+    }
diff --git a/pathfinder.jl_amd/csrc/pfmi_common.h b/pathfinder.jl_amd/csrc/pfmi_common.h
--- a/pathfinder.jl_amd/csrc/pfmi_common.h
+++ b/pathfinder.jl_amd/csrc/pfmi_common.h
@@ -178,6 +178,13 @@
     DevBuf mu;
     DevBuf logdet;
     DevBuf status;
+    DevBuf fit_order;
+    DevBuf fit_gate;
+    int32_t fit_gate_K = -1;
+    uint32_t fit_epoch = 0;
+    bool fit_gate_used = false;
+    bool fit_no_gate = false;
+    int64_t fit_lost_total = 0;
     DevBuf fit_scratch;
 
     bool elbo_done = false;
@@ -260,6 +267,8 @@
 struct HistSeg;
 int32_t pf_launch_history(pfmi_ctx *c, double eps, const HistSeg *seg = nullptr);
 int32_t pf_launch_fit(pfmi_ctx *c, int seg_l0 = 0, int seg_len = 0);
+bool pf_fit_gated_route(const pfmi_ctx *c);
+int32_t pf_launch_fit_gated(pfmi_ctx *c, double eps);
 int32_t pf_launch_elbo_draws(pfmi_ctx *c, const int32_t *d_points, const uint64_t *d_seeds, int64_t nfits,
                              int64_t n0, int64_t N, const double *d_u, int64_t u_stride,
                              double *d_x, int64_t x_stride, double *d_logp, double *d_logq,
```

Result: no change. 512.1 million (median of 6 runs) (+0.8%).
